# awslabs/aws-c-compression

Measured on AMD Instinct MI355X. Metric: GiB/s input consumed, encode+decode, 1 GiB random bytes; % HBM roofline, higher is better.
Workload: dtype u8

## Files before the change

### aws-c-compression_amd/csrc/hip/decode_common.hpp

```cpp
#ifndef HUFFMAN_AMD_DECODE_COMMON_HPP
#define HUFFMAN_AMD_DECODE_COMMON_HPP
#include "kernels_common.hpp"

namespace {


constexpr u32 kSubWords = HUFD_DEC_SUB_BYTES / 4;
constexpr u32 kSubRows = kSubWords + 2;
constexpr u32 kRowStride = HUFD_DEC_LANES + 1;
constexpr u32 kChunkWords = (kSubRows * kRowStride + 3u) & ~3u;
constexpr u32 kGroupLanes = 16;
constexpr u32 kGroups = HUFD_DEC_LANES / kGroupLanes;
constexpr u32 kQuarters = 4;
constexpr u32 kQuarterBits = HUFD_DEC_SUB_BITS / kQuarters;
constexpr u32 kCpRows = HUFD_DEC_CP_ROWS;
constexpr u32 kEmitThreads = HUFD_DEC_LANES * kQuarters;
constexpr u32 kExitStop = 15, kExitNoRef = 14;
constexpr u8 kRegularFew = 4;

__device__ __forceinline__ u16 fn_pack(bool stop, u32 exit_state, u32 count) {
    return (u16)((stop ? 0x8000u : 0u) | (exit_state << 11) | count);
}
__device__ __forceinline__ u32 wide_pack(bool stop, u32 exit_state, u32 count) {
    return (stop ? 0x80000000u : 0u) | (exit_state << 26) | count;
}
__device__ __forceinline__ u32 widen(u16 f) {
    return wide_pack((f & 0x8000u) != 0, (f >> 11) & 15u, f & 0x7FFu);
}
__device__ __forceinline__ bool wide_stop(u32 f) {
    return (f >> 31) != 0;
}
__device__ __forceinline__ u32 wide_state(u32 f) {
    return (f >> 26) & 31u;
}
__device__ __forceinline__ u32 wide_count(u32 f) {
    return f & 0x03FFFFFFu;
}

__device__ __forceinline__ u32 chunk_word(const u32 *timg, u32 lane, u32 r) {
    return timg[r * kRowStride + lane];
}

__device__ __forceinline__ u32 chunk_window(const u32 *timg, u32 lane, u32 pos) {
    const u32 r = pos >> 5;
    const u64 two = ((u64)chunk_word(timg, lane, r) << 32) | chunk_word(timg, lane, r + 1);
    return (u32)((two << (pos & 31)) >> 32);
}

template <u32 THREADS = HUFD_DEC_LANES>
__device__ __forceinline__ void chunk_load(u32 *timg, const u8 *src, u64 valid_bytes) {
    const u32 t = threadIdx.x;
// ... 512 lines not shown
```

### aws-c-compression_amd/csrc/hip/decode_emit_kernels.hip

```cpp
#include "decode_common.hpp"
#include "launch_common.hpp"

namespace {


__device__ __forceinline__ void dec_emit_chunk(
    const hufd_tables &tb,
    const hufd_dec_item *items,
    const u32 *chunk_item,
    const u8 *d_in,
    u8 *d_out,
    const u16 *fn_tab,
    const u16 *cp_tab,
    const u16 *lane_count_tab,
    const u8 *chunk_regular,
    const u32 *chunk_entry,
    const u64 *chunk_base,
    hufd_dec_result *results,
    u32 c) {

    const u32 ns = tb.n_states;
    u32 *timg = reinterpret_cast<u32 *>(dyn_lds);
    u8 *stage = reinterpret_cast<u8 *>(timg + kChunkWords);
    u16 *ftab = reinterpret_cast<u16 *>(stage);
    u32 *gtab = reinterpret_cast<u32 *>(stage + HUFD_DEC_STAGE_BYTES);
    u32 *g_entry = gtab + kGroups * HUFD_DEC_MAX_STATES;
    u32 *g_base = g_entry + kGroups;
    u32 *l_entry = g_base + kGroups;
    u32 *l_base = l_entry + HUFD_DEC_LANES;
    u32 *l_cnt = l_base + HUFD_DEC_LANES;
    u32 *blk_count = l_cnt + HUFD_DEC_LANES;
    u16 *cpt = reinterpret_cast<u16 *>(blk_count + 4);
    u16 *lut = cpt + kCpRows * HUFD_DEC_LANES;

    const u32 t = threadIdx.x;
    const u32 lane = t % HUFD_DEC_LANES, q = t / HUFD_DEC_LANES;
    const u32 entry = chunk_entry[c];
    if (!(entry & 0x100u)) {
        return;
    }
    const u32 item_index = chunk_item[c];
    const hufd_dec_item it = items[item_index];
    const u64 chunk_off = (u64)(c - it.first_chunk) * HUFD_DEC_CHUNK_BYTES;
    const u64 valid = it.in_len > chunk_off ? it.in_len - chunk_off : 0;
    const u64 cbase = chunk_base[c];

    HUFD_STAMP(1, 0);
    const u16 my_cp = cp_tab[(u64)c * kCpRows * HUFD_DEC_LANES + t];
    u16 my_fn[(HUFD_DEC_MAX_STATES * HUFD_DEC_LANES + kEmitThreads - 1) / kEmitThreads];
#pragma unroll
    for (u32 j = 0; j < sizeof(my_fn) / sizeof(my_fn[0]); ++j) {
        const u32 i = t + j * kEmitThreads;
        my_fn[j] = i < ns * HUFD_DEC_LANES ? fn_tab[(u64)c * ns * HUFD_DEC_LANES + i] : (u16)0;
    }
    chunk_load<kEmitThreads>(timg, d_in + it.in_off + chunk_off, valid);
    lut_load<kEmitThreads>(lut, tb);
    cpt[t] = my_cp;
#pragma unroll
    for (u32 j = 0; j < sizeof(my_fn) / sizeof(my_fn[0]); ++j) {
        const u32 i = t + j * kEmitThreads;
        if (i < ns * HUFD_DEC_LANES) {
            ftab[i] = my_fn[j];
        }
    }
    __syncthreads();
    HUFD_STAMP(1, 1);

    const u32 merged_row = (kQuarters - 1) * HUFD_DEC_LANES;
    bool lane_reached = false;
    u32 lane_state = 0, lane_count = 0, lane_stop = 0, lane_incl = 0;
    if (t < HUFD_DEC_LANES) {
        lane_state = t ? (u32)(cpt[merged_row + t - 1] >> 12) : (entry & 0xFFu);
        l_entry[t] = lane_state == kExitStop ? 1u : 0u;
    }
    if (t == 0) {
        blk_count[1] = 0;
    }
    __syncthreads();
    if (t < HUFD_DEC_LANES) {
        u32 first_unreached = HUFD_DEC_LANES;
        for (u32 w = HUFD_DEC_LANES / kWave; w-- > 0;) {
            const u64 b = __ballot(l_entry[w * kWave + (t & (kWave - 1))] != 0);
            first_unreached = b ? w * kWave + (u32)__builtin_ctzll(b) : first_unreached;
        }
        lane_reached = t < first_unreached;
        const u32 mine_row = cpt[merged_row + t];
        lane_stop = (mine_row >> 12) == kExitStop ? 1u : 0u;
        const bool fits = !lane_reached || (lane_state < kExitNoRef && ((mine_row >> lane_state) & 1u));
        if (!fits) {
            blk_count[1] = 1;
        }
        lane_state = (fits && lane_reached) ? lane_state : 0;
        lane_count = !lane_reached ? 0u
                     : (t != 0 && chunk_regular[c] != 0) ? (u32)lane_count_tab[(u64)c * HUFD_DEC_LANES + t]
                                                         : (u32)(ftab[lane_state * HUFD_DEC_LANES + t] & 0x7FFu);
        lane_incl = wave_inclusive_sum(lane_count, t & (kWave - 1));
        if ((t & (kWave - 1)) == kWave - 1) {
            g_base[t / kWave] = lane_incl;
        }
    }
    __syncthreads();
    const bool all_fit = blk_count[1] == 0;
    if (all_fit) {
        if (t < HUFD_DEC_LANES) {
            u32 before = 0, total = 0;
#pragma unroll
            for (u32 w = 0; w < HUFD_DEC_LANES / kWave; ++w) {
                const u32 sum = g_base[w];
                before += w < t / kWave ? sum : 0;
                total += sum;
            }
            l_base[t] = before + lane_incl - lane_count;
            l_cnt[t] = lane_count;
            l_entry[t] = entry_pack(lane_reached ? lane_state : 0u, lane_reached) | ((lane_reached && lane_stop) ? 0x200u : 0u);
            if (t == 0) {
                blk_count[0] = total;
            }
        }
    } else {
        if (t < kGroups * ns) {
            const u32 g = t / ns, start = t % ns;
            gtab[g * ns + start] = wide_pack(chain_fold(kGroupLanes, start, [&](u32 i, u32 stt) {
                return widen(ftab[stt * HUFD_DEC_LANES + g * kGroupLanes + i]);
            }));
        }
        __syncthreads();
        if (t == 0) {
// ... 107 lines not shown
    HUFD_STAMP(1, 4);

    if (staged && writable) {
        u8 *gbase = out_ptr - mis;
        const u32 lo = mis, hi = mis + writable;
        const u32 row_lo = (lo + 15) >> 4, row_hi = hi >> 4;
        if (row_lo <= row_hi) {
            for (u32 b = lo + t; b < row_lo * 16; b += kEmitThreads) {
                gbase[b] = stage[b];
            }
            for (u32 r = row_lo + t; r < row_hi; r += kEmitThreads) {
                *reinterpret_cast<uint4 *>(gbase + (u64)r * 16) = *reinterpret_cast<const uint4 *>(stage + r * 16);
            }
            for (u32 b = row_hi * 16 + t; b < hi; b += kEmitThreads) {
                gbase[b] = stage[b];
            }
        } else {
            for (u32 b = lo + t; b < hi; b += kEmitThreads) {
                gbase[b] = stage[b];
            }
        }
    }
    HUFD_STAMP(1, 5);
}

__global__ __launch_bounds__(kEmitThreads, 4) void dec_emit_kernel(
    hufd_tables tb,
    const hufd_dec_item *items,
    const u32 *chunk_item,
    u32 n_chunks,
    const u8 *d_in,
    u8 *d_out,
    const u16 *fn_tab,
    const u16 *cp_tab,
    const u16 *lane_count_tab,
    const u8 *chunk_regular,
    const u32 *chunk_entry,
    const u64 *chunk_base,
    hufd_dec_result *results,
    const u32 *list,
    const u32 *list_count,
    u32 *counters = nullptr ,
    u32 *summary = nullptr ,
    u32 self_cleared = 0 ) {
    if (blockIdx.x == 0 && threadIdx.x == 0) {
        if (summary) {
            for (u32 k = 0; k < HUFK_DEC_COUNTERS; ++k) {
                summary[k] = counters[k];
            }
        }
        if (self_cleared) {
            counters[HUFK_DEC_COUNT_SLOW] = 0;
            counters[HUFK_DEC_COUNT_LONG] = 0;
            counters[HUFK_DEC_COUNT_FEW] = 0;
        }
    }
    const u32 n = list ? *list_count : n_chunks;
    for (u32 i = blockIdx.x; i < n; i += gridDim.x) {
        dec_emit_chunk(tb, items, chunk_item, d_in, d_out, fn_tab, cp_tab, lane_count_tab, chunk_regular, chunk_entry, chunk_base, results, list ? list[i] : i);
        __syncthreads();
    }
}


constexpr u32 kEmitChains = 2;
constexpr u32 kEmitFastThreads = kEmitThreads / kEmitChains;

template <u32 LB>
struct emit_shared {
    u32 wlut[1u << LB];
    u32 lane_base[HUFD_DEC_LANES];
    u32 wave_tot[HUFD_DEC_LANES / 64];
    u32 pad[4];
    u8 dump[512];
    u32 tail_words[2][kTailWords];
    u8 stage[HUFD_DEC_STAGE_BYTES + 32];
};

template <u32 LB>
__host__ __device__ constexpr u32 emit_lds_bytes(u32 stage_bytes) {
    return (u32)sizeof(emit_shared<LB>) - HUFD_DEC_STAGE_BYTES + stage_bytes;
}


template <u32 LB, bool TAIL, u32 SURE = 0>
__device__ __forceinline__ void dec_emit_fast_chunk(
    const u32 c,
    const hufd_tables &tb,
    const hufd_chunk_rec *chunk_rec,
    const u8 *d_in,
    u8 *d_out,
    const u16 *cp_tab,
    const u16 *lane_count,
    const hufd_emit_rec *emit_rec,
    hufd_dec_result *results,
    u32 *slow_list,
    u32 *slow_count,
    u32 *dense_list,
    u32 *dense_count,
    u32 stage_limit ) {

    emit_shared<LB> &sh = *reinterpret_cast<emit_shared<LB> *>(dyn_lds);
    const u32 t = threadIdx.x;
    const u32 q = t % kQuarters;
    const u32 lanes[kEmitChains] = {2 * (t / kQuarters), 2 * (t / kQuarters) + 1};
    constexpr bool kNarrowBlock = TAIL && LB == 10;
    constexpr u32 kLutPerThread = kNarrowBlock ? (1u << LB) / HUFD_DEC_LANES : ((1u << LB) + kEmitFastThreads - 1) / kEmitFastThreads;
    const u32 lut_stride = kNarrowBlock ? blockDim.x : kEmitFastThreads;
    u32 lut_raw[kLutPerThread];
#pragma unroll
    for (u32 j = 0; j < kLutPerThread; ++j) {
        const u32 i = t + j * lut_stride;
        lut_raw[j] = i < (1u << LB) ? tb.dec_lut[i >> (LB - tb.lut_bits)] : 0u;
    }
    const hufd_emit_rec erec = emit_rec[c];
    const hufd_chunk_rec rec = chunk_rec[c];
    if (!(erec.flags & HUFD_EMIT_REACHED)) {
        return;
    }
    const u32 s0 = erec.flags & HUFD_EMIT_STATE_MASK;
    const u64 valid = rec.valid;
    if (!TAIL && valid < (u64)HUFD_DEC_CHUNK_BYTES + 8u) {
        return;
    }
    const u32 n_full = !TAIL ? HUFD_DEC_LANES : (valid >= 8u ? (u32)((valid - 8u) / HUFD_DEC_SUB_BYTES) : 0u);
    const u64 cbase = erec.base;
    const u16 *cpt = cp_tab + (u64)c * kCpRows * HUFD_DEC_LANES;
    const u32 merged_row = (kQuarters - 1) * HUFD_DEC_LANES;
    const u32 chunk_symbols = erec.symbols;
    const u32 regular = (erec.flags & HUFD_EMIT_REGULAR_MASK) >> HUFD_EMIT_REGULAR_SHIFT;
    if (TAIL && regular == 3) {
        return;
    }
    const bool fits = regular != 0 && (regular == 2 || !(erec.flags & HUFD_EMIT_STOPS)) && (erec.flags & HUFD_EMIT_MERGED) != 0 &&
                      cbase + chunk_symbols <= rec.out_cap;
    const bool fast = fits && chunk_symbols + 16 <= stage_limit &&
                      (lds_offset_of(sh.wlut) & ((4u << LB) - 1u)) == 0 && SURE <= row_walk(LB, tb.max_bits).sure;
    if (!fast) {
        if (t == 0) {
            if (fits && chunk_symbols + 32 <= 2 * HUFD_DEC_STAGE_BYTES) {
                dense_list[atomicAdd(dense_count, 1u)] = c;
            } else {
                slow_list[atomicAdd(slow_count, 1u)] = c;
            }
        }
        return;
    }

    HUFD_STAMP(1, 0);
    constexpr u32 kRows = kSubWords / kQuarters;
    const u8 *sub[kEmitChains];
    u32 w[kEmitChains][kRows + 1];
    u32 my_cp[kEmitChains], next_cp[kEmitChains], entry_state[kEmitChains], cnt[kEmitChains];
    bool whole[kEmitChains];
#pragma unroll
    for (u32 ch = 0; ch < kEmitChains; ++ch) {
        sub[ch] = d_in + rec.src_off + (u64)lanes[ch] * HUFD_DEC_SUB_BYTES;
        whole[ch] = !TAIL || lanes[ch] < n_full;
#pragma unroll
        for (u32 j = 0; j <= kRows; ++j) {
            w[ch][j] = 0;
        }
        if (whole[ch]) {
            const unaligned_uint4 *p = reinterpret_cast<const unaligned_uint4 *>(sub[ch] + q * kRows * 4);
#pragma unroll
            for (u32 j = 0; j < kRows / 4; ++j) {
                const unaligned_uint4 v = p[j];
                w[ch][4 * j + 0] = __builtin_bswap32(v.x);
                w[ch][4 * j + 1] = __builtin_bswap32(v.y);
                w[ch][4 * j + 2] = __builtin_bswap32(v.z);
                w[ch][4 * j + 3] = __builtin_bswap32(v.w);
            }
            w[ch][kRows] = __builtin_bswap32(reinterpret_cast<const unaligned_u32 *>(sub[ch] + (q + 1) * kRows * 4)->x);
        }
        my_cp[ch] = q ? cpt[(q - 1) * HUFD_DEC_LANES + lanes[ch]] : 0u;
        next_cp[ch] = q + 1 < kQuarters ? cpt[q * HUFD_DEC_LANES + lanes[ch]] : 0u;
        entry_state[ch] = lanes[ch] ? (u32)(cpt[merged_row + lanes[ch] - 1] >> 12) : s0;
        cnt[ch] = lane_count[(u64)c * HUFD_DEC_LANES + lanes[ch]];
    }
#pragma unroll
    for (u32 j = 0; j < kLutPerThread; ++j) {
        const u32 i = t + j * lut_stride;
        const u32 e = lut_raw[j];
        const u32 len = e & 0xFFu;
        if (i < (1u << LB)) {
            sh.wlut[i] = ((e >> 8) << 16) | ((0x10000u - (len ? len : kWalkDeadLen)) & 0xFFFFu);
        }
    }
    const u32 live_t = !TAIL ? kEmitFastThreads
                             : (4 * ((n_full + 1) / 2) + kWave - 1) / kWave * kWave < HUFD_DEC_LANES
                                   ? HUFD_DEC_LANES
                                   : (4 * ((n_full + 1) / 2) + kWave - 1) / kWave * kWave;
    if (TAIL && t >= live_t) {
        __builtin_amdgcn_s_waitcnt(0xC07F);
        return;
    }
    u32 incl = 0, own_cnt = 0;
    if (t < HUFD_DEC_LANES) {
        own_cnt = t < n_full + 2 ? lane_count[(u64)c * HUFD_DEC_LANES + t] : 0u;
        incl = wave_inclusive_sum(t ? own_cnt : 0u, t & (kWave - 1));
        if ((t & (kWave - 1)) == kWave - 1) {
            sh.wave_tot[t / kWave] = incl;
        }
    }
    __syncthreads();
    u32 rest = 0;
#pragma unroll
    for (u32 wv = 0; wv < HUFD_DEC_LANES / kWave; ++wv) {
        rest += sh.wave_tot[wv];
    }
    const u32 first_count = chunk_symbols - rest;
    if (t < HUFD_DEC_LANES) {
        u32 before = 0;
#pragma unroll
        for (u32 wv = 0; wv < HUFD_DEC_LANES / kWave; ++wv) {
            before += wv < t / kWave ? sh.wave_tot[wv] : 0u;
        }
        sh.lane_base[t] = t ? first_count + before + incl - own_cnt : 0u;
    }
    __syncthreads();
    HUFD_STAMP(1, 1);

    u8 *out_ptr = d_out + rec.out_off + cbase;
    const u32 mis = (u32)((uintptr_t)out_ptr & 15u);
    const row_walk rw(LB, tb.max_bits);
    u32 st[kEmitChains];
    u8 *const lds_bytes = reinterpret_cast<u8 *>(&sh);
    const u32 stage_at = (u32)(reinterpret_cast<u8 *>(sh.stage) - lds_bytes), dump_at = (u32)(sh.dump - lds_bytes);
    const u32 stage_base = lds_offset_of(lds_bytes);
    u32 dst[kEmitChains];
    bool idle[kEmitChains];
    bool extend = false;
// ... 19 lines not shown
    for (u32 r = 0; r < kRows; ++r) {
        u64 pair[kEmitChains];
#pragma unroll
        for (u32 ch = 0; ch < kEmitChains; ++ch) {
            pair[ch] = ((u64)w[ch][r] << 32) | w[ch][r + 1];
        }
#pragma unroll
        for (u32 i = 0; i < sure; ++i) {
            u32 e[kEmitChains];
#pragma unroll
            for (u32 ch = 0; ch < kEmitChains; ++ch) {
                e[ch] = lds_word_at(((u32)(pair[ch] >> (st[ch] & 63u)) & rw.mask) | table);
            }
#pragma unroll
            for (u32 ch = 0; ch < kEmitChains; ++ch) {
                lds_bytes[dst[ch]++] = (u8)(e[ch] >> 16);
                st[ch] += e[ch];
            }
        }
#pragma unroll
        for (u32 ch = 0; ch < kEmitChains; ++ch) {
            {
                u32 at = dst[ch] + stage_base;
                emit_uncertain_codes(st[ch], at, pair[ch], table, rw);
                dst[ch] = at - stage_base;
            }
            st[ch] += 32u;
            st[ch] = idle[ch] ? rw.state_at(0, 0) : st[ch];
            dst[ch] = idle[ch] ? dump_at : dst[ch];
        }
    }
    }
    if (extend) {
        const u32 extend_end = (cpt[1 * HUFD_DEC_LANES] & 0x8000u) ? 2 * kRows : ((cpt[2 * HUFD_DEC_LANES] & 0x8000u) ? 3 * kRows : 4 * kRows);
        u32 hi = w[0][kRows];
        for (u32 r = kRows; r < extend_end; ++r) {
            const u32 lo = __builtin_bswap32(reinterpret_cast<const unaligned_u32 *>(d_in + rec.src_off + (r + 1) * 4)->x);
            const u64 pair = ((u64)hi << 32) | lo;
            while ((st[0] & 0xFFFFu) > rw.thr) {
                const u32 e = *reinterpret_cast<const u32 *>(lut + ((u32)(pair >> (st[0] & 63u)) & rw.mask));
                lds_bytes[dst[0]++] = (u8)(e >> 16);
                st[0] += e;
            }
            st[0] += 32u;
            hi = lo;
        }
    }
    HUFD_STAMP(1, 3);
    __syncthreads();
    HUFD_STAMP(1, 4);

    {
        u8 *gbase = out_ptr - mis;
        const u32 lo = mis, hi = mis + (TAIL && n_full < HUFD_DEC_LANES ? sh.lane_base[n_full] : chunk_symbols);
        const u32 row_lo = (lo + 15) >> 4, row_hi = hi >> 4;
        if (row_lo <= row_hi) {
            if (lo + t < row_lo * 16) {
                gbase[lo + t] = sh.stage[lo + t];
            }
#pragma unroll 2
            for (u32 r = row_lo + t; r < row_hi; r += live_t) {
                *reinterpret_cast<uint4 *>(gbase + (u64)r * 16) = *reinterpret_cast<const uint4 *>(sh.stage + r * 16);
            }
            if (row_hi * 16 + t < hi) {
                gbase[row_hi * 16 + t] = sh.stage[row_hi * 16 + t];
            }
        } else if (lo + t < hi) {
            gbase[lo + t] = sh.stage[lo + t];
        }
    }
    HUFD_STAMP(1, 5);
}

template <u32 LB, bool TAIL, u32 SURE = 0>
__global__ __launch_bounds__(kEmitFastThreads, TAIL ? 6 : 8) void dec_emit_fast_kernel(
    hufd_tables tb,
    const hufd_chunk_rec *chunk_rec,
    const u32 *tail_chunks,
    const u8 *d_in,
    u8 *d_out,
    const u16 *cp_tab,
    const u16 *lane_count,
    const hufd_emit_rec *emit_rec,
    hufd_dec_result *results,
    u32 *slow_list,
    u32 *slow_count,
    u32 *dense_list,
    u32 *dense_count,
    u32 stage_limit ) {
    dec_emit_fast_chunk<LB, TAIL, SURE>(
        TAIL ? tail_chunks[blockIdx.x] : blockIdx.x, tb, chunk_rec, d_in, d_out, cp_tab, lane_count, emit_rec, results, slow_list,
        slow_count, dense_list, dense_count, stage_limit);
}

constexpr u32 kEmitBigStage = 2 * HUFD_DEC_STAGE_BYTES;

template <u32 LB, u32 SURE>
__global__ __launch_bounds__(kEmitFastThreads, 4) void dec_emit_big_kernel(
    hufd_tables tb,
    const hufd_chunk_rec *chunk_rec,
    const u8 *d_in,
    u8 *d_out,
    const u16 *cp_tab,
    const u16 *lane_count,
    const hufd_emit_rec *emit_rec,
    hufd_dec_result *results,
    u32 *slow_list,
    u32 *slow_count,
    const u32 *big_list,
    const u32 *big_count) {
    const u32 n = *big_count;
    for (u32 k = blockIdx.x; k < n; k += gridDim.x) {
        if (chunk_rec[big_list[k]].valid < HUFD_DEC_CHUNK_BYTES + 8u) {
            continue;
        }
        dec_emit_fast_chunk<LB, false, SURE>(
            big_list[k], tb, chunk_rec, d_in, d_out, cp_tab, lane_count, emit_rec, results, slow_list, slow_count, slow_list,
            slow_count, kEmitBigStage);
        __syncthreads();
    }
}


template <u32 LB>
struct emit_pack_shared {
    u32 wlut[1u << LB];
    u32 lane_excl[HUFD_DEC_LANES + 4];
    u32 wave_tot[HUFD_DEC_LANES / 64];
    u32 slot_chunk[kPackMaxSlots];
    u32 slot_full[kPackMaxSlots];
    u8 dump[512];
    __attribute__((aligned(16))) u8 stage[16];
};
__host__ __device__ constexpr u32 emit_pack_stage_bytes(u32 stage_limit) {
    return (stage_limit + 32u + 15u) & ~15u;
}

template <u32 LB, u32 SURE>
__global__ __launch_bounds__(kEmitFastThreads, 6) void dec_emit_pack_kernel(
    hufd_tables tb,
    const hufd_chunk_rec *chunk_rec,
    const u32 *tail_chunks,
    u32 n_tail,
    u32 width,
    u32 slots,
    const u8 *d_in,
    u8 *d_out,
    const u16 *cp_tab,
    const u16 *lane_count,
    const u8 *chunk_regular,
    const u32 *chunk_fn,
    const u32 *chunk_entry,
    const u64 *chunk_base,
    u32 *slow_list,
    u32 *slow_count,
    u32 stage_limit ) {

    emit_pack_shared<LB> &sh = *reinterpret_cast<emit_pack_shared<LB> *>(dyn_lds);
    const u32 ns = tb.n_states;
    const u32 t = threadIdx.x;
    const u32 half = (width + 1) / 2, slot_threads = kQuarters * half, slot_lanes = 2 * half;
    const u32 slot = t / slot_threads, tt = t % slot_threads;
    const u32 q = tt % kQuarters;
    const u32 lanes[kEmitChains] = {2 * (tt / kQuarters), 2 * (tt / kQuarters) + 1};
    constexpr u32 kLutPerThread = ((1u << LB) + kEmitFastThreads - 1) / kEmitFastThreads;
    u32 lut_raw[kLutPerThread];
#pragma unroll
    for (u32 j = 0; j < kLutPerThread; ++j) {
        const u32 i = t + j * kEmitFastThreads;
        lut_raw[j] = i < (1u << LB) ? tb.dec_lut[i >> (LB - tb.lut_bits)] : 0u;
    }
    const u32 li = blockIdx.x * slots + slot;
    const bool have = slot < slots && li < n_tail;
    const u32 c = have ? tail_chunks[li] : 0u;
    const u32 centry = have ? chunk_entry[c] : 0u;
    const u32 s0 = centry & 0xFFu;
    const hufd_chunk_rec rec = chunk_rec[c];
    const u64 valid = rec.valid;
    const u32 n_full = valid >= 8u ? (u32)((valid - 8u) / HUFD_DEC_SUB_BYTES) : 0u;
    const u64 cbase = have ? chunk_base[c] : 0;
    const u16 *cpt = cp_tab + (u64)c * kCpRows * HUFD_DEC_LANES;
    const u32 merged_row = (kQuarters - 1) * HUFD_DEC_LANES;
    const u32 f0 = have ? chunk_fn[(u64)c * ns + s0] : 0u;
    const u32 chunk_symbols = wide_count(f0);
    const u32 regular = have ? chunk_regular[c] : 0u;
    const bool wanted = have && (centry & 0x100u) != 0 && regular != 3;
    const bool fits = wanted && regular == 2 && ((cpt[merged_row] >> s0) & 1u) != 0 && cbase + chunk_symbols <= rec.out_cap;
    const bool fast = fits && chunk_symbols + 16 <= stage_limit && n_full + 2 <= slot_lanes &&
                      (lds_offset_of(sh.wlut) & ((4u << LB) - 1u)) == 0 && SURE <= row_walk(LB, tb.max_bits).sure;
    if (tt == 0 && slot < kPackMaxSlots) {
        sh.slot_chunk[slot] = fast ? c : HUFD_NONE32;
        sh.slot_full[slot] = n_full;
        if (wanted && !fast) {
            slow_list[atomicAdd(slow_count, 1u)] = c;
        }
    }

    constexpr u32 kRows = kSubWords / kQuarters;
    u32 w[kEmitChains][kRows + 1];
    u32 my_cp[kEmitChains], next_cp[kEmitChains], entry_state[kEmitChains], cnt[kEmitChains];
    bool whole[kEmitChains];
#pragma unroll
    for (u32 ch = 0; ch < kEmitChains; ++ch) {
        whole[ch] = fast && lanes[ch] < n_full;
#pragma unroll
        for (u32 j = 0; j <= kRows; ++j) {
            w[ch][j] = 0;
        }
        my_cp[ch] = next_cp[ch] = entry_state[ch] = cnt[ch] = 0;
        if (whole[ch]) {
            const u8 *sub = d_in + rec.src_off + (u64)lanes[ch] * HUFD_DEC_SUB_BYTES;
            const unaligned_uint4 *p = reinterpret_cast<const unaligned_uint4 *>(sub + q * kRows * 4);
#pragma unroll
            for (u32 j = 0; j < kRows / 4; ++j) {
                const unaligned_uint4 v = p[j];
                w[ch][4 * j + 0] = __builtin_bswap32(v.x);
                w[ch][4 * j + 1] = __builtin_bswap32(v.y);
                w[ch][4 * j + 2] = __builtin_bswap32(v.z);
                w[ch][4 * j + 3] = __builtin_bswap32(v.w);
            }
            w[ch][kRows] = __builtin_bswap32(reinterpret_cast<const unaligned_u32 *>(sub + (q + 1) * kRows * 4)->x);
            my_cp[ch] = q ? cpt[(q - 1) * HUFD_DEC_LANES + lanes[ch]] : 0u;
            next_cp[ch] = q + 1 < kQuarters ? cpt[q * HUFD_DEC_LANES + lanes[ch]] : 0u;
            entry_state[ch] = lanes[ch] ? (u32)(cpt[merged_row + lanes[ch] - 1] >> 12) : s0;
            cnt[ch] = lane_count[(u64)c * HUFD_DEC_LANES + lanes[ch]];
        }
    }
#pragma unroll
    for (u32 j = 0; j < kLutPerThread; ++j) {
        const u32 i = t + j * kEmitFastThreads;
        const u32 e = lut_raw[j];
        const u32 len = e & 0xFFu;
        if (i < (1u << LB)) {
            sh.wlut[i] = ((e >> 8) << 16) | ((0x10000u - (len ? len : kWalkDeadLen)) & 0xFFFFu);
        }
    }
    __syncthreads();

    u32 incl = 0, own = 0;
    if (t < HUFD_DEC_LANES) {
        const u32 sa = t / slot_lanes, la = t % slot_lanes;
        const u32 ca = sa < slots && sa < kPackMaxSlots ? sh.slot_chunk[sa] : HUFD_NONE32;
        own = ca != HUFD_NONE32 && la != 0 && la < sh.slot_full[sa] + 2 && la < HUFD_DEC_LANES ? lane_count[(u64)ca * HUFD_DEC_LANES + la] : 0u;
        incl = wave_inclusive_sum(own, t & (kWave - 1));
        if ((t & (kWave - 1)) == kWave - 1) {
            sh.wave_tot[t / kWave] = incl;
        }
    }
    __syncthreads();
    if (t < HUFD_DEC_LANES) {
        u32 before = 0;
#pragma unroll
        for (u32 wv = 0; wv < HUFD_DEC_LANES / kWave; ++wv) {
            before += wv < t / kWave ? sh.wave_tot[wv] : 0u;
        }
        sh.lane_excl[t] = before + incl - own;
        if (t == HUFD_DEC_LANES - 1) {
            sh.lane_excl[HUFD_DEC_LANES] = before + incl;
        }
    }
    __syncthreads();
    if (!fast) {
        return;
    }

    const u32 base_g = slot * slot_lanes;
    const u32 slot_first = sh.lane_excl[base_g], slot_end = sh.lane_excl[base_g + slot_lanes];
    const u32 first_count = chunk_symbols - (slot_end - slot_first);
    const auto base_of = [&](u32 l) { return l ? first_count + sh.lane_excl[base_g + l] - slot_first : 0u; };
    u8 *out_ptr = d_out + rec.out_off + cbase;
    const u32 mis = (u32)((uintptr_t)out_ptr & 15u);
    const row_walk rw(LB, tb.max_bits);
    u8 *const lds_bytes = reinterpret_cast<u8 *>(&sh);
    const u32 stage_at = (u32)(sh.stage - lds_bytes) + slot * emit_pack_stage_bytes(stage_limit), dump_at = (u32)(sh.dump - lds_bytes);
    u32 st[kEmitChains], dst[kEmitChains];
    bool idle[kEmitChains];
// ... 16 lines not shown
        for (u32 r = 0; r < kRows; ++r) {
            u64 pair[kEmitChains];
#pragma unroll
            for (u32 ch = 0; ch < kEmitChains; ++ch) {
                pair[ch] = ((u64)w[ch][r] << 32) | w[ch][r + 1];
            }
#pragma unroll
            for (u32 i = 0; i < SURE; ++i) {
                u32 e[kEmitChains];
#pragma unroll
                for (u32 ch = 0; ch < kEmitChains; ++ch) {
                    e[ch] = lds_word_at(((u32)(pair[ch] >> (st[ch] & 63u)) & rw.mask) | table);
                }
#pragma unroll
                for (u32 ch = 0; ch < kEmitChains; ++ch) {
                    lds_bytes[dst[ch]++] = (u8)(e[ch] >> 16);
                    st[ch] += e[ch];
                }
            }
#pragma unroll
            for (u32 ch = 0; ch < kEmitChains; ++ch) {
                while ((st[ch] & 0xFFFFu) > rw.thr) {
                    const u32 e = lds_word_at(((u32)(pair[ch] >> (st[ch] & 63u)) & rw.mask) | table);
                    lds_bytes[dst[ch]++] = (u8)(e >> 16);
                    st[ch] += e;
                }
                st[ch] += 32u;
                st[ch] = idle[ch] ? rw.state_at(0, 0) : st[ch];
                dst[ch] = idle[ch] ? dump_at : dst[ch];
            }
        }
    }
    if (extend) {
        const u32 extend_end = (cpt[1 * HUFD_DEC_LANES] & 0x8000u) ? 2 * kRows : ((cpt[2 * HUFD_DEC_LANES] & 0x8000u) ? 3 * kRows : 4 * kRows);
        u32 hi = w[0][kRows];
        for (u32 r = kRows; r < extend_end; ++r) {
            const u32 lo = __builtin_bswap32(reinterpret_cast<const unaligned_u32 *>(d_in + rec.src_off + (r + 1) * 4)->x);
            const u64 pair = ((u64)hi << 32) | lo;
            while ((st[0] & 0xFFFFu) > rw.thr) {
                const u32 e = lds_word_at(((u32)(pair >> (st[0] & 63u)) & rw.mask) | table);
                lds_bytes[dst[0]++] = (u8)(e >> 16);
                st[0] += e;
            }
            st[0] += 32u;
            hi = lo;
        }
    }
    __syncthreads();

    {
        u8 *gbase = out_ptr - mis;
        const u8 *stage = lds_bytes + stage_at;
        const u32 lo = mis, hi = mis + base_of(n_full);
        const u32 row_lo = (lo + 15) >> 4, row_hi = hi >> 4;
        if (row_lo <= row_hi) {
            if (lo + tt < row_lo * 16) {
                gbase[lo + tt] = stage[lo + tt];
            }
            for (u32 r = row_lo + tt; r < row_hi; r += slot_threads) {
                *reinterpret_cast<uint4 *>(gbase + (u64)r * 16) = *reinterpret_cast<const uint4 *>(stage + r * 16);
            }
            if (row_hi * 16 + tt < hi) {
                gbase[row_hi * 16 + tt] = stage[row_hi * 16 + tt];
            }
        } else if (lo + tt < hi) {
            gbase[lo + tt] = stage[lo + tt];
        }
    }
}

__global__ __launch_bounds__(kTailThreads) void dec_emit_tail_kernel(
    hufd_tables tb,
    const hufd_dec_item *items,
    const u32 *chunk_item,
    const u32 *tail_chunks,
    u32 n_tail,
    const u8 *d_in,
    u8 *d_out,
    const u16 *cp_tab,
    const u16 *lane_count,
    const u8 *chunk_regular,
    const u32 *chunk_fn,
    const u32 *chunk_entry,
    const u64 *chunk_base,
    hufd_dec_result *results,
    u32 stage_limit ) {

    tail_lds &sh = *reinterpret_cast<tail_lds *>(dyn_lds);
    u16 *lut = reinterpret_cast<u16 *>(dyn_lds + sizeof(tail_lds));
    for (u32 i = threadIdx.x; i < (1u << tb.lut_bits); i += kTailThreads) {
        lut[i] = tb.dec_lut[i];
    }
    __syncthreads();
    const u32 i = blockIdx.x * kTailThreads + threadIdx.x;
    if (i >= n_tail) {
        return;
    }
    const u32 c = tail_chunks[i];
    const u32 centry = chunk_entry[c];
    const u32 kind = chunk_regular[c];
    if (!(centry & 0x100u) || (kind != 2 && kind != 3)) {
        return;
    }
    const u32 ns = tb.n_states, s0 = centry & 0xFFu;
    const u32 item_index = chunk_item[c];
    const hufd_dec_item it = items[item_index];
    const u64 chunk_off = (u64)(c - it.first_chunk) * HUFD_DEC_CHUNK_BYTES;
    const u64 valid = it.in_len - chunk_off;
    const u64 cbase = chunk_base[c];
    if (kind == 3) {
        u32 *tiny = sh.words[threadIdx.x];
        load_be32_run(tiny, d_in + it.in_off + chunk_off, valid, kTailWords);
        const u64 room = it.out_cap > cbase ? it.out_cap - cbase : 0;
        u8 *out = d_out + it.out_off + cbase;
        const u32 rem = (u32)(valid * 8);
        tail_reader tr;
        tr.start(tiny, s0);
        u32 pos = s0, why = HUFD_STOP_NONE;
        u64 n = 0;
        for (;;) {
            u32 sym = 0;
            const u32 len = code_at(tr.peek(), lut, tb.lut_bits, pos, rem, &sym, &why);
            if (!len) {
                results[item_index].stop_kind = why;
                results[item_index].stop_bit = chunk_off * 8 + pos;
                break;
            }
            if (n == room) {
                results[item_index].cap_bit = chunk_off * 8 + pos;
                break;
            }
            out[n++] = (u8)sym;
            tr.skip(len);
            pos += len;
        }
        return;
    }
    const u16 *cpt = cp_tab + (u64)c * kCpRows * HUFD_DEC_LANES;
    const u32 merged_row = (kQuarters - 1) * HUFD_DEC_LANES;
    const u32 f0 = chunk_fn[(u64)c * ns + s0];
    const u32 chunk_symbols = wide_count(f0);
    if (((cpt[merged_row] >> s0) & 1u) == 0 || cbase + chunk_symbols > it.out_cap || chunk_symbols + 16 > stage_limit) {
        return;
    }
    const u32 n_full = (u32)((valid - 8u) / HUFD_DEC_SUB_BYTES);
    const u32 first = n_full, second = n_full + 1;
    const u32 n_first = lane_count[(u64)c * HUFD_DEC_LANES + first];
    const u32 n_second = second < HUFD_DEC_LANES ? lane_count[(u64)c * HUFD_DEC_LANES + second] : 0u;
    const u32 entry = cpt[merged_row + first - 1] >> 12;
    const u8 *tsrc = d_in + it.in_off + chunk_off + (u64)n_full * HUFD_DEC_SUB_BYTES;
    const u64 tail_bytes = valid - (u64)n_full * HUFD_DEC_SUB_BYTES;
    u32 *words = sh.words[threadIdx.x];
    load_be32_run(words, tsrc, tail_bytes, kTailWords);
    const u32 limit = (second < HUFD_DEC_LANES ? 2u : 1u) * HUFD_DEC_SUB_BITS;
    u8 *out = d_out + it.out_off + cbase + (chunk_symbols - n_first - n_second);
    u32 stop_pos = 0, stop_why = HUFD_STOP_NONE;
    (void)tail_follow(words, lut, tb.lut_bits, entry, (u32)(tail_bytes * 8), limit, out, &stop_pos, &stop_why);
    if (stop_why != HUFD_STOP_NONE) {
        results[item_index].stop_kind = stop_why;
        results[item_index].stop_bit = (chunk_off + (u64)n_full * HUFD_DEC_SUB_BYTES) * 8 + stop_pos;
    }
}


static uint32_t dec_emit_lds_bytes(const hufd_tables *tb) {
    return kChunkWords * 4 + HUFD_DEC_STAGE_BYTES + kGroups * HUFD_DEC_MAX_STATES * 4 + kGroups * 8 +
           HUFD_DEC_LANES * 12 + 16 + kCpRows * HUFD_DEC_LANES * 2 + (2u << tb->lut_bits) + 16;
}

}

using hufk_host::persistent_grid;
using hufk_host::stage_mark;
using hufk_host::current_compute_units;
using hufk_host::kBesideMinChunks;
using hufk_host::decode_launch_state;

hipError_t hufk_host::init_decode_emit(int lds_max) {
    hipError_t e = hipFuncSetAttribute(
        reinterpret_cast<const void *>(&dec_emit_kernel), hipFuncAttributeMaxDynamicSharedMemorySize, lds_max);
#define HUFK_ALLOW_BIG_LDS(LBV, SUREV)                                                                                  \
    if (e == hipSuccess) {                                                                                             \
        e = hipFuncSetAttribute(                                                                                       \
            reinterpret_cast<const void *>(&dec_emit_big_kernel<LBV, SUREV>), hipFuncAttributeMaxDynamicSharedMemorySize, \
            lds_max);                                                                                                  \
    }
    HUFK_ALLOW_BIG_LDS(10, 3)
    HUFK_ALLOW_BIG_LDS(10, 4)
    HUFK_ALLOW_BIG_LDS(12, 2)
#undef HUFK_ALLOW_BIG_LDS
    return e;
}

void hufk_host::decode_emit_stage(const struct hufk_decode_args *a, hipStream_t st, const decode_launch_state &s) {
    const uint32_t lb_of_launch = s.lb, sure = s.sure;
    u32 *const emit_count = a->counters + HUFK_DEC_COUNT_EMIT, *const dense_count = a->counters + HUFK_DEC_COUNT_DENSE;
#define HUFK_LAUNCH_EMIT_FAST(LBV, TAILV, SUREV, GRID, STREAMV)                                                          \
hipLaunchKernelGGL(                                                                                                \
    (dec_emit_fast_kernel<LBV, TAILV, SUREV>), dim3(GRID), dim3((TAILV) && (LBV) == 10 ? tail_block : kEmitFastThreads), \
    emit_lds_bytes<LBV>(TAILV ? tail_stage : HUFD_DEC_STAGE_BYTES), STREAMV, a->tables, a->chunk_rec,              \
    emit_single_chunks, (const u8 *)a->d_in, (u8 *)a->d_out, (const u16 *)a->cp_tab, (const u16 *)a->lane_count,   \
    (const hufd_emit_rec *)a->emit_rec, a->results, a->emit_list, emit_count,                                      \
    !TAILV && big ? a->dense_list : a->emit_list, !TAILV && big ? dense_count : emit_count,                  \
    TAILV ? tail_stage : HUFD_DEC_STAGE_BYTES)
    const uint32_t tail_live = a->tail_wide_lanes ? (kQuarters * ((a->tail_wide_lanes + 1) / 2) + kWave - 1) / kWave * kWave : kEmitFastThreads;
    const uint32_t tail_block = tail_live < HUFD_DEC_LANES ? HUFD_DEC_LANES : (tail_live < kEmitFastThreads ? tail_live : kEmitFastThreads);
    const bool some_inside = a->n_tail < a->n_chunks;
    const bool big = !a->quiet;
    const bool have_side = a->n_tail && a->side_stream && a->fork_event && a->join_event && a->n_chunks >= kBesideMinChunks;
    const bool beside = some_inside && have_side && (uint64_t)a->n_tail * 8 <= a->n_chunks;
    hipStream_t tst = beside ? (hipStream_t)a->side_stream : st;
    hipStream_t ends_st = have_side ? (hipStream_t)a->side_stream : st;
    (void)tst;
    (void)ends_st;
    if (have_side) {
        (void)hipEventRecord((hipEvent_t)a->fork_event, st);
        (void)hipStreamWaitEvent((hipStream_t)a->side_stream, (hipEvent_t)a->fork_event, 0);
    }
    const uint32_t emit_sure = sure;
    const uint32_t epack_width = a->tail_lanes + 2u < 16u ? 16u : a->tail_lanes + 2u;
    const uint32_t epack_threads = kQuarters * ((epack_width + 1) / 2);
    const uint32_t epack_stage = emit_pack_stage_bytes((a->tail_stage_bytes + 255u) & ~255u);
    const uint32_t epack_fixed = (uint32_t)(a->tables.lut_bits <= 10 ? sizeof(emit_pack_shared<10>) : sizeof(emit_pack_shared<12>));
    uint32_t epack_slots = kEmitFastThreads / epack_threads;
    epack_slots = epack_slots > kPackMaxSlots ? kPackMaxSlots : epack_slots;
    epack_slots = epack_slots * epack_stage + epack_fixed > 60u * 1024u ? (60u * 1024u - epack_fixed) / epack_stage : epack_slots;
    const bool epack = a->one_chunk_a_workgroup == 0 && a->n_tail_narrow >= kPackMinChunks && epack_width <= HUFD_DEC_LANES / 2 &&
                       a->tail_stage_bytes && epack_slots >= 2;
    const uint32_t tail_stage = epack ? (a->tail_stage_bytes + 255u) & ~255u
                                : a->tail_stage_bytes >= 4096 && a->tail_stage_bytes < HUFD_DEC_STAGE_BYTES
                                    ? (a->tail_stage_bytes + 255u) & ~255u
                                    : HUFD_DEC_STAGE_BYTES;
    const uint32_t e_packed = epack ? a->n_tail_narrow : 0u, e_single = a->n_tail - e_packed;
    const u32 *emit_single_chunks = a->tail_chunks + e_packed;
#define HUFK_LAUNCH_EMIT_PACK(LBV, SUREV)                                                                               \
hipLaunchKernelGGL(                                                                                                \
    (dec_emit_pack_kernel<LBV, SUREV>), dim3((e_packed + epack_slots - 1) / epack_slots), dim3(kEmitFastThreads),    \
    (uint32_t)sizeof(emit_pack_shared<LBV>) + epack_slots * epack_stage, tst, a->tables, a->chunk_rec, a->tail_chunks, \
    e_packed, epack_width, epack_slots, (const u8 *)a->d_in, (u8 *)a->d_out, (const u16 *)a->cp_tab,               \
    (const u16 *)a->lane_count, (const u8 *)a->chunk_regular, (const u32 *)a->chunk_fn, (const u32 *)a->chunk_entry, \
    (const u64 *)a->chunk_base, a->emit_list, emit_count, tail_stage)
    if (e_packed) {
        if (lb_of_launch == 10) {
            switch (emit_sure) {
                case 3: HUFK_LAUNCH_EMIT_PACK(10, 3); break;
                default: HUFK_LAUNCH_EMIT_PACK(10, 4); break;
            }
        } else {
            HUFK_LAUNCH_EMIT_PACK(12, 2);
        }
    }
#undef HUFK_LAUNCH_EMIT_PACK
    if (lb_of_launch == 10) {
        if (e_single) {
            switch (emit_sure) {
                case 3: HUFK_LAUNCH_EMIT_FAST(10, true, 3, e_single, tst); break;
                default: HUFK_LAUNCH_EMIT_FAST(10, true, 4, e_single, tst); break;
            }
        }
        if (some_inside) {
            switch (emit_sure) {
                case 3: HUFK_LAUNCH_EMIT_FAST(10, false, 3, a->n_chunks, st); break;
                default: HUFK_LAUNCH_EMIT_FAST(10, false, 4, a->n_chunks, st); break;
            }
        }
    } else {
        if (e_single) {
            HUFK_LAUNCH_EMIT_FAST(12, true, 2, e_single, tst);
        }
        if (some_inside) {
            HUFK_LAUNCH_EMIT_FAST(12, false, 2, a->n_chunks, st);
        }
    }
#undef HUFK_LAUNCH_EMIT_FAST
    if (a->n_tail) {
        const uint32_t lds = (uint32_t)sizeof(tail_lds) + (2u << a->tables.lut_bits);
        hipLaunchKernelGGL(
            dec_emit_tail_kernel, dim3((a->n_tail + kTailThreads - 1) / kTailThreads), dim3(kTailThreads), lds, ends_st,
            a->tables, a->items, a->chunk_item, a->tail_chunks, a->n_tail, (const u8 *)a->d_in, (u8 *)a->d_out,
            (const u16 *)a->cp_tab, (const u16 *)a->lane_count, (const u8 *)a->chunk_regular,
            (const u32 *)a->chunk_fn, (const u32 *)a->chunk_entry, (const u64 *)a->chunk_base, a->results, tail_stage);
    }
    if (have_side) {
        (void)hipEventRecord((hipEvent_t)a->join_event, (hipStream_t)a->side_stream);
        (void)hipStreamWaitEvent(st, (hipEvent_t)a->join_event, 0);
    }
#define HUFK_LAUNCH_EMIT_BIG(LBV, SUREV)                                                                                \
do {                                                                                                               \
    const uint32_t lds = emit_lds_bytes<LBV>(kEmitBigStage);                                                       \
    hipLaunchKernelGGL(                                                                                            \
        (dec_emit_big_kernel<LBV, SUREV>),                                                                         \
        dim3(persistent_grid(dec_emit_big_kernel<LBV, SUREV>, kEmitFastThreads, lds, a->n_chunks)),                 \
        dim3(kEmitFastThreads), lds, st, a->tables, a->chunk_rec, (const u8 *)a->d_in, (u8 *)a->d_out,             \
        (const u16 *)a->cp_tab, (const u16 *)a->lane_count, (const hufd_emit_rec *)a->emit_rec, a->results,        \
        a->emit_list, emit_count,                                                                               \
        (const u32 *)a->dense_list, (const u32 *)dense_count);                                                  \
} while (0)
    if (!big) {
    } else if (lb_of_launch == 10) {
        switch (emit_sure) {
            case 3: HUFK_LAUNCH_EMIT_BIG(10, 3); break;
            default: HUFK_LAUNCH_EMIT_BIG(10, 4); break;
        }
    } else {
        HUFK_LAUNCH_EMIT_BIG(12, 2);
    }
#undef HUFK_LAUNCH_EMIT_BIG
    hipLaunchKernelGGL(
        dec_emit_kernel,
        dim3(persistent_grid(dec_emit_kernel, kEmitThreads, dec_emit_lds_bytes(&a->tables), a->n_chunks)),
        dim3(kEmitThreads), dec_emit_lds_bytes(&a->tables), st, a->tables, a->items, a->chunk_item, a->n_chunks,
        (const u8 *)a->d_in, (u8 *)a->d_out, a->fn_tab, a->cp_tab, (const u16 *)a->lane_count,
        (const u8 *)a->chunk_regular, a->chunk_entry, a->chunk_base, a->results, (const u32 *)a->emit_list,
        (const u32 *)emit_count, a->counters, a->summary, a->counters_self_cleared);
}
```

### aws-c-compression_amd/csrc/hip/decode_launch.hip

```cpp
#include "decode_common.hpp"
#include "launch_common.hpp"

namespace {


__device__ void dec_finish_item(
    const hufd_dec_item &it,
    u64 total,
    bool stopped,
    hufd_dec_item_state *state,
    hufd_dec_result *result) {
    state->total_symbols = total;
    result->total_symbols = total;
    result->cap_bit = kNoBit;
    result->reserved = 0;
    if (!stopped) {
        result->stop_kind = HUFD_STOP_END;
        result->stop_bit = it.in_len * 8;
    } else {
        result->stop_kind = HUFD_STOP_NONE;
        result->stop_bit = kNoBit;
    }
}

__device__ __forceinline__ hufd_emit_rec emit_rec_of(
    u32 c, u32 state, bool stopped, u64 total, u32 f, const u8 *chunk_regular, const u16 *cp_tab) {
    hufd_emit_rec r;
    r.flags = state & HUFD_EMIT_STATE_MASK;
    r.symbols = 0;
    r.base = total;
    if (!stopped) {
        const u32 regular = chunk_regular[c];
        const u32 merged = cp_tab[((u64)c * kCpRows + (kQuarters - 1)) * HUFD_DEC_LANES];
        r.flags |= HUFD_EMIT_REACHED | (regular << HUFD_EMIT_REGULAR_SHIFT) | (((merged >> state) & 1u) ? HUFD_EMIT_MERGED : 0u) |
                   (wide_stop(f) ? HUFD_EMIT_STOPS : 0u);
        r.symbols = wide_count(f);
    }
    return r;
}

__global__ __launch_bounds__(256) void dec_scan_small_kernel(
    const hufd_dec_item *items,
    u32 n_items,
    u32 ns,
    const u32 *chunk_fn,
    const u8 *chunk_regular,
    const u16 *cp_tab,
    u32 *chunk_entry,
    u64 *chunk_base,
    hufd_emit_rec *emit_rec,
    hufd_dec_item_state *states,
    hufd_dec_result *results) {

    const u32 i = blockIdx.x * blockDim.x + threadIdx.x;
    if (i >= n_items) {
        return;
    }
    const hufd_dec_item it = items[i];
    if (it.tiny) {
        return;
    }
    if (it.n_chunks > HUFD_SCAN_SMALL_MAX) {
        return;
    }
    u32 state = it.first_bit;
    u64 total = 0;
    bool stopped = false;
    for (u32 k = 0; k < it.n_chunks; ++k) {
        const u32 c = it.first_chunk + k;
        chunk_entry[c] = entry_pack(state, !stopped);
        chunk_base[c] = total;
        const u32 f = stopped ? 0u : chunk_fn[(u64)c * ns + state];
        emit_rec[c] = emit_rec_of(c, state, stopped, total, f, chunk_regular, cp_tab);
        if (!stopped) {
            total += wide_count(f);
            stopped = wide_stop(f);
            state = wide_state(f);
        }
    }
    dec_finish_item(it, total, stopped, &states[i], &results[i]);
}

constexpr u32 kRunChunks = HUFD_SCAN_RUN_CHUNKS, kSubRun = HUFD_SCAN_SUB_CHUNKS, kSubRuns = kRunChunks / kSubRun;

__device__ __forceinline__ u32 scan_run_load(const hufd_dec_item &it, u32 k, u32 ns, const u32 *chunk_fn, u32 *fn, u32 *sub) {
    const u32 lo = k * kRunChunks;
    const u32 n = it.n_chunks - lo < kRunChunks ? it.n_chunks - lo : kRunChunks;
    const u32 *src = chunk_fn + (u64)(it.first_chunk + lo) * ns;
    for (u32 i = threadIdx.x; i < n * ns; i += blockDim.x) {
        fn[i] = src[i];
    }
    __syncthreads();
    if (threadIdx.x < kSubRuns * ns) {
        const u32 j = threadIdx.x / ns, start = threadIdx.x % ns;
        const u32 first = j * kSubRun;
        const u32 cnt = first < n ? (n - first < kSubRun ? n - first : kSubRun) : 0;
        sub[j * ns + start] =
            wide_pack(chain_fold(cnt, start, [&](u32 i, u32 stt) { return fn[(first + i) * ns + stt]; }));
    }
    __syncthreads();
    return n;
}

__device__ __host__ constexpr u32 scan_run_lds_bytes_device(u32 ns) {
    return kRunChunks * ns * 4 + kSubRuns * ns * 4 + kSubRuns * 4 + kSubRuns * 8 + 16;
}
// ... 40 lines not shown
        }
        __syncthreads();
        const u32 groups = (n + kTopGroup - 1) / kTopGroup;
        for (u32 idx = threadIdx.x; idx < groups * ns; idx += blockDim.x) {
            const u32 g = idx / ns, first = g * kTopGroup;
            const u32 cnt = n - first < kTopGroup ? n - first : kTopGroup;
            const fold_result r = chain_fold(cnt, idx % ns, [&](u32 q, u32 stt) { return fn[(first + q) * ns + stt]; });
            group_to[idx] = (r.stop ? 0x80000000u : 0u) | r.state;
            group_count[idx] = (u32)r.count;
        }
        __syncthreads();
        for (u32 g = 0; g < groups && !p.stopped; ++g) {
            const u32 to = group_to[g * ns + p.state];
            p.total += group_count[g * ns + p.state];
            p.stopped = (to >> 31) != 0;
            p.state = to & 0x7FFFFFFFu;
        }
    }
    __syncthreads();
    return p;
}

static uint32_t scan_apply_lds_bytes(uint32_t ns) {
    return scan_run_lds_bytes(ns) + kTopTile * ns * 4 + 2 * kTopGroups * ns * 4;
}

__global__ __launch_bounds__(256) void dec_scan_apply_kernel(
    const hufd_dec_item *items,
    const u32 *runs,
    u32 ns,
    const u32 *chunk_fn,
    const u32 *run_fn,
    const u8 *chunk_regular,
    const u16 *cp_tab,
    u32 *chunk_entry,
    u64 *chunk_base,
    hufd_emit_rec *emit_rec,
    hufd_dec_item_state *states,
    hufd_dec_result *results) {
    u32 *fn = reinterpret_cast<u32 *>(dyn_lds);
    u32 *sub = fn + kRunChunks * ns;
    u32 *sub_entry = sub + kSubRuns * ns;
    u64 *sub_base = reinterpret_cast<u64 *>(sub_entry + kSubRuns);
    u32 *path_fn = reinterpret_cast<u32 *>(dyn_lds + scan_run_lds_bytes_device(ns));
    u32 *path_group = path_fn + kTopTile * ns;
    const u32 run = blockIdx.x;
    const u32 item = runs[2 * run], k = runs[2 * run + 1];
    const hufd_dec_item it = items[item];
    const scan_point at = scan_path_to_run(it, run_fn + (u64)(run - k) * ns, k, ns, path_fn, path_group);
    const u32 n = scan_run_load(it, k, ns, chunk_fn, fn, sub);
    if (threadIdx.x == 0) {
        u32 state = at.state;
        bool stopped = at.stopped;
        u64 total = at.total;
        for (u32 j = 0; j < kSubRuns; ++j) {
            sub_entry[j] = entry_pack(state, !stopped);
            sub_base[j] = total;
            if (!stopped) {
                const u32 f = sub[j * ns + state];
                total += wide_count(f);
                stopped = wide_stop(f);
                state = wide_state(f);
            }
        }
        if ((k + 1) * kRunChunks >= it.n_chunks) {
            dec_finish_item(it, total, stopped, &states[item], &results[item]);
        }
    }
    __syncthreads();
    if (threadIdx.x < kSubRuns) {
        const u32 j = threadIdx.x;
        u32 state = sub_entry[j] & 0xFFu;
        bool stopped = !(sub_entry[j] & 0x100u);
        u64 total = sub_base[j];
        const u32 first = j * kSubRun;
        const u32 cnt = first < n ? (n - first < kSubRun ? n - first : kSubRun) : 0;
        for (u32 q = 0; q < cnt; ++q) {
            const u32 c = it.first_chunk + k * kRunChunks + first + q;
            chunk_entry[c] = entry_pack(state, !stopped);
            chunk_base[c] = total;
            if (!stopped) {
                const u32 f = fn[(first + q) * ns + state];
                total += wide_count(f);
                stopped = wide_stop(f);
                state = wide_state(f);
            }
        }
    }
    __syncthreads();
    for (u32 q = threadIdx.x; q < n; q += blockDim.x) {
        const u32 c = it.first_chunk + k * kRunChunks + q;
        const u32 centry = chunk_entry[c];
        const u32 state = centry & 0xFFu;
        const bool stopped = !(centry & 0x100u);
        emit_rec[c] = emit_rec_of(c, state, stopped, chunk_base[c], stopped ? 0u : fn[q * ns + state], chunk_regular, cp_tab);
    }
}


__global__ __launch_bounds__(256) void dec_plan_chunks_kernel(
    const hufd_dec_item *items, u32 n_items, u32 n_chunks, u32 *chunk_item, hufd_chunk_rec *chunk_rec) {
    const u32 c = blockIdx.x * blockDim.x + threadIdx.x;
    if (c >= n_chunks) {
        return;
    }
    u32 lo = 0, hi = n_items;
    while (hi - lo > 1) {
        const u32 mid = lo + (hi - lo) / 2;
        if (items[mid].first_chunk <= c) {
            lo = mid;
        } else {
            hi = mid;
        }
    }
    const hufd_dec_item it = items[lo];
    const u64 off = (u64)(c - it.first_chunk) * HUFD_DEC_CHUNK_BYTES, left = it.in_len - off;
    hufd_chunk_rec rec;
    rec.src_off = it.in_off + off;
    rec.out_off = it.out_off;
    rec.out_cap = it.out_cap;
    rec.valid = left < 0xFFFFFFFFull ? (u32)left : 0xFFFFFFFFu;
    rec.item = lo;
    rec.entry_bit = c == it.first_chunk ? it.first_bit : HUFD_NONE32;
    rec.reserved = 0;
    chunk_item[c] = lo;
    chunk_rec[c] = rec;
}

// ... 190 lines not shown
    const bool fixed = a->n_fixed_blocks && a->tables.fixed_bits;
    if (fixed) {
        (void)hipMemsetAsync(a->states, 0xFF, (size_t)a->n_items * sizeof(hufd_dec_item_state), st);
    }
    const uint32_t lb_of_launch = a->tables.lut_bits <= 10 ? 10u : 12u;
    const uint32_t sure_of_coder = row_walk(lb_of_launch, a->tables.max_bits).sure;
    const uint32_t sure = lb_of_launch == 10 ? (sure_of_coder > 4 ? 4u : sure_of_coder) : (sure_of_coder > 2 ? 2u : sure_of_coder);
    if (a->n_chunks && (a->tables.max_bits > HUFD_DEC_MAX_LUT_BITS || (lb_of_launch == 10 ? sure < 3 : sure != 2))) {
        return (int)hipErrorInvalidValue;
    }
    const bool one_go = a->n_tiny || a->n_deep || fixed;
    struct hufk_decode_args counting;
    const struct hufk_decode_args *items_pass = a;
    if (pk && one_go) {
        const int e = hufk_unpack_blank(a->items, a->n_items, pk->items, st);
        if (e) {
            return e;
        }
        counting = *a;
        counting.items = pk->items;
        items_pass = &counting;
    }
    decode_launch_state state = {lb_of_launch, sure, false};
    if (a->n_chunks) {
        if (!a->counters_self_cleared) {
            (void)hipMemsetAsync(a->counters, 0, HUFK_DEC_COUNTERS * sizeof(uint32_t), st);
        }
        hufk_host::decode_sync_stage(a, st, state);
    }
    stage_mark(a->stage_events, 1, st);
    if (a->n_tiny != a->n_items && a->n_large != a->n_items) {
        hipLaunchKernelGGL(
            dec_scan_small_kernel, dim3((a->n_items + 255) / 256), dim3(256), 0, st, a->items, a->n_items, ns, a->chunk_fn,
            (const u8 *)a->chunk_regular, (const u16 *)a->cp_tab, a->chunk_entry, a->chunk_base, a->emit_rec, a->states, a->results);
    }
    hufk_host::decode_items_stage(items_pass, st);
    if (a->n_large) {
        const uint32_t lds = scan_run_lds_bytes(ns);
        hipLaunchKernelGGL(
            dec_scan_runs_kernel, dim3(a->n_runs), dim3(256), lds, st, a->items, a->runs, ns, a->chunk_fn, a->run_fn);
        hipLaunchKernelGGL(
            dec_scan_apply_kernel, dim3(a->n_runs), dim3(256), scan_apply_lds_bytes(ns), st, a->items, a->runs, ns, a->chunk_fn,
            (const u32 *)a->run_fn, (const u8 *)a->chunk_regular, (const u16 *)a->cp_tab, a->chunk_entry, a->chunk_base,
            a->emit_rec, a->states, a->results);
    }
    hufk_host::decode_sync_true_stage(a, st, state);
    stage_mark(a->stage_events, 2, st);
    struct hufk_decode_args placed;
    if (pk) {
        const int e = hufk_unpack_offsets(
            a->items, a->results, a->n_items, pk->tile_items, pk->align, pk->capacity, pk->tile_sums, pk->offsets, pk->items,
            pk->summary, a->chunk_rec, a->n_chunks, pk->chunk_rec, pk->stored_rec, st);
        if (e) {
            return e;
        }
        placed = *a;
        placed.items = pk->items;
        placed.chunk_rec = pk->chunk_rec;
        placed.tail_stage_bytes = pk->tail_stage_bytes;
        a = &placed;
        if (one_go) {
            if (fixed) {
                (void)hipMemsetAsync(a->states, 0xFF, (size_t)a->n_items * sizeof(hufd_dec_item_state), st);
            }
            hufk_host::decode_items_stage(a, st);
        }
    }
    if (a->n_chunks) {
        hufk_host::decode_emit_stage(a, st, state);
    }
    if (pk && pk->stored_rec) {
        const int e = hufk_stored_copy_decode(
            pk->stored_rec, pk->stored_tile_first, pk->stored_tiles, a->n_items, pk->items, a->results, a->d_in, a->d_out, st);
        if (e) {
            return e;
        }
// ... 38 lines not shown
```

### aws-c-compression_amd/csrc/hip/decode_sync_kernels.hip

```cpp
#include "decode_common.hpp"
#include "launch_common.hpp"

namespace {


template <u32 NS>
__device__ __forceinline__ void dec_sync_chunk(
    const hufd_tables &tb,
    const hufd_dec_item *items,
    const u32 *chunk_item,
    const u8 *d_in,
    u16 *fn_tab,
    u16 *cp_tab,
    u32 *chunk_fn,
    u8 *chunk_regular,
    u32 c) {

    const u32 ns = tb.n_states;
    u32 *timg = reinterpret_cast<u32 *>(dyn_lds);
    u16 *ftab = reinterpret_cast<u16 *>(timg);
    u32 *gtab = timg + kChunkWords;
    u16 *lut = reinterpret_cast<u16 *>(gtab + kGroups * ns);

    const u32 lane = threadIdx.x;
    const hufd_dec_item it = items[chunk_item[c]];
    const u64 chunk_off = (u64)(c - it.first_chunk) * HUFD_DEC_CHUNK_BYTES;
    const u64 valid = it.in_len > chunk_off ? it.in_len - chunk_off : 0;
    if (lane == 0) {
        chunk_regular[c] = 0;
    }

    HUFD_STAMP(0, 0);
    chunk_load(timg, d_in + it.in_off + chunk_off, valid);
    lut_load(lut, tb);
    const u32 shift = 32 - tb.lut_bits;

    __syncthreads();
    HUFD_STAMP(0, 1);

    const u32 rem = clamp_remaining(valid, lane);
    constexpr u32 kDead = 0xFFFFFFFFu;
    constexpr u32 kNobody = 0xFFFFFFFEu;

    u32 pos[NS], cnt[NS];
    u32 p = kDead;
    {
// ... 63 lines not shown
        r_live = r_live && !ref_stop && ref_pos < end;
        if (qq + 1 < kQuarters) {
            cp_ok[qq] = r_live && ref_pos - bound < 16u;
            cp_pos[qq] = ref_pos;
            cp_steps[qq] = ref_steps;
        }
    }
    if (have_ref && ref_pos < HUFD_DEC_SUB_BITS) {
        ref_stop = true;
    }
    const u32 ref_exit = ref_stop ? 0 : ref_pos - HUFD_DEC_SUB_BITS;
    u16 fn[NS];
#pragma unroll
    for (u32 s = 0; s < NS; ++s) {
        if (pos[s] == kDead) {
            fn[s] = fn_pack(true, 0, cnt[s] - 1u);
        } else if (have_ref) {
            fn[s] = fn_pack(ref_stop, ref_exit, (cnt[s] + ref_steps) & 0x7FFu);
        } else {
            fn[s] = fn_pack(false, pos[s] - HUFD_DEC_SUB_BITS, cnt[s]);
        }
    }
    HUFD_STAMP(0, 3);
    __syncthreads();
    HUFD_STAMP(0, 4);
#pragma unroll
    for (u32 s = 0; s < NS; ++s) {
        if (s < ns) {
            ftab[s * HUFD_DEC_LANES + lane] = fn[s];
            fn_tab[((u64)c * ns + s) * HUFD_DEC_LANES + lane] = fn[s];
        }
    }
    {
        u16 *cp = cp_tab + (u64)c * kCpRows * HUFD_DEC_LANES + lane;
#pragma unroll
        for (u32 qq = 0; qq + 1 < kQuarters; ++qq) {
            const u32 tail = ref_steps - cp_steps[qq];
            cp[qq * HUFD_DEC_LANES] =
                (u16)(cp_ok[qq] ? 0x8000u | ((cp_pos[qq] - (qq + 1) * kQuarterBits) << 11) | tail : 0u);
        }
        u32 merged = 0;
#pragma unroll
        for (u32 s = 0; s < NS; ++s) {
            merged |= (have_ref && pos[s] != kDead) ? 1u << s : 0u;
        }
        const u32 common = have_ref ? (ref_stop ? kExitStop : ref_exit) : kExitNoRef;
        cp[(kQuarters - 1) * HUFD_DEC_LANES] = (u16)(merged | (common << 12));
    }
    __syncthreads();

    if (lane < kGroups * ns) {
        const u32 g = lane / ns, start = lane % ns;
        gtab[g * ns + start] = wide_pack(chain_fold(kGroupLanes, start, [&](u32 i, u32 stt) {
            return widen(ftab[stt * HUFD_DEC_LANES + g * kGroupLanes + i]);
        }));
    }
    __syncthreads();
    if (lane < ns) {
        chunk_fn[(u64)c * ns + lane] =
            wide_pack(chain_fold(kGroups, lane, [&](u32 g, u32 stt) { return gtab[g * ns + stt]; }));
    }
    HUFD_STAMP(0, 5);
}

template <u32 NS>
__global__ __launch_bounds__(HUFD_DEC_LANES) void dec_sync_kernel(
    hufd_tables tb,
    const hufd_dec_item *items,
    const u32 *chunk_item,
    u32 n_chunks,
    const u8 *d_in,
    u16 *fn_tab,
    u16 *cp_tab,
    u32 *chunk_fn,
    u8 *chunk_regular,
    const u32 *list,
    const u32 *list_count,
    u32 *clear ) {
    if (clear && blockIdx.x == 0 && threadIdx.x == 0) {
        clear[HUFK_DEC_COUNT_EMIT] = 0;
        clear[HUFK_DEC_COUNT_DENSE] = 0;
    }
    const u32 n = list ? *list_count : n_chunks;
    for (u32 i = blockIdx.x; i < n; i += gridDim.x) {
        const u32 c = list ? list[i] : i;
        if (list && chunk_regular[c] == kRegularFew) {
            continue;
        }
        dec_sync_chunk<NS>(tb, items, chunk_item, d_in, fn_tab, cp_tab, chunk_fn, chunk_regular, c);
        __syncthreads();
    }
}

template <u32 LB>
struct lean_shared {
    u32 wlut[1u << LB];
    u32 exit_state[HUFD_DEC_LANES];
    u32 sub0[kFastMaxMeet + 4];
    u32 wave_sum[HUFD_DEC_LANES / 64];
    u32 bad;
    u32 pad[3];
    u16 hops[1u << LB];
};



constexpr u32 kOneRecs = 9;
__device__ __host__ constexpr u32 one_rec_row(u32 j) {
    return j == 0 ? 6u : j == 1 ? 8u : j == 2 ? 10u : j == 3 ? 12u : j == 4 ? 16u : j == 5 ? 20u : j == 6 ? 24u : j == 7 ? 28u : 32u;
}
constexpr u32 kOneMaxMerge = kSubWords;
constexpr u32 kOneMaxMerge0 = kSubWords;
constexpr u32 kOneRecs0 = kOneRecs;
constexpr u32 kOneGarbageRow = 4, kOneGarbageDead = 48;

__device__ __host__ constexpr u32 one_rec_index(u32 row) {
    u32 at = kOneRecs;
    for (u32 j = 0; j < kOneRecs; ++j) {
        at = one_rec_row(j) == row ? j : at;
    }
    return at;
}
// ... 29 lines not shown
    }
    template <u32 SURE>
    __device__ __forceinline__ u32 row(u32 state, u32 xh, u32 xl, u32 table) const {
#pragma unroll
        for (u32 i = 0; i < SURE; ++i) {
            state += look(state, xh, xl, table);
        }
        return byte_rows_uncertain(state, xh, xl, table, mask, thr);
    }
};

template <u32 LB>
struct one_shared {
    u32 wlut[1u << LB];
    u32 exit_state[HUFD_DEC_LANES];
    u32 sub0[kSubWords + 4];
    u32 last0;
    u32 tiny[kTailWords];
    u32 wave_sum[HUFD_DEC_LANES / 64];
    u32 bad;
    u32 decided0;
    u32 moved;
    u32 bad_mine;

};

template <u32 LB, u32 SURE, bool TAIL = false>
__global__ __launch_bounds__(HUFD_DEC_LANES, 8) void dec_sync_one_kernel(
    hufd_tables tb,
    const hufd_chunk_rec *chunk_rec,
    const u32 *tail_chunks,
    const u8 *d_in,
    u16 *fn_tab,
    u16 *cp_tab,
    u32 *chunk_fn,
    u16 *lane_count,
    u8 *chunk_regular,
    u32 *tail_entry,
    u32 *slow_list,
    u32 *slow_count,
    u32 *long_list,
    u32 *long_count) {
    constexpr bool FOLLOW = false;
    const u32 c = TAIL ? wave_uniform(tail_chunks[blockIdx.x]) : blockIdx.x;
#include "decode_sync_one_body.inc"
}

template <u32 LB, u32 SURE>
__global__ __launch_bounds__(HUFD_DEC_LANES, 8) void dec_sync_one_mixed_kernel(
    hufd_tables tb,
    const hufd_chunk_rec *chunk_rec,
    const u32 *tail_chunks,
    u32 n_tail,
    const u8 *d_in,
    u16 *fn_tab,
    u16 *cp_tab,
    u32 *chunk_fn,
    u16 *lane_count,
    u8 *chunk_regular,
    u32 *tail_entry,
    u32 *slow_list,
    u32 *slow_count,
    u32 *long_list,
    u32 *long_count) {
    if (blockIdx.x < n_tail) {
        constexpr bool TAIL = true, FOLLOW = true;
        const u32 c = wave_uniform(tail_chunks[blockIdx.x]);
#include "decode_sync_one_body.inc"
    } else {
        constexpr bool TAIL = false, FOLLOW = false;
        const u32 c = blockIdx.x - n_tail;
#include "decode_sync_one_body.inc"
    }
}




template <u32 LB>
struct pack_shared {
    u32 wlut[1u << LB];
    u32 exit_state[HUFD_DEC_LANES];
    u32 sub0[kPackMaxSlots][kFastMaxMeet + 4];
    u32 sum[kPackMaxSlots];
    u32 bad[kPackMaxSlots];
    u32 alive[kPackMaxSlots];
    u32 meet0[kPackMaxSlots];
    u32 tail0[kPackMaxSlots];
    u16 hops[1u << LB];
};

template <u32 LB, u32 SURE>
__global__ __launch_bounds__(HUFD_DEC_LANES, 6) void dec_sync_pack_kernel(
    hufd_tables tb,
    const hufd_chunk_rec *chunk_rec,
    const u32 *tail_chunks,
    u32 n_tail,
    u32 width,
    const u8 *d_in,
    u16 *fn_tab,
    u16 *cp_tab,
    u32 *chunk_fn,
    u16 *lane_count,
    u8 *chunk_regular,
    u32 *tail_entry,
    u32 *long_list,
    u32 *long_count) {

    pack_shared<LB> &sh = *reinterpret_cast<pack_shared<LB> *>(dyn_lds);
    const u32 ns = tb.n_states;
    const u32 t = threadIdx.x;
    const u32 slots = HUFD_DEC_LANES / width;
    const u32 slot = t / width, lane = t % width;
    const row_walk rw(LB, tb.max_bits);
    const u32 table = lds_offset_of(sh.wlut);
    {
        constexpr u32 kLutPerLane = (1u << LB) / HUFD_DEC_LANES;
        u32 lut_raw[kLutPerLane];
#pragma unroll
        for (u32 j = 0; j < kLutPerLane; ++j) {
            lut_raw[j] = tb.dec_lut[(t + j * HUFD_DEC_LANES) >> (LB - tb.lut_bits)];
        }
#pragma unroll
        for (u32 j = 0; j < kLutPerLane; ++j) {
            const u32 len = lut_raw[j] & 0xFFu;
            sh.wlut[t + j * HUFD_DEC_LANES] = 0x10000u - (len ? len : kWalkDeadLen);
            sh.hops[t + j * HUFD_DEC_LANES] = (u16)(len ? 1u << len : 0u);
        }
    }
    const u32 li = blockIdx.x * slots + slot;
    const bool have = slot < slots && li < n_tail;
    const u32 c = have ? tail_chunks[li] : 0u;
    const hufd_chunk_rec rec = chunk_rec[c];
    const u64 valid = rec.valid;
    const u8 *src = d_in + rec.src_off;
    const u32 n_full = valid >= 8u ? (u32)((valid - 8u) / HUFD_DEC_SUB_BYTES) : 0u;
    const bool eligible = tb.lut_bits <= LB && tb.max_bits <= HUFD_DEC_MAX_LUT_BITS && rw.sure >= SURE && (table & ((4u << LB) - 1u)) == 0 &&
                          n_full <= width;
    bool mine = have;
    if (mine && n_full == 0 && tb.lut_bits <= HUFD_DEC_MAX_LUT_BITS) {
        if (lane == 0) {
            chunk_regular[c] = 3;
        }
        mine = false;
    }
    if (mine && !eligible) {
        if (lane == 0) {
            chunk_regular[c] = 0;
            long_list[atomicAdd(long_count, 1u)] = c;
        }
        mine = false;
    }
    const bool active = mine && lane < n_full;
    u16 *cp = cp_tab + (u64)c * kCpRows * HUFD_DEC_LANES;
    u32 w[kFastRows];
    {
        const u32 from = active ? lane : 0u;
        const u8 *at = mine ? src + (u64)from * HUFD_DEC_SUB_BYTES : d_in;
        const unaligned_uint4 *line = reinterpret_cast<const unaligned_uint4 *>(at);
#pragma unroll
        for (u32 q = 0; q < kSubWords / 4; ++q) {
            const unaligned_uint4 v = mine ? line[q] : unaligned_uint4{0, 0, 0, 0};
            w[4 * q + 0] = v.x;
            w[4 * q + 1] = v.y;
            w[4 * q + 2] = v.z;
            w[4 * q + 3] = v.w;
        }
        w[kSubWords] = mine ? reinterpret_cast<const unaligned_u32 *>(at + HUFD_DEC_SUB_BYTES)->x : 0u;
    }
#pragma unroll
    for (u32 r = 0; r < kFastRows; ++r) {
        w[r] = __builtin_bswap32(w[r]);
    }
    if (slot < kPackMaxSlots && lane == 0) {
        sh.bad[slot] = 0;
        sh.sum[slot] = 0;
        sh.alive[slot] = 0;
#pragma unroll
        for (u32 r = 0; r <= kFastMaxMeet; ++r) {
            sh.sub0[slot][r] = w[r];
        }
    }
    __syncthreads();

    u64 heads = active ? (1ull << ns) - 1ull : 0ull;
    u32 meet_row = 0;
    bool one = false, settled = false;
// ... 67 lines not shown
            const u32 lo = sh.sub0[slot][r + 1];
            st = lean_row<SURE, true>(st, hi, lo, table, rw);
            const bool now = rw.died(st) && !dd;
            cand_dead = now ? (st >> 16) - 1u : cand_dead;
            dd = dd || now;
            st = rw.next_row(st, dd);
            hi = lo;
        }
        cand_reached = !dd && rw.offset_of(st) == target;
        cand_count = (st >> 16) + sh.tail0[slot];
        if (cand_reached) {
            atomicOr(&sh.alive[slot], 1u << lane);
        }
    }
    if (active && lane) {
        atomicAdd(&sh.sum[slot], count);
    }
    if (mine && !ok) {
        sh.bad[slot] = 1;
    }
    __syncthreads();
    if (!mine) {
        return;
    }
    if (sh.bad[slot]) {
        if (lane == 0) {
            chunk_regular[c] = 0;
            long_list[atomicAdd(long_count, 1u)] = c;
        }
        return;
    }

    if (active) {
        u16 *mcp = cp + lane;
#pragma unroll
        for (u32 qq = 0; qq + 1 < kQuarters; ++qq) {
            const bool usable = (qq + 1) * (kSubWords / kQuarters) >= meet_row;
            u32 tail = ref_count - (cp_state[qq] >> 16), bits = rw.offset_of(cp_state[qq]);
            bool have_cp = usable;
            if (qq == 0 && late && lane != 0) {
                tail = count - (head_cp >> 16);
                bits = rw.offset_of(head_cp);
                have_cp = true;
            }
            mcp[qq * HUFD_DEC_LANES] = (u16)(have_cp ? 0x8000u | (bits << 11) | tail : 0u);
        }
        lane_count[(u64)c * HUFD_DEC_LANES + lane] = (u16)(lane ? count : ref_count);
        mcp[(kQuarters - 1) * HUFD_DEC_LANES] = (u16)((lane ? 1u << entry : sh.alive[slot]) | (ref_exit << 12));
    }
    if (lane < 2 && n_full + lane < HUFD_DEC_LANES) {
        const u32 l = n_full + lane;
#pragma unroll
        for (u32 qq = 0; qq + 1 < kQuarters; ++qq) {
            cp[qq * HUFD_DEC_LANES + l] = 0;
        }
        lane_count[(u64)c * HUFD_DEC_LANES + l] = 0;
        cp[(kQuarters - 1) * HUFD_DEC_LANES + l] = (u16)(kExitStop << 12);
    }
    if (lane + 1 == n_full) {
        tail_entry[c] = ref_exit;
    }
    if (lane == 0) {
        chunk_regular[c] = 2;
    }
    if (lane < ns) {
        const u32 rest = sh.sum[slot];
        const u32 first_exit = sh.exit_state[slot * width];
        fn_tab[((u64)c * ns + lane) * HUFD_DEC_LANES] =
            cand_reached ? fn_pack(false, first_exit, cand_count & 0x7FFu) : fn_pack(true, 0, cand_dead);
        chunk_fn[(u64)c * ns + lane] = cand_reached ? wide_pack(false, 0u, cand_count + rest) : wide_pack(true, 0, cand_dead);
    }
}


constexpr u32 kGuessRows = 8;
constexpr u32 kGuessRounds = 6;
constexpr u32 kGuessDeadMark = 1u << 25;
constexpr u32 kGuessDeadEntry = kGuessDeadMark + 0x10000u - 1u;

template <u32 LB, u32 SURE>
__device__ __forceinline__ void dec_sync_guess_chunk(
    const u32 c,
    const hufd_tables &tb,
    const hufd_chunk_rec *chunk_rec,
    const u8 *d_in,
    u16 *fn_tab,
    u16 *cp_tab,
    u32 *chunk_fn,
    u16 *lane_count,
    u8 *chunk_regular,
    u32 *slow_list,
    u32 *slow_count) {

    lean_shared<LB> &sh = *reinterpret_cast<lean_shared<LB> *>(dyn_lds);
    u32 *again = sh.pad;
    const u32 ns = tb.n_states;
    const u32 lane = threadIdx.x;
    const hufd_chunk_rec rec = chunk_rec[c];
    const u8 *src = d_in + rec.src_off;
    const row_walk rw(LB, tb.max_bits);
    const u32 table = lds_offset_of(sh.wlut);
    const bool eligible = tb.lut_bits <= LB && tb.max_bits <= HUFD_DEC_MAX_LUT_BITS && tb.min_bits >= 3 && rw.sure >= SURE &&
                          (table & ((4u << LB) - 1u)) == 0;
    if (!eligible) {
        if (lane == 0) {
            slow_list[atomicAdd(slow_count, 1u)] = c;
        }
        return;
    }

    for (u32 i = lane; i < (1u << LB); i += HUFD_DEC_LANES) {
        const u32 len = tb.dec_lut[i >> (LB - tb.lut_bits)] & 0xFFu;
        sh.wlut[i] = len ? 0x10000u - len : kGuessDeadEntry;
        sh.hops[i] = (u16)(len ? 1u << len : 0u);
    }
    if (lane == 0) {
        sh.bad = 0;
        again[0] = 0;
    }
    __syncthreads();
    u32 meet_row = 0, meet_bit = 0;
    if (lane < kWave) {
// ... 141 lines not shown
                if (e & kGuessDeadMark) {
                    dd = true;
                    cand_dead = st >> 16;
                } else {
                    st += e;
                }
            }
            st = rw.next_row(st, dd);
            hi = lo;
        }
        cand_reached = !dd && lane < ns && rw.offset_of(st) == target;
        cand_alive = __ballot(cand_reached);
        cand_count = (st >> 16) + tail0;
    }

    const u32 wsum = wave_sum(lane ? count : 0u);
    if ((lane & (kWave - 1)) == 0) {
        sh.wave_sum[lane / kWave] = wsum;
    }
    if (!ok) {
        sh.bad = 1;
    }
    __syncthreads();
    if (sh.bad) {
        if (lane == 0) {
            slow_list[atomicAdd(slow_count, 1u)] = c;
        }
        return;
    }

    u32 lane_o = lane;
    opaque(lane_o);
    u16 *fn_out = fn_tab + (u64)c * ns * HUFD_DEC_LANES;
    u16 *cp = cp_tab + (u64)c * kCpRows * HUFD_DEC_LANES + lane_o;
#pragma unroll
    for (u32 qq = 0; qq + 1 < kQuarters; ++qq) {
        const bool have = lane != 0 || (qq + 1) * (kSubWords / kQuarters) >= meet_row;
        const u32 tail = count - (cp_state[qq] >> 16), bits = rw.offset_of(cp_state[qq]);
        cp[qq * HUFD_DEC_LANES] = (u16)(have ? 0x8000u | (bits << 11) | tail : 0u);
    }
    lane_count[(u64)c * HUFD_DEC_LANES + lane_o] = (u16)count;
    cp[(kQuarters - 1) * HUFD_DEC_LANES] = (u16)((lane ? 1u << entry : (u32)cand_alive) | (exit_bit << 12));
    if (lane == 0) {
        chunk_regular[c] = 1;
    }
    if (lane < ns) {
        u32 rest = 0;
#pragma unroll
        for (u32 wv = 0; wv < HUFD_DEC_LANES / kWave; ++wv) {
            rest += sh.wave_sum[wv];
        }
        const u32 first_exit = sh.exit_state[0];
        const u32 last_exit = sh.exit_state[HUFD_DEC_LANES - 1];
        fn_out[(u64)lane_o * HUFD_DEC_LANES] =
            cand_reached ? fn_pack(false, first_exit, cand_count & 0x7FFu) : fn_pack(true, 0, cand_dead);
        chunk_fn[(u64)c * ns + lane_o] =
            cand_reached ? wide_pack(false, last_exit, cand_count + rest) : wide_pack(true, 0, cand_dead);
    }
}

template <u32 LB, u32 SURE>
__global__ __launch_bounds__(HUFD_DEC_LANES, 4) void dec_sync_guess_kernel(
    hufd_tables tb,
    const hufd_chunk_rec *chunk_rec,
    const u8 *d_in,
    u16 *fn_tab,
    u16 *cp_tab,
    u32 *chunk_fn,
    u16 *lane_count,
    u8 *chunk_regular,
    const u32 *given_up,
    const u32 *given_up_count,
    u32 *slow_list,
    u32 *slow_count) {
    const u32 n = *given_up_count;
    for (u32 k = blockIdx.x; k < n; k += gridDim.x) {
        const u32 c = given_up[k];
        if (chunk_rec[c].valid < (u64)HUFD_DEC_CHUNK_BYTES + 8u) {
            if (threadIdx.x == 0) {
                slow_list[atomicAdd(slow_count, 1u)] = c;
            }
            continue;
        }
        dec_sync_guess_chunk<LB, SURE>(c, tb, chunk_rec, d_in, fn_tab, cp_tab, chunk_fn, lane_count, chunk_regular, slow_list, slow_count);
        __syncthreads();
    }
}


constexpr u32 kFewMaxWalks = 8;
constexpr u32 kFewHeadRows = 2;

template <u32 LB>
struct few_shared {
    u32 wlut[1u << LB];
    u16 ftab[HUFD_DEC_MAX_STATES * HUFD_DEC_LANES];
    u32 gtab[kGroups * HUFD_DEC_MAX_STATES];
    u32 entry_of[HUFD_DEC_LANES];
    u32 bad;
    u32 pad[3];
};

template <u32 LB>
__device__ __forceinline__ u32 few_row(u32 st, u32 hi, u32 lo, u32 table, const row_walk &rw, bool &dd, u32 &dead_count) {
    st = lean_row<0, true, true>(st, hi, lo, table, rw);
    const bool now = rw.died(st) && !dd;
    dead_count = now ? (st >> 16) - 1u : dead_count;
    dd = dd || now;
    return rw.next_row(st, dd);
}

template <u32 LB>
__device__ __forceinline__ void few_load_words(u32 (&w)[kFastRows], const u8 *sub) {
    const unaligned_uint4 *line = reinterpret_cast<const unaligned_uint4 *>(sub);
#pragma unroll
    for (u32 q = 0; q < kSubWords / 4; ++q) {
        const unaligned_uint4 v = line[q];
        w[4 * q + 0] = __builtin_bswap32(v.x);
        w[4 * q + 1] = __builtin_bswap32(v.y);
        w[4 * q + 2] = __builtin_bswap32(v.z);
        w[4 * q + 3] = __builtin_bswap32(v.w);
    }
    w[kSubWords] = __builtin_bswap32(reinterpret_cast<const unaligned_u32 *>(sub + HUFD_DEC_SUB_BYTES)->x);
}

template <u32 LB>
__device__ __forceinline__ void few_table(few_shared<LB> &sh, const hufd_tables &tb, u32 lane) {
    for (u32 i = lane; i < (1u << LB); i += HUFD_DEC_LANES) {
        const u32 len = tb.dec_lut[i >> (LB - tb.lut_bits)] & 0xFFu;
        sh.wlut[i] = 0x10000u - (len ? len : kWalkDeadLen);
    }
}

template <u32 LB>
__global__ __launch_bounds__(HUFD_DEC_LANES, 4) void dec_sync_few_kernel(
    hufd_tables tb,
    const hufd_chunk_rec *chunk_rec,
    const u8 *d_in,
    u16 *fn_tab,
    u16 *cp_tab,
    u32 *chunk_fn,
    u8 *chunk_regular,
    const u32 *list,
    const u32 *list_count,
    u32 *done_list,
    u32 *done_count) {

    few_shared<LB> &sh = *reinterpret_cast<few_shared<LB> *>(dyn_lds);
    const u32 ns = tb.n_states;
    const u32 lane = threadIdx.x;
    const u32 table = lds_offset_of(sh.wlut);
    const row_walk rw(LB, tb.max_bits);
    const u32 n = *list_count;
    if (n == 0 || tb.lut_bits > LB || tb.max_bits > HUFD_DEC_MAX_LUT_BITS || ns > HUFD_DEC_MAX_STATES || (table & ((4u << LB) - 1u)) != 0) {
        return;
    }
    few_table<LB>(sh, tb, lane);
    if (lane == 0) {
        sh.bad = 0;
    }
    __syncthreads();
    for (u32 k = blockIdx.x; k < n; k += gridDim.x) {
        const u32 c = list[k];
        const hufd_chunk_rec rec = chunk_rec[c];
        if (rec.valid < (u64)HUFD_DEC_CHUNK_BYTES + 8u) {
            continue;
        }
        u32 w[kFastRows];
        few_load_words<LB>(w, d_in + rec.src_off + (u64)lane * HUFD_DEC_SUB_BYTES);

        u32 landed = 0, pending = 0;
#pragma unroll
        for (u32 s = 0; s < HUFD_DEC_MAX_STATES; ++s) {
// ... 20 lines not shown
            bool dd = false;
#pragma unroll
            for (u32 r = kFewHeadRows; r < kSubWords; ++r) {
                st = few_row<LB>(st, w[r], w[r + 1], table, rw, dd, dead_count);
            }
            const u32 ex = rw.offset_of(st);
            ok = ok && (dd || ex < ns);
            const u32 more = dd ? dead_count : st >> 16;
            for (u32 s = 0; s < ns; ++s) {
                const u32 f = sh.ftab[s * HUFD_DEC_LANES + lane];
                if (((pending >> s) & 1u) && ((f >> 11) & 15u) == o) {
                    sh.ftab[s * HUFD_DEC_LANES + lane] = fn_pack(dd, dd ? 0u : ex & 15u, ((f & 0x7FFu) + more) & 0x7FFu);
                    pending &= ~(1u << s);
                }
            }
        }
        if (!ok) {
            sh.bad = 1;
        }
        __syncthreads();
        const bool bad = sh.bad != 0;
        __syncthreads();
        if (bad) {
            if (lane == 0) {
                sh.bad = 0;
            }
            __syncthreads();
            continue;
        }
        for (u32 s = 0; s < ns; ++s) {
            fn_tab[((u64)c * ns + s) * HUFD_DEC_LANES + lane] = sh.ftab[s * HUFD_DEC_LANES + lane];
        }
        {
            u16 *cp = cp_tab + (u64)c * kCpRows * HUFD_DEC_LANES + lane;
#pragma unroll
            for (u32 qq = 0; qq + 1 < kQuarters; ++qq) {
                cp[qq * HUFD_DEC_LANES] = 0;
            }
            cp[(kQuarters - 1) * HUFD_DEC_LANES] = (u16)(kExitNoRef << 12);
        }
        __syncthreads();
        if (lane < kGroups * ns) {
            const u32 g = lane / ns, start = lane % ns;
            sh.gtab[g * ns + start] = wide_pack(chain_fold(kGroupLanes, start, [&](u32 i, u32 stt) {
                return widen(sh.ftab[stt * HUFD_DEC_LANES + g * kGroupLanes + i]);
            }));
        }
        __syncthreads();
        if (lane < ns) {
            chunk_fn[(u64)c * ns + lane] =
                wide_pack(chain_fold(kGroups, lane, [&](u32 g, u32 stt) { return sh.gtab[g * ns + stt]; }));
        }
        if (lane == 0) {
            chunk_regular[c] = kRegularFew;
            done_list[atomicAdd(done_count, 1u)] = c;
        }
        __syncthreads();
    }
}

template <u32 LB>
__global__ __launch_bounds__(HUFD_DEC_LANES, 8) void dec_sync_true_kernel(
    hufd_tables tb,
    const hufd_chunk_rec *chunk_rec,
    const u8 *d_in,
    const u16 *fn_tab,
    u16 *cp_tab,
    u16 *lane_count,
    u8 *chunk_regular,
    const u32 *chunk_entry,
    hufd_emit_rec *emit_rec,
    const u32 *list,
    const u32 *list_count) {

    few_shared<LB> &sh = *reinterpret_cast<few_shared<LB> *>(dyn_lds);
    const u32 ns = tb.n_states;
    const u32 lane = threadIdx.x;
    const u32 table = lds_offset_of(sh.wlut);
    const row_walk rw(LB, tb.max_bits);
    const u32 n = *list_count;
    if (n == 0) {
        return;
    }
    few_table<LB>(sh, tb, lane);
    if (lane == 0) {
        sh.bad = 0;
    }
    __syncthreads();
    for (u32 k = blockIdx.x; k < n; k += gridDim.x) {
        const u32 c = list[k];
        const u32 centry = chunk_entry[c];
        if (!(centry & 0x100u)) {
            if (lane == 0) {
                chunk_regular[c] = 0;
                emit_rec[c].flags &= ~(HUFD_EMIT_REGULAR_MASK | HUFD_EMIT_MERGED);
            }
            continue;
        }
        const hufd_chunk_rec rec = chunk_rec[c];
        u32 w[kFastRows];
        few_load_words<LB>(w, d_in + rec.src_off + (u64)lane * HUFD_DEC_SUB_BYTES);
// ... 5 lines not shown
            u32 at = centry & 0xFFu;
            bool stops = at >= ns;
            for (u32 l = 0; l < HUFD_DEC_LANES && !stops; ++l) {
                sh.entry_of[l] = at;
                const u32 f = sh.ftab[at * HUFD_DEC_LANES + l];
                stops = (f & 0x8000u) != 0;
                at = (f >> 11) & 15u;
            }
            sh.bad = stops ? 1u : 0u;
        }
        __syncthreads();
        bool ok = sh.bad == 0;
        const u32 entry = ok ? sh.entry_of[lane] : 0u;
        const u32 next_entry = ok && lane + 1 < HUFD_DEC_LANES ? sh.entry_of[lane + 1] : HUFD_NONE32;
        __syncthreads();
        u32 st = rw.state_at(entry, 0), dead_count = 0;
        u32 cp_state[kQuarters - 1] = {0, 0, 0};
        bool dd = false;
#pragma unroll
        for (u32 r = 0; r < kSubWords; ++r) {
            if (r && r % (kSubWords / kQuarters) == 0) {
                cp_state[r / (kSubWords / kQuarters) - 1] = st;
            }
            st = few_row<LB>(st, w[r], w[r + 1], table, rw, dd, dead_count);
        }
        const u32 count = st >> 16, ex = rw.offset_of(st);
        if (ok && (dd || ex >= ns || (next_entry != HUFD_NONE32 && ex != next_entry))) {
            sh.bad = 1;
        }
        __syncthreads();
        const bool good = sh.bad == 0;
        __syncthreads();
        if (good) {
            u16 *cp = cp_tab + (u64)c * kCpRows * HUFD_DEC_LANES + lane;
#pragma unroll
            for (u32 qq = 0; qq + 1 < kQuarters; ++qq) {
                const u32 tail = count - (cp_state[qq] >> 16), bits = rw.offset_of(cp_state[qq]);
                cp[qq * HUFD_DEC_LANES] = (u16)(bits < 16u ? 0x8000u | (bits << 11) | tail : 0u);
            }
            lane_count[(u64)c * HUFD_DEC_LANES + lane] = (u16)count;
            cp[(kQuarters - 1) * HUFD_DEC_LANES] = (u16)((1u << entry) | (ex << 12));
        }
        if (lane == 0) {
            chunk_regular[c] = good ? 1 : 0;
            emit_rec[c].flags = (emit_rec[c].flags & ~(HUFD_EMIT_REGULAR_MASK | HUFD_EMIT_MERGED)) |
                                (good ? (1u << HUFD_EMIT_REGULAR_SHIFT) | HUFD_EMIT_MERGED : 0u);
            sh.bad = 0;
        }
        __syncthreads();
    }
}

__global__ __launch_bounds__(kTailThreads) void dec_sync_tail_kernel(
    hufd_tables tb,
    const hufd_dec_item *items,
    const u32 *chunk_item,
    const u32 *tail_chunks,
    u32 n_tail,
    const u8 *d_in,
    const u8 *chunk_regular,
    const u32 *tail_entry,
    u16 *fn_tab,
    u16 *cp_tab,
    u32 *chunk_fn,
    u16 *lane_count) {

    tail_lds &sh = *reinterpret_cast<tail_lds *>(dyn_lds);
    u16 *lut = reinterpret_cast<u16 *>(dyn_lds + sizeof(tail_lds));
    for (u32 i = threadIdx.x; i < (1u << tb.lut_bits); i += kTailThreads) {
        lut[i] = tb.dec_lut[i];
    }
    __syncthreads();
    const u32 i = blockIdx.x * kTailThreads + threadIdx.x;
    if (i >= n_tail) {
        return;
    }
    const u32 c = tail_chunks[i];
    const u32 kind = chunk_regular[c];
    if (kind != 2 && kind != 3) {
        return;
    }
    const u32 ns = tb.n_states;
    const hufd_dec_item it = items[chunk_item[c]];
    const u64 chunk_off = (u64)(c - it.first_chunk) * HUFD_DEC_CHUNK_BYTES;
    const u64 valid = it.in_len - chunk_off;
    if (kind == 3) {
        u32 *tiny = sh.words[threadIdx.x];
        load_be32_run(tiny, d_in + it.in_off + chunk_off, valid, kTailWords);
        const bool only = c == it.first_chunk;
        for (u32 st = only ? it.first_bit : 0u; st < (only ? it.first_bit + 1u : ns); ++st) {
            u32 stop_pos = 0, stop_why = 0;
            const tail_walk tw = tail_follow(tiny, lut, tb.lut_bits, st, (u32)(valid * 8), 2 * HUFD_DEC_SUB_BITS, nullptr, &stop_pos, &stop_why);
            chunk_fn[(u64)c * ns + st] = wide_pack(true, 0, tw.count[0] + tw.count[1]);
        }
        return;
    }
    const u32 n_full = (u32)((valid - 8u) / HUFD_DEC_SUB_BYTES);
    const u8 *tsrc = d_in + it.in_off + chunk_off + (u64)n_full * HUFD_DEC_SUB_BYTES;
    const u64 tail_bytes = valid - (u64)n_full * HUFD_DEC_SUB_BYTES;
    u32 *words = sh.words[threadIdx.x];
    load_be32_run(words, tsrc, tail_bytes, kTailWords);
    const u32 entry = tail_entry[c];
    const u32 limit = (n_full + 1 < HUFD_DEC_LANES ? 2u : 1u) * HUFD_DEC_SUB_BITS;
    u32 stop_pos = 0, stop_why = 0;
    const tail_walk tw = tail_follow(words, lut, tb.lut_bits, entry, (u32)(tail_bytes * 8), limit, nullptr, &stop_pos, &stop_why);

    u16 *fn_out = fn_tab + (u64)c * ns * HUFD_DEC_LANES;
    u16 *cp = cp_tab + (u64)c * kCpRows * HUFD_DEC_LANES;
    for (u32 k = 0; k < 2; ++k) {
        const u32 lane = n_full + k;
        const bool reached = k == 0 || tw.stop != 0;
        if (lane >= HUFD_DEC_LANES || !reached) {
            break;
        }
        const u32 my_entry = k == 0 ? entry : tw.exit;
        const bool stops_here = tw.stop == k;
        lane_count[(u64)c * HUFD_DEC_LANES + lane] = (u16)tw.count[k];
        fn_out[(u64)my_entry * HUFD_DEC_LANES + lane] =
            stops_here ? fn_pack(true, 0, tw.count[k] & 0x7FFu) : fn_pack(false, tw.exit, tw.count[k] & 0x7FFu);
        cp[(kQuarters - 1) * HUFD_DEC_LANES + lane] = (u16)((1u << my_entry) | ((stops_here ? kExitStop : tw.exit) << 12));
    }
    const bool stops = tw.stop != 2u;
    for (u32 st = 0; st < ns; ++st) {
        const u32 f = chunk_fn[(u64)c * ns + st];
        if (!wide_stop(f)) {
            chunk_fn[(u64)c * ns + st] = wide_pack(stops, stops ? 0u : tw.exit, wide_count(f) + tw.count[0] + tw.count[1]);
        }
    }
}


static uint32_t dec_sync_lds_bytes(const hufd_tables *tb) {
    return kChunkWords * 4 + kGroups * tb->n_states * 4 + (2u << tb->lut_bits);
}

}

using hufk_host::persistent_grid;
using hufk_host::stage_mark;
using hufk_host::current_compute_units;
using hufk_host::kBesideMinChunks;
using hufk_host::decode_launch_state;

hipError_t hufk_host::init_decode_sync(int lds_max) {
    hipError_t e = hipSuccess;
    const void *kernels[] = {
        reinterpret_cast<const void *>(&dec_sync_kernel<8>), reinterpret_cast<const void *>(&dec_sync_kernel<10>),
        reinterpret_cast<const void *>(&dec_sync_kernel<12>)};
    for (const void *k : kernels) {
        if (e == hipSuccess) {
            e = hipFuncSetAttribute(k, hipFuncAttributeMaxDynamicSharedMemorySize, lds_max);
        }
    }
    return e;
}

void hufk_host::decode_sync_stage(const struct hufk_decode_args *a, hipStream_t st, decode_launch_state &s) {
    const uint32_t ns = a->tables.n_states, lb_of_launch = s.lb, sure = s.sure;
    bool few = false;
    const auto sync = ns <= 8 ? dec_sync_kernel<8> : (ns <= 10 ? dec_sync_kernel<10> : dec_sync_kernel<12>);
    u32 *const slow_count = a->counters + HUFK_DEC_COUNT_SLOW, *const few_count = a->counters + HUFK_DEC_COUNT_FEW;
    const bool some_inside = a->n_tail < a->n_chunks;
    const bool guessing = some_inside && !a->quiet;
    u32 *lean_long_list = guessing ? a->emit_list : a->slow_list;
    u32 *lean_long_count = guessing ? a->counters + HUFK_DEC_COUNT_LONG : slow_count;
    const bool folded = hufk_host::tails_are_folded(a);
    const bool beside = !folded && some_inside && a->n_tail && a->side_stream && a->fork_event && a->join_event &&
                        (uint64_t)a->n_tail * 8 <= a->n_chunks && a->n_chunks >= kBesideMinChunks;
    hipStream_t tst = beside ? (hipStream_t)a->side_stream : st;
    if (beside) {
        (void)hipEventRecord((hipEvent_t)a->fork_event, st);
        (void)hipStreamWaitEvent(tst, (hipEvent_t)a->fork_event, 0);
    }
    const uint32_t pack_width = a->tail_lanes + 2u < 16u ? 16u : a->tail_lanes + 2u;
    const bool pack = a->one_chunk_a_workgroup == 0 && a->n_tail_narrow >= kPackMinChunks && pack_width <= HUFD_DEC_LANES / 2;
    const uint32_t pack_slots = HUFD_DEC_LANES / pack_width;
    const uint32_t n_packed = pack ? a->n_tail_narrow : 0u, n_single = a->n_tail - n_packed;
    const u32 *single_chunks = a->tail_chunks + n_packed;
#define HUFK_LAUNCH_SYNC_LEAN(LBV, SUREV)                                                                               \
if (folded) {                                                                                                      \
    hipLaunchKernelGGL(                                                                                            \
        (dec_sync_one_mixed_kernel<LBV, SUREV>), dim3(a->n_chunks + a->n_tail), dim3(HUFD_DEC_LANES),              \
        (uint32_t)sizeof(one_shared<LBV>), st, a->tables, a->chunk_rec, a->tail_chunks, a->n_tail,                  \
        (const u8 *)a->d_in, a->fn_tab, a->cp_tab, a->chunk_fn, a->lane_count, a->chunk_regular, a->tail_entry,     \
        a->slow_list, slow_count, lean_long_list, lean_long_count);                                                \
} else if (n_packed) {                                                                                                    \
    hipLaunchKernelGGL(                                                                                            \
        (dec_sync_pack_kernel<LBV, SUREV>), dim3((n_packed + pack_slots - 1) / pack_slots), dim3(HUFD_DEC_LANES),   \
        (uint32_t)sizeof(pack_shared<LBV>), tst, a->tables, a->chunk_rec, a->tail_chunks, n_packed, pack_width,     \
        (const u8 *)a->d_in, a->fn_tab, a->cp_tab, a->chunk_fn, a->lane_count, a->chunk_regular, a->tail_entry,     \
        lean_long_list, lean_long_count);                                                                          \
}                                                                                                                  \
if (!folded && n_single) {                                                                                         \
    hipLaunchKernelGGL(                                                                                            \
        (dec_sync_one_kernel<LBV, SUREV, true>), dim3(n_single), dim3(HUFD_DEC_LANES),                              \
        (uint32_t)sizeof(one_shared<LBV>), tst, a->tables, a->chunk_rec, single_chunks,                             \
        (const u8 *)a->d_in, a->fn_tab, a->cp_tab, a->chunk_fn, a->lane_count, a->chunk_regular, a->tail_entry,     \
        a->slow_list, slow_count, lean_long_list, lean_long_count);                                                \
}                                                                                                                  \
if (!folded && some_inside) {                                                                                      \
    hipLaunchKernelGGL(                                                                                            \
        (dec_sync_one_kernel<LBV, SUREV, false>), dim3(a->n_chunks), dim3(HUFD_DEC_LANES),                          \
        (uint32_t)sizeof(one_shared<LBV>), st, a->tables, a->chunk_rec, a->tail_chunks,                             \
        (const u8 *)a->d_in, a->fn_tab, a->cp_tab, a->chunk_fn, a->lane_count, a->chunk_regular, a->tail_entry,     \
        a->slow_list, slow_count, lean_long_list, lean_long_count);                                                \
}
    if (lb_of_launch == 10) {
        switch (sure) {
            case 3: HUFK_LAUNCH_SYNC_LEAN(10, 3); break;
            default: HUFK_LAUNCH_SYNC_LEAN(10, 4); break;
        }
    } else {
        HUFK_LAUNCH_SYNC_LEAN(12, 2);
    }
#undef HUFK_LAUNCH_SYNC_LEAN
    if (a->n_tail && !folded) {
        const uint32_t lds = (uint32_t)sizeof(tail_lds) + (2u << a->tables.lut_bits);
        hipLaunchKernelGGL(
            dec_sync_tail_kernel, dim3((a->n_tail + kTailThreads - 1) / kTailThreads), dim3(kTailThreads), lds, tst,
            a->tables, a->items, a->chunk_item, a->tail_chunks, a->n_tail, (const u8 *)a->d_in,
            (const u8 *)a->chunk_regular, (const u32 *)a->tail_entry, a->fn_tab, a->cp_tab, a->chunk_fn, a->lane_count);
    }
    if (beside) {
        (void)hipEventRecord((hipEvent_t)a->join_event, tst);
        (void)hipStreamWaitEvent(st, (hipEvent_t)a->join_event, 0);
    }
    const u32 *long_list = a->slow_list, *long_count = slow_count;
    if (guessing) {
#define HUFK_LAUNCH_SYNC_GUESS(LBV, SUREV)                                                                              \
hipLaunchKernelGGL(                                                                                                \
    (dec_sync_guess_kernel<LBV, SUREV>),                                                                           \
    dim3(persistent_grid(dec_sync_guess_kernel<LBV, SUREV>, HUFD_DEC_LANES, (uint32_t)sizeof(lean_shared<LBV>),     \
                         a->n_chunks)),                                                                            \
    dim3(HUFD_DEC_LANES), (uint32_t)sizeof(lean_shared<LBV>), st, a->tables, a->chunk_rec, (const u8 *)a->d_in,     \
    a->fn_tab, a->cp_tab, a->chunk_fn, a->lane_count, a->chunk_regular, (const u32 *)a->slow_list,                 \
    (const u32 *)slow_count, a->emit_list, a->counters + HUFK_DEC_COUNT_LONG)
        if (lb_of_launch == 10) {
            switch (sure) {
                case 3: HUFK_LAUNCH_SYNC_GUESS(10, 3); break;
                default: HUFK_LAUNCH_SYNC_GUESS(10, 4); break;
            }
        } else {
            HUFK_LAUNCH_SYNC_GUESS(12, 2);
        }
#undef HUFK_LAUNCH_SYNC_GUESS
        long_list = a->emit_list;
        long_count = a->counters + HUFK_DEC_COUNT_LONG;
        if (a->few_walks) {
            few = true;
            if (a->tables.lut_bits <= 10) {
                hipLaunchKernelGGL(
                    (dec_sync_few_kernel<10>),
                    dim3(persistent_grid(dec_sync_few_kernel<10>, HUFD_DEC_LANES, (uint32_t)sizeof(few_shared<10>), a->n_chunks)),
                    dim3(HUFD_DEC_LANES), (uint32_t)sizeof(few_shared<10>), st, a->tables, a->chunk_rec, (const u8 *)a->d_in,
                    a->fn_tab, a->cp_tab, a->chunk_fn, a->chunk_regular, long_list, long_count, a->slow_list, few_count);
            } else {
                hipLaunchKernelGGL(
                    (dec_sync_few_kernel<12>),
                    dim3(persistent_grid(dec_sync_few_kernel<12>, HUFD_DEC_LANES, (uint32_t)sizeof(few_shared<12>), a->n_chunks)),
                    dim3(HUFD_DEC_LANES), (uint32_t)sizeof(few_shared<12>), st, a->tables, a->chunk_rec, (const u8 *)a->d_in,
                    a->fn_tab, a->cp_tab, a->chunk_fn, a->chunk_regular, long_list, long_count, a->slow_list, few_count);
            }
        }
    }
    hipLaunchKernelGGL(
        sync, dim3(persistent_grid(sync, HUFD_DEC_LANES, dec_sync_lds_bytes(&a->tables), a->n_chunks)),
        dim3(HUFD_DEC_LANES), dec_sync_lds_bytes(&a->tables), st, a->tables, a->items, a->chunk_item, a->n_chunks,
        (const u8 *)a->d_in, a->fn_tab, a->cp_tab, a->chunk_fn, a->chunk_regular, long_list, long_count,
        a->counters_self_cleared ? a->counters : (u32 *)nullptr);
    s.few = few;
}

void hufk_host::decode_sync_true_stage(const struct hufk_decode_args *a, hipStream_t st, const decode_launch_state &s) {
    if (!s.few) {
        return;
    }
    if (a->tables.lut_bits <= 10) {
        hipLaunchKernelGGL(
            (dec_sync_true_kernel<10>),
            dim3(persistent_grid(dec_sync_true_kernel<10>, HUFD_DEC_LANES, (uint32_t)sizeof(few_shared<10>), a->n_chunks)),
            dim3(HUFD_DEC_LANES), (uint32_t)sizeof(few_shared<10>), st, a->tables, a->chunk_rec, (const u8 *)a->d_in,
            (const u16 *)a->fn_tab, a->cp_tab, a->lane_count, a->chunk_regular, (const u32 *)a->chunk_entry,
            a->emit_rec, (const u32 *)a->slow_list, (const u32 *)(a->counters + HUFK_DEC_COUNT_FEW));
    } else {
        hipLaunchKernelGGL(
            (dec_sync_true_kernel<12>),
            dim3(persistent_grid(dec_sync_true_kernel<12>, HUFD_DEC_LANES, (uint32_t)sizeof(few_shared<12>), a->n_chunks)),
            dim3(HUFD_DEC_LANES), (uint32_t)sizeof(few_shared<12>), st, a->tables, a->chunk_rec, (const u8 *)a->d_in,
            (const u16 *)a->fn_tab, a->cp_tab, a->lane_count, a->chunk_regular, (const u32 *)a->chunk_entry,
            a->emit_rec, (const u32 *)a->slow_list, (const u32 *)(a->counters + HUFK_DEC_COUNT_FEW));
    }
}
```

### aws-c-compression_amd/csrc/hip/decode_sync_one_body.inc

```

    static_assert(TAIL || !FOLLOW, "only a chunk its stream ends in has an end to follow");
    HUFD_STAMP(0, 0);
    one_shared<LB> &sh = *reinterpret_cast<one_shared<LB> *>(dyn_lds);
    const u32 ns = tb.n_states;
    const u32 lane = threadIdx.x;
    const hufd_chunk_rec rec = chunk_rec[c];
    const u64 valid = rec.valid;
    const u8 *src = d_in + rec.src_off;
    if (!TAIL && valid < (u64)HUFD_DEC_CHUNK_BYTES + 8u) {
        return;
    }
    const u32 n_full = !TAIL ? HUFD_DEC_LANES : (valid >= 8u ? (u32)((valid - 8u) / HUFD_DEC_SUB_BYTES) : 0u);
    const bool active = !TAIL || lane < n_full;
    if (TAIL && n_full == 0 && tb.lut_bits <= HUFD_DEC_MAX_LUT_BITS) {
        if (lane == 0) {
            chunk_regular[c] = 3;
        }
        if (FOLLOW) {
            u16 *lut = reinterpret_cast<u16 *>(sh.wlut);
            for (u32 i = lane; i < (1u << tb.lut_bits); i += HUFD_DEC_LANES) {
                lut[i] = tb.dec_lut[i];
            }
            __syncthreads();
            if (lane == 0) {
                u32 *tiny = sh.tiny;
                load_be32_run(tiny, src, valid, kTailWords);
                const bool only = rec.entry_bit != HUFD_NONE32;
                for (u32 st = only ? rec.entry_bit : 0u; st < (only ? rec.entry_bit + 1u : ns); ++st) {
                    u32 stop_pos = 0, stop_why = 0;
                    const tail_walk tw = tail_follow(tiny, lut, tb.lut_bits, st, (u32)(valid * 8), 2 * HUFD_DEC_SUB_BITS, nullptr, &stop_pos, &stop_why);
                    chunk_fn[(u64)c * ns + st] = wide_pack(true, 0, tw.count[0] + tw.count[1]);
                }
            }
        }
        return;
    }
    const one_walk ow(LB);
    u32 table = lds_offset_of(sh.wlut);
    opaque(table);
    const bool eligible = n_full >= 1 && tb.lut_bits <= LB && tb.max_bits <= HUFD_DEC_MAX_LUT_BITS &&
                          row_walk(LB, tb.max_bits).sure >= SURE && (table & ((4u << LB) - 1u)) == 0;
    if (!eligible) {
        if (lane == 0) {
            chunk_regular[c] = 0;
            long_list[atomicAdd(long_count, 1u)] = c;
        }
        return;
    }
    u16 *cp = cp_tab + (u64)c * kCpRows * HUFD_DEC_LANES + lane;
    constexpr u32 kLutPerLane = (1u << LB) / HUFD_DEC_LANES, kLutBatch = 4;
    const auto table_share = [&](u32 j0) {
        u32 lut_raw[kLutBatch];
#pragma unroll
        for (u32 j = 0; j < kLutBatch; ++j) {
            lut_raw[j] = tb.dec_lut[(lane + (j0 + j) * HUFD_DEC_LANES) >> (LB - tb.lut_bits)];
        }
#pragma unroll
        for (u32 j = 0; j < kLutBatch; ++j) {
            sh.wlut[lane + (j0 + j) * HUFD_DEC_LANES] = one_walk::entry_of(lut_raw[j] & 0xFFu);
        }
    };
    if (TAIL && lane >= kWave && (lane & ~(kWave - 1)) >= n_full) {
#pragma unroll
        for (u32 j0 = 0; j0 < kLutPerLane; j0 += kLutBatch) {
            table_share(j0);
        }
        if (!FOLLOW || (lane != n_full && lane != n_full + 1)) {
#pragma unroll
            for (u32 qq = 0; qq + 1 < kQuarters; ++qq) {
                cp[qq * HUFD_DEC_LANES] = 0;
            }
            lane_count[(u64)c * HUFD_DEC_LANES + lane] = 0;
            cp[(kQuarters - 1) * HUFD_DEC_LANES] = (u16)(kExitStop << 12);
        }
        return;
    }
    u32 w[kFastRows];
    {
        const u32 mine = active ? lane : 0u;
        const unaligned_uint4 *line = reinterpret_cast<const unaligned_uint4 *>(src + (u64)mine * HUFD_DEC_SUB_BYTES);
#pragma unroll
        for (u32 q = 0; q < kSubWords / 4; ++q) {
            const unaligned_uint4 v = line[q];
            w[4 * q + 0] = v.x;
            w[4 * q + 1] = v.y;
            w[4 * q + 2] = v.z;
            w[4 * q + 3] = v.w;
        }
        w[kSubWords] = reinterpret_cast<const unaligned_u32 *>(src + (u64)(mine + 1) * HUFD_DEC_SUB_BYTES)->x;
    }
#pragma unroll
    for (u32 j0 = 0; j0 < kLutPerLane; j0 += kLutBatch) {
        table_share(j0);
    }
    if (lane == 0) {
        sh.bad = 0;
        sh.decided0 = 0;
        sh.moved = 0;
        sh.bad_mine = 0;
#pragma unroll
        for (u32 wv = 0; wv < HUFD_DEC_LANES / kWave; ++wv) {
            sh.wave_sum[wv] = 0;
        }
    }
    {
        u32 behind = __builtin_bswap32(w[kFastRows - 1]);
// ... 113 lines not shown
            }
        }
        if (active && lane && !hopeless && !met && entry < ns) {
            met = true;
            h_at = st;
            r_at = last;
            meet_row = kSubWords;
            ref_exit = ow.offset_of(st);
            sh.exit_state[lane] = ref_exit;
            sh.moved = 1;
        }
        if (active && lane) {
            ok_mine = !hopeless && met && entry < ns && ref_exit < ns && one_walk::dead_of(h_at) == 0 &&
                      one_walk::dead_of(last) == one_walk::dead_of(r_at);
            count = one_walk::count_of(h_at) + one_walk::count_of(last) - one_walk::count_of(r_at);
        }
    }

    HUFD_STAMP(0, 7);
    {
        const u32 wsum0 = wave_sum(lane ? count : 0u);
        if ((lane & (kWave - 1)) == 0) {
            sh.wave_sum[lane / kWave] = wsum0;
        }
        if (!ok) {
            sh.bad = 1;
        }
        if (!ok_mine) {
            sh.bad_mine = 1;
        }
    }
    __syncthreads();
    const bool stay = sh.moved != 0;
    auto lane_records = [&]() {
        if (active) {
#pragma unroll
            for (u32 qq = 0; qq + 1 < kQuarters; ++qq) {
                const u32 boundary = (qq + 1) * (kSubWords / kQuarters);
                bool have = boundary >= meet_row;
                const u32 at_boundary = kept_get(kOneRecs + qq);
                u32 tail = one_walk::count_of(last) - one_walk::count_of(at_boundary), bits = ow.offset_of(at_boundary);
                if (!have && lane != 0) {
                    tail = count - one_walk::count_of(head_cp[qq]);
                    bits = ow.offset_of(head_cp[qq]);
                    have = true;
                }
                cp[qq * HUFD_DEC_LANES] = (u16)(have ? 0x8000u | (bits << 11) | tail : 0u);
            }
        } else if (!FOLLOW || (lane != n_full && lane != n_full + 1)) {
#pragma unroll
            for (u32 qq = 0; qq + 1 < kQuarters; ++qq) {
                cp[qq * HUFD_DEC_LANES] = 0;
            }
            lane_count[(u64)c * HUFD_DEC_LANES + lane] = 0;
            cp[(kQuarters - 1) * HUFD_DEC_LANES] = (u16)(kExitStop << 12);
        }
        if (TAIL && lane + 1 == n_full) {
            tail_entry[c] = ref_exit;
        }
    };
    if (!stay && lane >= kWave) {
        if (!sh.bad && !sh.bad_mine) {
            lane_records();
            if (active) {
                lane_count[(u64)c * HUFD_DEC_LANES + lane] = (u16)count;
                cp[(kQuarters - 1) * HUFD_DEC_LANES] = (u16)((1u << entry) | (ref_exit << 12));
            }
        }
        return;
    }
    u32 cand_count = 0, cand_dead = 0, meet_row0 = 0, ref_count0 = 0;
    bool cand_reached = false;
    u64 cand_alive = 0;
    if (lane < kWave) {
        constexpr u32 kTwin = kWave - 1;
        const bool twin = lane == kTwin;
        const u32 last0 = sh.last0;
        u32 st = ow.state_at(lane < ns ? lane : 0u);
        const u32 only = rec.entry_bit;
        bool dd = only == HUFD_NONE32 ? lane >= ns : lane != only, met = false;
        u32 c_at = 0, r_at = 0;
        u32 at0 = st, latest = 0;
        u32 hi = sh.sub0[0];
        for (u32 r = 0; !hopeless; ++r) {
            const u32 there = __shfl(st, kTwin);
            const bool now = !twin && !dd && !met && ((st ^ there) & one_walk::kPos) == 0 && one_walk::dead_of(last0) == one_walk::dead_of(there);
            if (now) {
                met = true;
                c_at = st;
                r_at = there;
            }
            if (__any(now)) {
                at0 = there;
                latest = r;
            }
            if (__all(dd || met || twin) || r == kSubWords) {
                break;
            }
            const u32 lo = sh.sub0[r + 1];
            if (twin) {
// ... 100 lines not shown
                    }
                    fine = ref_exit < ns && one_walk::dead_of(h_at) == 0 && one_walk::dead_of(last) == one_walk::dead_of(r_at);
                    count = one_walk::count_of(h_at) + one_walk::count_of(last) - one_walk::count_of(r_at);
                }
                ok_mine = fine;
            }
            __syncthreads();
            if (!sh.moved) {
                break;
            }
        }
        if (round == kRounds || !ok_mine) {
            sh.bad = 1;
        }
        const u32 wsum_now = wave_sum(lane ? count : 0u);
        if ((lane & (kWave - 1)) == 0) {
            sh.wave_sum[lane / kWave] = wsum_now;
        }
        __syncthreads();
    }
    if (sh.bad) {
        if (lane == 0) {
            chunk_regular[c] = 0;
            if (TAIL || !sh.decided0) {
                long_list[atomicAdd(long_count, 1u)] = c;
            } else {
                slow_list[atomicAdd(slow_count, 1u)] = c;
            }
        }
        return;
    }

    u16 *fn_out = fn_tab + (u64)c * ns * HUFD_DEC_LANES;
    lane_records();
    if (active) {
        const u32 total = lane ? count : ref_count0;
        lane_count[(u64)c * HUFD_DEC_LANES + lane] = (u16)total;
        cp[(kQuarters - 1) * HUFD_DEC_LANES] = (u16)((lane ? 1u << entry : (u32)cand_alive) | (ref_exit << 12));
    }
    if (lane == 0) {
        chunk_regular[c] = TAIL ? 2 : 1;
    }
    u32 follow_exit = 0, follow_count = 0, follow_stop = 2;
    if (FOLLOW && lane < kWave) {
        u16 *lut = reinterpret_cast<u16 *>(sh.wlut);
        u32 *words = sh.wlut + (1u << LB) / 2;
        const u32 entry_t = sh.exit_state[n_full - 1];
        wave_step();
        for (u32 i = lane; i < (1u << tb.lut_bits); i += kWave) {
            lut[i] = tb.dec_lut[i];
        }
        tail_walk tw = {{0, 0}, 0, 2};
        if (lane == 0) {
            const u8 *tsrc = src + (u64)n_full * HUFD_DEC_SUB_BYTES;
            const u64 tail_bytes = valid - (u64)n_full * HUFD_DEC_SUB_BYTES;
            load_be32_run(words, tsrc, tail_bytes, kTailWords);
        }
        wave_step();
        if (lane == 0) {
            const u64 tail_bytes = valid - (u64)n_full * HUFD_DEC_SUB_BYTES;
            const u32 limit = (n_full + 1 < HUFD_DEC_LANES ? 2u : 1u) * HUFD_DEC_SUB_BITS;
            u32 stop_pos = 0, stop_why = 0;
            tw = tail_follow(words, lut, tb.lut_bits, entry_t, (u32)(tail_bytes * 8), limit, nullptr, &stop_pos, &stop_why);
            for (u32 k = 0; k < 2; ++k) {
                const u32 ln = n_full + k;
                if (ln >= HUFD_DEC_LANES) {
                    break;
                }
                u16 *cpl = cp_tab + (u64)c * kCpRows * HUFD_DEC_LANES + ln;
                const bool reached = k == 0 || tw.stop != 0;
#pragma unroll
                for (u32 qq = 0; qq + 1 < kQuarters; ++qq) {
                    cpl[qq * HUFD_DEC_LANES] = 0;
                }
                if (reached) {
                    const u32 my_entry = k == 0 ? entry_t : tw.exit;
                    const bool stops_here = tw.stop == k;
                    lane_count[(u64)c * HUFD_DEC_LANES + ln] = (u16)tw.count[k];
                    fn_out[(u64)my_entry * HUFD_DEC_LANES + ln] =
                        stops_here ? fn_pack(true, 0, tw.count[k] & 0x7FFu) : fn_pack(false, tw.exit, tw.count[k] & 0x7FFu);
                    cpl[(kQuarters - 1) * HUFD_DEC_LANES] = (u16)((1u << my_entry) | ((stops_here ? kExitStop : tw.exit) << 12));
                } else {
                    lane_count[(u64)c * HUFD_DEC_LANES + ln] = 0;
                    cpl[(kQuarters - 1) * HUFD_DEC_LANES] = (u16)(kExitStop << 12);
                }
            }
        }
        follow_exit = __shfl(tw.exit, 0);
        follow_count = __shfl(tw.count[0] + tw.count[1], 0);
        follow_stop = __shfl(tw.stop, 0);
    }
    if (lane < ns) {
        u32 rest = 0;
#pragma unroll
        for (u32 wv = 0; wv < HUFD_DEC_LANES / kWave; ++wv) {
            rest += sh.wave_sum[wv];
        }
        const u32 first_exit = sh.exit_state[0];
        const u32 last_exit = sh.exit_state[HUFD_DEC_LANES - 1];
        fn_out[(u64)lane * HUFD_DEC_LANES] =
            cand_reached ? fn_pack(false, first_exit, cand_count & 0x7FFu) : fn_pack(true, 0, cand_dead);
        const bool stops = follow_stop != 2u;
        chunk_fn[(u64)c * ns + lane] =
            cand_reached ? (FOLLOW ? wide_pack(stops, stops ? 0u : follow_exit, cand_count + rest + follow_count)
                                   : wide_pack(false, TAIL ? 0u : last_exit, cand_count + rest))
                         : wide_pack(true, 0, cand_dead);
    }
    HUFD_STAMP(0, 6);
```

### aws-c-compression_amd/csrc/hip/device_types.h

```cpp
#ifndef HUFFMAN_AMD_DEVICE_TYPES_H
#define HUFFMAN_AMD_DEVICE_TYPES_H
#include <stdint.h>

#define HUFD_ENC_SEG_BYTES 16384u
#define HUFD_ENC_THREADS 256u
#define HUFD_ENC_BLOCK_BYTES 4096u
#define HUFD_ENC_BLOCK_MAX_BYTES 16384u
#define HUFD_ENC_TINY_BYTES 512u

#define HUFD_DEC_SUB_BYTES 128u
#define HUFD_DEC_SUB_BITS (HUFD_DEC_SUB_BYTES * 8u)
#define HUFD_DEC_LANES 256u
#define HUFD_DEC_CHUNK_BYTES (HUFD_DEC_SUB_BYTES * HUFD_DEC_LANES)
#define HUFD_TINY_MANY_BYTES 2048u
#define HUFD_ENC_SOLO_BYTES 4096u
#define HUFD_ENC_SOLO_MANY_BYTES HUFD_ENC_SEG_BYTES
#define HUFD_ENC_SOLO_MANY_ITEMS 256u
#define HUFD_ENC_TINY_WAVE_BYTES 1024u
#define HUFD_ENC_TINY_PER_BYTE 18u
#define HUFD_ENC_TINY_PER_BYTE_ONE_PASS 100u
#define HUFD_DEC_TINY_PER_BYTE 40u
#define HUFD_TINY_FEW_BYTES 128u
#define HUFD_DEC_MAX_STATES 16u
#define HUFD_DEC_CP_ROWS 4u
// ... 137 lines not shown
    uint64_t total_symbols;
};

struct hufd_dec_result {
    uint64_t total_symbols;
    uint64_t stop_bit;
    uint64_t cap_bit;
    uint32_t stop_kind;
    uint32_t reserved;
};

struct hufd_chunk_rec {
    uint64_t src_off;
    uint64_t out_off;
    uint64_t out_cap;
    uint32_t valid;
    uint32_t item;
    uint32_t entry_bit;
    uint32_t reserved;
};

#define HUFD_EMIT_STATE_MASK 0xFFu
#define HUFD_EMIT_REACHED 0x100u
#define HUFD_EMIT_REGULAR_SHIFT 9u
#define HUFD_EMIT_REGULAR_MASK (7u << HUFD_EMIT_REGULAR_SHIFT)
#define HUFD_EMIT_MERGED 0x1000u
#define HUFD_EMIT_STOPS 0x2000u
struct hufd_emit_rec {
    uint32_t flags;
    uint32_t symbols;
    uint64_t base;
};

#define HUFD_ITEMS_DEVICE_ARRAY 0u
#define HUFD_ITEMS_STRIDED 1u
#define HUFD_ITEMS_FROM_ENCODE 2u
#define HUFD_ITEMS_PACKED_INPUT 3u
#define HUFD_ITEMS_BLOCK_RANGES 4u
#define HUFD_ITEMS_SYMBOL_RANGES 5u
#define HUFD_ITEMS_ITEM_BLOCK_RANGES 6u
#define HUFD_ITEMS_ITEM_SYMBOL_RANGES 7u
#define HUFD_ITEMS_PACKED_STORED_INPUT 8u
struct hufd_block_range {
    uint64_t first_block;
    uint64_t block_count;
    uint64_t out_offset;
};
struct hufd_symbol_range {
    uint64_t first_symbol;
    uint64_t symbol_count;
    uint64_t out_offset;
};
struct hufd_item_block_range {
    uint64_t item;
    uint64_t first_block;
    uint64_t block_count;
    uint64_t out_offset;
};
struct hufd_item_symbol_range {
    uint64_t item;
    uint64_t first_symbol;
    uint64_t symbol_count;
    uint64_t out_offset;
};
#define HUFD_NO_BIT 0xFFFFFFFFFFFFFFFFull
struct hufd_item_source {
// ... 54 lines not shown
```

### aws-c-compression_amd/csrc/hip/huffman_kernels.h

```cpp
#ifndef HUFFMAN_AMD_KERNELS_H
#define HUFFMAN_AMD_KERNELS_H
#include <stdint.h>

#include "device_types.h"

#ifdef __cplusplus
extern "C" {
#endif

struct hufk_encode_args {
    struct hufd_tables tables;
    const struct hufd_enc_item *items;
    uint32_t n_items;
    const struct hufd_enc_seg *segs;
    uint32_t n_segs;
    const uint32_t *large_items;
    uint32_t n_large;
    const uint32_t *tiny_items;
    uint32_t n_tiny;
    const uint32_t *solo_items;
    uint32_t n_solo;
    uint32_t length_only;
    const void *d_in;
    void *d_out;
// ... 26 lines not shown
#define HUFK_DEC_COUNT_FEW 2u
#define HUFK_DEC_COUNT_EMIT 3u
#define HUFK_DEC_COUNT_DENSE 4u
#define HUFK_DEC_COUNTERS 8u

struct hufk_decode_args {
    struct hufd_tables tables;
    const struct hufd_dec_item *items;
    uint32_t n_items;
    const uint32_t *chunk_item;
    uint32_t n_chunks;
    const uint32_t *tail_chunks;
    uint32_t n_tail;
    const uint32_t *tiny_items;
    uint32_t n_tiny;
    const uint32_t *deep_items;
    uint32_t n_deep;
    const struct hufk_wide_item *wide;
    uint32_t n_wide;
    uint64_t wide_from;
    void *wide_block;
    uint32_t wide_fails;
    uint32_t few_walks;
    const uint32_t *fixed_blocks;
    uint32_t n_fixed_blocks;
    const uint32_t *large_items;
    uint32_t n_large;
    const uint32_t *runs;
    uint32_t n_runs;
    uint32_t *run_fn;
    const void *d_in;
    void *d_out;
    uint16_t *fn_tab;
    uint16_t *cp_tab;
    uint32_t *chunk_fn;
    uint32_t *slow_list;
    uint32_t *emit_list;
    uint32_t *dense_list;
    uint32_t *counters;
    uint32_t counters_self_cleared;
    uint32_t *summary;
    uint32_t quiet;
    uint16_t *lane_count;
    uint8_t *chunk_regular;
    uint32_t *tail_entry;
    uint32_t *chunk_entry;
    uint64_t *chunk_base;
    struct hufd_emit_rec *emit_rec;
    const struct hufd_chunk_rec *chunk_rec;
    void *side_stream;
    void *fork_event;
    void *join_event;
    struct hufd_dec_item_state *states;
    struct hufd_dec_result *results;
    uint32_t tail_stage_bytes;
    uint32_t tail_lanes;
    uint32_t tail_wide_lanes;
    uint32_t n_tail_narrow;
    uint32_t one_chunk_a_workgroup;
    uint32_t tails_apart;
    void **stage_events;
    const uint64_t *stored_rec;
    const uint64_t *stored_tile_first;
    uint64_t stored_tiles;
};

int hufk_init(void);

uint32_t hufk_enc_image_words(uint32_t max_bits);
int hufk_encode_one_pass_applies(const struct hufd_tables *tables);
uint64_t hufk_encode_zero_bytes(uint32_t n_segs, uint32_t n_items);
int hufk_encode_launch(const struct hufk_encode_args *args, void *stream);
int hufk_decode_launch(const struct hufk_decode_args *args, void *stream);
struct hufk_decode_pack {
    uint32_t tile_items;
    uint32_t tail_stage_bytes;
// ... 167 lines not shown
```

### aws-c-compression_amd/csrc/host/engine.c

```c
#include "engine.h"
#include "arena.h"

#include <aws/compression/huffman_amd_batch_index.h>
#include <aws/compression/huffman_amd_packed_index.h>
#include <aws/compression/huffman_amd_build.h>
#include <aws/compression/huffman_amd_fit.h>
#include <aws/compression/huffman_amd_index.h>
#include <aws/compression/huffman_amd_packed.h>
#include <aws/compression/huffman_amd_plan_counts.h>
#include <aws/compression/huffman_amd_planes.h>
#include <aws/compression/huffman_amd_planes_delta.h>
#include <aws/compression/huffman_amd_ranges.h>
#include <aws/compression/huffman_amd_stored.h>
#include <aws/compression/huffman_amd_stored_index.h>

#include <assert.h>
#include <stdlib.h>
#include <string.h>

static uint32_t s_testing_encode_road = 0, s_testing_decode_road = 0;
static uint64_t s_testing_per_byte[2] = {0, 0};

void aws_huffman_amd_testing_set_encode_road(uint32_t flags) {
    __atomic_store_n(&s_testing_encode_road, flags, __ATOMIC_RELAXED);
// ... 1480 lines not shown
}

int aws_huffman_amd_encode_plan_results(
    struct aws_huffman_amd_encode_plan *p,
    struct aws_huffman_amd_encode_result *results,
    void *stream) {

    struct hufd_enc_result *raw = malloc((p->n_items ? p->n_items : 1) * sizeof(*raw));
    if (!raw) {
        return aws_raise_error(AWS_ERROR_OOM);
    }
    if (aws_huffman_amd_encode_plan_raw_results(p, raw, stream)) {
        free(raw);
        return AWS_OP_ERR;
    }
    for (uint32_t i = 0; i < p->n_items; ++i) {
        aws_huffman_amd_encode_result_from_raw(&raw[i], &results[i]);
    }
    free(raw);
    return AWS_OP_SUCCESS;
}


#define DEC_SUMMARY_BYTES 256u
#define DEC_PLAN_ARRAYS(X, ci, cc, cl, cr, ns)                                                                            \
    X(d_items, (ci) * sizeof(struct hufd_dec_item))                                                                    \
    X(d_chunk_item, (cc) * sizeof(uint32_t))                                                                           \
    X(d_tail, (ci) * 2 * sizeof(uint32_t))                                                                             \
    X(d_tiny, (ci) * sizeof(uint32_t))                                                                                 \
    X(d_large, (cl) * 2 * sizeof(uint32_t))                                                                            \
    X(d_runs, (cr) * 2 * sizeof(uint32_t))                                                                             \
    X(d_run_fn, (cr) * (ns) * sizeof(uint32_t))                                                                        \
    X(d_fn_tab, (cc) * (ns) * HUFD_DEC_LANES * sizeof(uint16_t))                                                       \
    X(d_cp_tab, (cc) * HUFD_DEC_CP_ROWS * HUFD_DEC_LANES * sizeof(uint16_t))                                           \
    X(d_chunk_fn, (cc) * (ns) * sizeof(uint32_t))                                                                      \
    X(d_slow_list, ((cc) + 1) * sizeof(uint32_t))                                         \
    X(d_emit_list, ((cc) + 1) * sizeof(uint32_t))                                                                      \
    X(d_dense_list, ((cc) + 1) * sizeof(uint32_t))                                                                     \
    X(d_counters, HUFK_DEC_COUNTERS * sizeof(uint32_t))                                                                \
    X(d_lane_count, (cc) * HUFD_DEC_LANES * sizeof(uint16_t))                                                          \
    X(d_chunk_regular, (cc))                                                                                           \
    X(d_tail_entry, (cc) * sizeof(uint32_t))                                                                           \
    X(d_chunk_entry, (cc) * sizeof(uint32_t))                                                                          \
    X(d_chunk_base, (cc) * sizeof(uint64_t))                                                                           \
    X(d_emit_rec, (cc) * sizeof(struct hufd_emit_rec))                                                                 \
    X(d_chunk_rec, (cc) * sizeof(struct hufd_chunk_rec))                                                               \
    X(d_states, (ci) * sizeof(struct hufd_dec_item_state))                                                             \
                                                                                 \
    X(d_summary, DEC_SUMMARY_BYTES)                                                                                    \
    X(d_results, (ci) * sizeof(struct hufd_dec_result))

static void dec_plan_release_device(struct aws_huffman_amd_decode_plan *p) {
    hufs_free(p->d_arena);
    p->d_arena = NULL;
#define DEC_FORGET(name, bytes) p->name = NULL;
    DEC_PLAN_ARRAYS(DEC_FORGET, 0, 0, 0, 0, 0)
#undef DEC_FORGET
    p->cap_items = p->cap_chunks = p->cap_large = p->cap_runs = 0;
}

static bool dec_item_is_tiny(const struct aws_huffman_amd_decode_item *it, uint64_t limit) {
    return it->in_len > 0 && it->in_len <= limit;
}

static uint64_t dec_tiny_limit(const struct aws_huffman_amd_decode_item *items, size_t n_items, struct item_stats *st) {
    static const uint64_t classes[2] = {HUFD_DEC_COOP_BYTES, HUFD_DEC_TINY_BYTES};
    uint64_t count[2] = {0, 0}, longest[2] = {0, 0};
    st->shortest = UINT64_MAX;
    st->longest = 0;
    st->worst_bits = 0;
    for (size_t i = 0; i < n_items; ++i) {
        const uint64_t len = items[i].in_len;
        st->shortest = len < st->shortest ? len : st->shortest;
        st->longest = len > st->longest ? len : st->longest;
        st->worst_bits = items[i].first_bit > st->worst_bits ? items[i].first_bit : st->worst_bits;
        for (int c = 0; c < 2; ++c) {
            if (len <= classes[c]) {
                ++count[c];
                longest[c] = len > longest[c] ? len : longest[c];
            }
        }
    }
    for (int c = 0; c < 2; ++c) {
// ... 836 lines not shown
    void **stage_events) {

    struct hufk_decode_args a;
    memset(&a, 0, sizeof(a));
    a.tables = p->engine->tables;
    a.items = p->d_items;
    a.n_items = p->n_items;
    a.chunk_item = p->d_chunk_item;
    a.n_chunks = p->n_chunks;
    a.tail_chunks = p->d_tail;
    a.n_tail = p->n_tail;
    a.tail_stage_bytes = p->tail_stage_bytes;
    a.tail_lanes = p->tail_lanes;
    a.tail_wide_lanes = p->tail_wide_lanes;
    a.n_tail_narrow = p->n_tail_narrow;
    a.deep_items = p->d_tiny + (p->n_items - p->n_deep);
    a.n_deep = p->n_deep;
    a.wide = p->h_wide;
    a.n_wide = p->n_wide;
    a.wide_from = p->wide_from;
    a.wide_block = p->d_wide_block;
    a.fixed_blocks = p->d_fixed;
    a.n_fixed_blocks = p->n_fixed;
    a.tiny_items = p->d_tiny;
    a.n_tiny = p->n_tiny;
    a.large_items = p->d_large;
    a.n_large = p->n_large;
    a.runs = p->d_runs;
    a.n_runs = p->n_runs;
    a.run_fn = p->d_run_fn;
    a.d_in = device_input;
    a.d_out = device_output;
    a.fn_tab = p->d_fn_tab;
    a.cp_tab = p->d_cp_tab;
    a.chunk_fn = p->d_chunk_fn;
    a.slow_list = p->d_slow_list + 1;
    a.emit_list = p->d_emit_list + 1;
    a.dense_list = p->d_dense_list + 1;
    a.counters = p->d_counters;
    a.counters_self_cleared = 1;
    a.summary = p->d_summary;
    a.quiet = p->quiet && !(testing_decode_road() & AWS_HUFFMAN_AMD_TEST_DECODE_ALL_KERNELS);
    a.lane_count = p->d_lane_count;
    a.chunk_regular = p->d_chunk_regular;
    a.tail_entry = p->d_tail_entry;
    a.chunk_entry = p->d_chunk_entry;
    a.chunk_base = p->d_chunk_base;
    a.emit_rec = p->d_emit_rec;
    a.chunk_rec = p->d_chunk_rec;
    a.side_stream = p->engine->side_stream;
    a.fork_event = p->engine->fork_event;
    a.join_event = p->engine->join_event;
    a.states = p->d_states;
    a.results = p->d_results;
    {
        const uint32_t road = testing_decode_road();
        a.one_chunk_a_workgroup = (road & AWS_HUFFMAN_AMD_TEST_DECODE_ONE_CHUNK_A_WORKGROUP) != 0;
        a.tails_apart = (road & AWS_HUFFMAN_AMD_TEST_DECODE_TAILS_APART) != 0;
        a.wide_fails = road & AWS_HUFFMAN_AMD_TEST_DECODE_WIDE_FN_FAILS ? 2u : (road & AWS_HUFFMAN_AMD_TEST_DECODE_WIDE_FAILS ? 1u : 0u);
        a.few_walks = road & AWS_HUFFMAN_AMD_TEST_DECODE_LONG_WAY ? 0u : 1u;
    }
    a.stage_events = stage_events;
    if (p->stored_ranges) {
        a.stored_rec = p->d_stored_rec;
        a.stored_tile_first = p->d_stored_tile_first;
        a.stored_tiles = p->stored_tiles;
    }
    *args = a;
}

int aws_huffman_amd_decode_plan_launch_staged(
    struct aws_huffman_amd_decode_plan *p,
    const void *device_input,
    void *device_output,
    void *stream,
    void **stage_events) {
// ... 1617 lines not shown
```

### aws-c-compression_amd/csrc/host/engine.h

```cpp
#ifndef HUFFMAN_AMD_ENGINE_H
#define HUFFMAN_AMD_ENGINE_H
#include <aws/compression/huffman_amd.h>

#include <pthread.h>

#include "../hip/device_types.h"
#include "../hip/hip_shim.h"
#include "../hip/huffman_kernels.h"

struct aws_huffman_amd_engine {
    int device;
    void *stream;
    void *side_stream;
    void *fork_event, *join_event;

    struct aws_huffman_symbol_coder *coder;
    void *key_encode;
    void *key_decode;
    void *key_userdata;
    uint64_t fingerprint;

    uint64_t enc_table[256];
    uint16_t *dec_lut_host;
    uint32_t *deep_lut_host;
// ... 70 lines not shown
    struct hufd_enc_item *d_packed_items;
    uint64_t *d_pack_tile_sums;
    uint64_t *d_pack_summary;
    size_t cap_packed_items, cap_pack_tiles;
    bool packed;
    bool packed_sized;
    bool stored;
    void *d_block_index_arena;
    uint64_t *d_block_index_tile_first;
    uint64_t *d_block_index_tile_sums;
    uint64_t *d_block_index_summary;
    size_t cap_block_index_items, cap_block_index_tiles;
    bool block_indexed;
};

struct aws_huffman_amd_decode_plan {
    struct aws_huffman_amd_engine *engine;
    uint32_t n_items, n_chunks, n_large, n_runs, n_tail, n_tiny, n_deep;
    uint32_t tail_stage_bytes;
    uint32_t tail_lanes;
    uint32_t tail_wide_lanes;
    uint32_t n_tail_narrow;
    size_t cap_items, cap_chunks, cap_large, cap_runs;
    struct aws_huffman_amd_decode_item *h_items;
    void *d_arena;
    struct hufd_dec_item *d_items;
    uint32_t *d_chunk_item;
    uint32_t *d_tiny;
    uint32_t *d_tail;
    uint32_t *d_large;
    uint32_t *d_runs;
    uint32_t *d_run_fn;
    uint16_t *d_fn_tab;
    uint16_t *d_cp_tab;
    uint32_t *d_chunk_fn;
    uint32_t *d_slow_list;
    uint32_t *d_emit_list;
    uint32_t *d_dense_list;
    uint32_t *d_counters;
    uint32_t launches_with_chunks;
    uint16_t *d_lane_count;
    uint8_t *d_chunk_regular;
    uint32_t *d_tail_entry;
    uint32_t *d_chunk_entry;
    uint64_t *d_chunk_base;
    struct hufd_emit_rec *d_emit_rec;
    struct hufd_chunk_rec *d_chunk_rec;
    struct aws_huffman_amd_plan_stats stats;
    void *d_plan_scratch;
    size_t cap_plan_scratch;
    void *done_event;
    bool done_on_engine_stream;
    bool unkeepable;
    uint64_t *d_range_bits;
    size_t cap_range_bits;
    bool chained;
    struct hufd_dec_item_state *d_states;
    uint32_t *d_summary;
    struct hufd_dec_result *d_results;
    bool quiet;
    struct hufk_wide_item *h_wide;
    uint32_t n_wide;
    uint64_t wide_from;
    void *d_wide_block;
    size_t cap_wide_block;
    uint32_t *d_fixed;
    uint32_t n_fixed;
    size_t cap_fixed;
    void *d_packed_arena;
    struct hufd_dec_item *d_packed_items;
    struct hufd_chunk_rec *d_packed_chunk_rec;
    uint64_t *d_pack_tile_sums;
    uint64_t *d_pack_summary;
    size_t cap_packed_items, cap_packed_chunks, cap_pack_tiles;
// ... 45 lines not shown
```

Measured before the change: 671.4.

## Pack per-lane checkpoints, merged word and count into one 16-byte record

Replaces the separate row-major cp_tab (four u16 rows per chunk) and lane_count arrays with an array of 16-byte per-lane records holding three checkpoints, the merged exit word and the symbol count. Producers write each lane's data with one vector store, and emit kernels read it with one vector load instead of several scattered u16 loads. The intent is fewer memory transactions on the decode scan-to-emit handoff. In exchange the footprint grows from 10 to 16 bytes per lane, and some paths still do extra scalar record reads for the neighbouring lane's merged word.

```diff
diff --git a/aws-c-compression_amd/csrc/hip/decode_common.hpp b/aws-c-compression_amd/csrc/hip/decode_common.hpp
--- a/aws-c-compression_amd/csrc/hip/decode_common.hpp
+++ b/aws-c-compression_amd/csrc/hip/decode_common.hpp
@@ -17,6 +17,42 @@
 constexpr u32 kEmitThreads = HUFD_DEC_LANES * kQuarters;
 constexpr u32 kExitStop = 15, kExitNoRef = 14;
 constexpr u8 kRegularFew = 4;
+
+static_assert(sizeof(hufd_lane_rec) == 16 && alignof(hufd_lane_rec) == 16, "a record is one 16-byte load or store");
+static_assert(kQuarters - 1 == 3 && kCpRows == kQuarters, "three checkpoints and the merged word a record");
+
+__device__ __forceinline__ uint4 lane_rec_load(const hufd_lane_rec *lane_rec, u32 c, u32 lane) {
+    return *reinterpret_cast<const uint4 *>(lane_rec + (u64)c * HUFD_DEC_LANES + lane);
+}
+__device__ __forceinline__ void lane_rec_store(hufd_lane_rec *lane_rec, u32 c, u32 lane, const uint4 &v) {
+    *reinterpret_cast<uint4 *>(lane_rec + (u64)c * HUFD_DEC_LANES + lane) = v;
+}
+__device__ __forceinline__ uint4 lane_rec_pack(u32 cp0, u32 cp1, u32 cp2, u32 merged, u32 count) {
+    uint4 v;
+    v.x = (cp0 & 0xFFFFu) | (cp1 << 16);
+    v.y = (cp2 & 0xFFFFu) | (merged << 16);
+    v.z = count & 0xFFFFu;
+    v.w = 0;
+    return v;
+}
+__device__ __forceinline__ uint4 lane_rec_unreached() {
+    return lane_rec_pack(0, 0, 0, kExitStop << 12, 0);
+}
+__device__ __forceinline__ u32 lane_rec_cp(const uint4 &v, u32 qq) {
+    return qq == 0 ? v.x & 0xFFFFu : (qq == 1 ? v.x >> 16 : v.y & 0xFFFFu);
+}
+__device__ __forceinline__ u32 lane_rec_merged(const uint4 &v) {
+    return v.y >> 16;
+}
+__device__ __forceinline__ u32 lane_rec_count(const uint4 &v) {
+    return v.z & 0xFFFFu;
+}
+__device__ __forceinline__ u32 lane_rec_merged(const hufd_lane_rec *lane_rec, u32 c, u32 lane) {
+    return lane_rec[(u64)c * HUFD_DEC_LANES + lane].merged;
+}
+__device__ __forceinline__ u32 lane_rec_count(const hufd_lane_rec *lane_rec, u32 c, u32 lane) {
+    return lane_rec[(u64)c * HUFD_DEC_LANES + lane].count;
+}
 
 __device__ __forceinline__ u16 fn_pack(bool stop, u32 exit_state, u32 count) {
     return (u16)((stop ? 0x8000u : 0u) | (exit_state << 11) | count);
diff --git a/aws-c-compression_amd/csrc/hip/decode_emit_kernels.hip b/aws-c-compression_amd/csrc/hip/decode_emit_kernels.hip
--- a/aws-c-compression_amd/csrc/hip/decode_emit_kernels.hip
+++ b/aws-c-compression_amd/csrc/hip/decode_emit_kernels.hip
@@ -11,8 +11,7 @@
     const u8 *d_in,
     u8 *d_out,
     const u16 *fn_tab,
-    const u16 *cp_tab,
-    const u16 *lane_count_tab,
+    const hufd_lane_rec *lane_rec,
     const u8 *chunk_regular,
     const u32 *chunk_entry,
     const u64 *chunk_base,
@@ -46,7 +45,10 @@
     const u64 cbase = chunk_base[c];
 
     HUFD_STAMP(1, 0);
-    const u16 my_cp = cp_tab[(u64)c * kCpRows * HUFD_DEC_LANES + t];
+    uint4 my_rec = lane_rec_unreached();
+    if (t < HUFD_DEC_LANES) {
+        my_rec = lane_rec_load(lane_rec, c, t);
+    }
     u16 my_fn[(HUFD_DEC_MAX_STATES * HUFD_DEC_LANES + kEmitThreads - 1) / kEmitThreads];
 #pragma unroll
     for (u32 j = 0; j < sizeof(my_fn) / sizeof(my_fn[0]); ++j) {
@@ -55,7 +57,13 @@
     }
     chunk_load<kEmitThreads>(timg, d_in + it.in_off + chunk_off, valid);
     lut_load<kEmitThreads>(lut, tb);
-    cpt[t] = my_cp;
+    if (t < HUFD_DEC_LANES) {
+#pragma unroll
+        for (u32 qq = 0; qq + 1 < kQuarters; ++qq) {
+            cpt[qq * HUFD_DEC_LANES + t] = (u16)lane_rec_cp(my_rec, qq);
+        }
+        cpt[(kQuarters - 1) * HUFD_DEC_LANES + t] = (u16)lane_rec_merged(my_rec);
+    }
 #pragma unroll
     for (u32 j = 0; j < sizeof(my_fn) / sizeof(my_fn[0]); ++j) {
         const u32 i = t + j * kEmitThreads;
@@ -92,7 +100,7 @@
         }
         lane_state = (fits && lane_reached) ? lane_state : 0;
         lane_count = !lane_reached ? 0u
-                     : (t != 0 && chunk_regular[c] != 0) ? (u32)lane_count_tab[(u64)c * HUFD_DEC_LANES + t]
+                     : (t != 0 && chunk_regular[c] != 0) ? lane_rec_count(my_rec)
                                                          : (u32)(ftab[lane_state * HUFD_DEC_LANES + t] & 0x7FFu);
         lane_incl = wave_inclusive_sum(lane_count, t & (kWave - 1));
         if ((t & (kWave - 1)) == kWave - 1) {
@@ -266,8 +274,7 @@
     const u8 *d_in,
     u8 *d_out,
     const u16 *fn_tab,
-    const u16 *cp_tab,
-    const u16 *lane_count_tab,
+    const hufd_lane_rec *lane_rec,
     const u8 *chunk_regular,
     const u32 *chunk_entry,
     const u64 *chunk_base,
@@ -291,7 +298,7 @@
     }
     const u32 n = list ? *list_count : n_chunks;
     for (u32 i = blockIdx.x; i < n; i += gridDim.x) {
-        dec_emit_chunk(tb, items, chunk_item, d_in, d_out, fn_tab, cp_tab, lane_count_tab, chunk_regular, chunk_entry, chunk_base, results, list ? list[i] : i);
+        dec_emit_chunk(tb, items, chunk_item, d_in, d_out, fn_tab, lane_rec, chunk_regular, chunk_entry, chunk_base, results, list ? list[i] : i);
         __syncthreads();
     }
 }
@@ -324,8 +331,7 @@
     const hufd_chunk_rec *chunk_rec,
     const u8 *d_in,
     u8 *d_out,
-    const u16 *cp_tab,
-    const u16 *lane_count,
+    const hufd_lane_rec *lane_rec,
     const hufd_emit_rec *emit_rec,
     hufd_dec_result *results,
     u32 *slow_list,
@@ -359,8 +365,6 @@
     }
     const u32 n_full = !TAIL ? HUFD_DEC_LANES : (valid >= 8u ? (u32)((valid - 8u) / HUFD_DEC_SUB_BYTES) : 0u);
     const u64 cbase = erec.base;
-    const u16 *cpt = cp_tab + (u64)c * kCpRows * HUFD_DEC_LANES;
-    const u32 merged_row = (kQuarters - 1) * HUFD_DEC_LANES;
     const u32 chunk_symbols = erec.symbols;
     const u32 regular = (erec.flags & HUFD_EMIT_REGULAR_MASK) >> HUFD_EMIT_REGULAR_SHIFT;
     if (TAIL && regular == 3) {
@@ -387,6 +391,8 @@
     u32 w[kEmitChains][kRows + 1];
     u32 my_cp[kEmitChains], next_cp[kEmitChains], entry_state[kEmitChains], cnt[kEmitChains];
     bool whole[kEmitChains];
+    const uint4 recs[kEmitChains] = {lane_rec_load(lane_rec, c, lanes[0]), lane_rec_load(lane_rec, c, lanes[1])};
+    const u32 entry_front = lanes[0] ? (u32)__builtin_ctz((lane_rec_merged(recs[0]) & 0xFFFu) | 0x1000u) : s0;
 #pragma unroll
     for (u32 ch = 0; ch < kEmitChains; ++ch) {
         sub[ch] = d_in + rec.src_off + (u64)lanes[ch] * HUFD_DEC_SUB_BYTES;
@@ -407,10 +413,11 @@
             }
             w[ch][kRows] = __builtin_bswap32(reinterpret_cast<const unaligned_u32 *>(sub[ch] + (q + 1) * kRows * 4)->x);
         }
-        my_cp[ch] = q ? cpt[(q - 1) * HUFD_DEC_LANES + lanes[ch]] : 0u;
-        next_cp[ch] = q + 1 < kQuarters ? cpt[q * HUFD_DEC_LANES + lanes[ch]] : 0u;
-        entry_state[ch] = lanes[ch] ? (u32)(cpt[merged_row + lanes[ch] - 1] >> 12) : s0;
-        cnt[ch] = lane_count[(u64)c * HUFD_DEC_LANES + lanes[ch]];
+        const u64 cps = ((u64)recs[ch].y << 32) | recs[ch].x;
+        my_cp[ch] = q ? (u32)(cps >> (16u * (q - 1u))) & 0xFFFFu : 0u;
+        next_cp[ch] = q + 1 < kQuarters ? (u32)(cps >> (16u * q)) & 0xFFFFu : 0u;
+        entry_state[ch] = ch ? lane_rec_merged(recs[0]) >> 12 : entry_front;
+        cnt[ch] = lane_rec_count(recs[ch]);
     }
 #pragma unroll
     for (u32 j = 0; j < kLutPerThread; ++j) {
@@ -431,7 +438,7 @@
     }
     u32 incl = 0, own_cnt = 0;
     if (t < HUFD_DEC_LANES) {
-        own_cnt = t < n_full + 2 ? lane_count[(u64)c * HUFD_DEC_LANES + t] : 0u;
+        own_cnt = t < n_full + 2 ? lane_rec_count(lane_rec, c, t) : 0u;
         incl = wave_inclusive_sum(t ? own_cnt : 0u, t & (kWave - 1));
         if ((t & (kWave - 1)) == kWave - 1) {
             sh.wave_tot[t / kWave] = incl;
@@ -517,7 +524,8 @@
     }
     }
     if (extend) {
-        const u32 extend_end = (cpt[1 * HUFD_DEC_LANES] & 0x8000u) ? 2 * kRows : ((cpt[2 * HUFD_DEC_LANES] & 0x8000u) ? 3 * kRows : 4 * kRows);
+        const uint4 rec0 = lane_rec_load(lane_rec, c, 0);
+        const u32 extend_end = (lane_rec_cp(rec0, 1) & 0x8000u) ? 2 * kRows : ((lane_rec_cp(rec0, 2) & 0x8000u) ? 3 * kRows : 4 * kRows);
         u32 hi = w[0][kRows];
         for (u32 r = kRows; r < extend_end; ++r) {
             const u32 lo = __builtin_bswap32(reinterpret_cast<const unaligned_u32 *>(d_in + rec.src_off + (r + 1) * 4)->x);
@@ -564,8 +572,7 @@
     const u32 *tail_chunks,
     const u8 *d_in,
     u8 *d_out,
-    const u16 *cp_tab,
-    const u16 *lane_count,
+    const hufd_lane_rec *lane_rec,
     const hufd_emit_rec *emit_rec,
     hufd_dec_result *results,
     u32 *slow_list,
@@ -574,7 +581,7 @@
     u32 *dense_count,
     u32 stage_limit ) {
     dec_emit_fast_chunk<LB, TAIL, SURE>(
-        TAIL ? tail_chunks[blockIdx.x] : blockIdx.x, tb, chunk_rec, d_in, d_out, cp_tab, lane_count, emit_rec, results, slow_list,
+        TAIL ? tail_chunks[blockIdx.x] : blockIdx.x, tb, chunk_rec, d_in, d_out, lane_rec, emit_rec, results, slow_list,
         slow_count, dense_list, dense_count, stage_limit);
 }
 
@@ -586,8 +593,7 @@
     const hufd_chunk_rec *chunk_rec,
     const u8 *d_in,
     u8 *d_out,
-    const u16 *cp_tab,
-    const u16 *lane_count,
+    const hufd_lane_rec *lane_rec,
     const hufd_emit_rec *emit_rec,
     hufd_dec_result *results,
     u32 *slow_list,
@@ -600,7 +606,7 @@
             continue;
         }
         dec_emit_fast_chunk<LB, false, SURE>(
-            big_list[k], tb, chunk_rec, d_in, d_out, cp_tab, lane_count, emit_rec, results, slow_list, slow_count, slow_list,
+            big_list[k], tb, chunk_rec, d_in, d_out, lane_rec, emit_rec, results, slow_list, slow_count, slow_list,
             slow_count, kEmitBigStage);
         __syncthreads();
     }
@@ -631,8 +637,7 @@
     u32 slots,
     const u8 *d_in,
     u8 *d_out,
-    const u16 *cp_tab,
-    const u16 *lane_count,
+    const hufd_lane_rec *lane_rec,
     const u8 *chunk_regular,
     const u32 *chunk_fn,
     const u32 *chunk_entry,
@@ -664,13 +669,11 @@
     const u64 valid = rec.valid;
     const u32 n_full = valid >= 8u ? (u32)((valid - 8u) / HUFD_DEC_SUB_BYTES) : 0u;
     const u64 cbase = have ? chunk_base[c] : 0;
-    const u16 *cpt = cp_tab + (u64)c * kCpRows * HUFD_DEC_LANES;
-    const u32 merged_row = (kQuarters - 1) * HUFD_DEC_LANES;
     const u32 f0 = have ? chunk_fn[(u64)c * ns + s0] : 0u;
     const u32 chunk_symbols = wide_count(f0);
     const u32 regular = have ? chunk_regular[c] : 0u;
     const bool wanted = have && (centry & 0x100u) != 0 && regular != 3;
-    const bool fits = wanted && regular == 2 && ((cpt[merged_row] >> s0) & 1u) != 0 && cbase + chunk_symbols <= rec.out_cap;
+    const bool fits = wanted && regular == 2 && ((lane_rec_merged(lane_rec, c, 0) >> s0) & 1u) != 0 && cbase + chunk_symbols <= rec.out_cap;
     const bool fast = fits && chunk_symbols + 16 <= stage_limit && n_full + 2 <= slot_lanes &&
                       (lds_offset_of(sh.wlut) & ((4u << LB) - 1u)) == 0 && SURE <= row_walk(LB, tb.max_bits).sure;
     if (tt == 0 && slot < kPackMaxSlots) {
@@ -685,6 +688,7 @@
     u32 w[kEmitChains][kRows + 1];
     u32 my_cp[kEmitChains], next_cp[kEmitChains], entry_state[kEmitChains], cnt[kEmitChains];
     bool whole[kEmitChains];
+    uint4 recs[kEmitChains] = {lane_rec_unreached(), lane_rec_unreached()};
 #pragma unroll
     for (u32 ch = 0; ch < kEmitChains; ++ch) {
         whole[ch] = fast && lanes[ch] < n_full;
@@ -705,10 +709,12 @@
                 w[ch][4 * j + 3] = __builtin_bswap32(v.w);
             }
             w[ch][kRows] = __builtin_bswap32(reinterpret_cast<const unaligned_u32 *>(sub + (q + 1) * kRows * 4)->x);
-            my_cp[ch] = q ? cpt[(q - 1) * HUFD_DEC_LANES + lanes[ch]] : 0u;
-            next_cp[ch] = q + 1 < kQuarters ? cpt[q * HUFD_DEC_LANES + lanes[ch]] : 0u;
-            entry_state[ch] = lanes[ch] ? (u32)(cpt[merged_row + lanes[ch] - 1] >> 12) : s0;
-            cnt[ch] = lane_count[(u64)c * HUFD_DEC_LANES + lanes[ch]];
+            recs[ch] = lane_rec_load(lane_rec, c, lanes[ch]);
+            const u64 cps = ((u64)recs[ch].y << 32) | recs[ch].x;
+            my_cp[ch] = q ? (u32)(cps >> (16u * (q - 1u))) & 0xFFFFu : 0u;
+            next_cp[ch] = q + 1 < kQuarters ? (u32)(cps >> (16u * q)) & 0xFFFFu : 0u;
+            entry_state[ch] = ch ? lane_rec_merged(recs[0]) >> 12 : (lanes[0] ? lane_rec_merged(lane_rec, c, lanes[0] - 1) >> 12 : s0);
+            cnt[ch] = lane_rec_count(recs[ch]);
         }
     }
 #pragma unroll
@@ -726,7 +732,7 @@
     if (t < HUFD_DEC_LANES) {
         const u32 sa = t / slot_lanes, la = t % slot_lanes;
         const u32 ca = sa < slots && sa < kPackMaxSlots ? sh.slot_chunk[sa] : HUFD_NONE32;
-        own = ca != HUFD_NONE32 && la != 0 && la < sh.slot_full[sa] + 2 && la < HUFD_DEC_LANES ? lane_count[(u64)ca * HUFD_DEC_LANES + la] : 0u;
+        own = ca != HUFD_NONE32 && la != 0 && la < sh.slot_full[sa] + 2 && la < HUFD_DEC_LANES ? lane_rec_count(lane_rec, ca, la) : 0u;
         incl = wave_inclusive_sum(own, t & (kWave - 1));
         if ((t & (kWave - 1)) == kWave - 1) {
             sh.wave_tot[t / kWave] = incl;
@@ -809,7 +815,8 @@
         }
     }
     if (extend) {
-        const u32 extend_end = (cpt[1 * HUFD_DEC_LANES] & 0x8000u) ? 2 * kRows : ((cpt[2 * HUFD_DEC_LANES] & 0x8000u) ? 3 * kRows : 4 * kRows);
+        const uint4 rec0 = lane_rec_load(lane_rec, c, 0);
+        const u32 extend_end = (lane_rec_cp(rec0, 1) & 0x8000u) ? 2 * kRows : ((lane_rec_cp(rec0, 2) & 0x8000u) ? 3 * kRows : 4 * kRows);
         u32 hi = w[0][kRows];
         for (u32 r = kRows; r < extend_end; ++r) {
             const u32 lo = __builtin_bswap32(reinterpret_cast<const unaligned_u32 *>(d_in + rec.src_off + (r + 1) * 4)->x);
@@ -854,8 +861,7 @@
     u32 n_tail,
     const u8 *d_in,
     u8 *d_out,
-    const u16 *cp_tab,
-    const u16 *lane_count,
+    const hufd_lane_rec *lane_rec,
     const u8 *chunk_regular,
     const u32 *chunk_fn,
     const u32 *chunk_entry,
@@ -913,18 +919,16 @@
         }
         return;
     }
-    const u16 *cpt = cp_tab + (u64)c * kCpRows * HUFD_DEC_LANES;
-    const u32 merged_row = (kQuarters - 1) * HUFD_DEC_LANES;
     const u32 f0 = chunk_fn[(u64)c * ns + s0];
     const u32 chunk_symbols = wide_count(f0);
-    if (((cpt[merged_row] >> s0) & 1u) == 0 || cbase + chunk_symbols > it.out_cap || chunk_symbols + 16 > stage_limit) {
+    if (((lane_rec_merged(lane_rec, c, 0) >> s0) & 1u) == 0 || cbase + chunk_symbols > it.out_cap || chunk_symbols + 16 > stage_limit) {
         return;
     }
     const u32 n_full = (u32)((valid - 8u) / HUFD_DEC_SUB_BYTES);
     const u32 first = n_full, second = n_full + 1;
-    const u32 n_first = lane_count[(u64)c * HUFD_DEC_LANES + first];
-    const u32 n_second = second < HUFD_DEC_LANES ? lane_count[(u64)c * HUFD_DEC_LANES + second] : 0u;
-    const u32 entry = cpt[merged_row + first - 1] >> 12;
+    const u32 n_first = lane_rec_count(lane_rec, c, first);
+    const u32 n_second = second < HUFD_DEC_LANES ? lane_rec_count(lane_rec, c, second) : 0u;
+    const u32 entry = lane_rec_merged(lane_rec, c, first - 1) >> 12;
     const u8 *tsrc = d_in + it.in_off + chunk_off + (u64)n_full * HUFD_DEC_SUB_BYTES;
     const u64 tail_bytes = valid - (u64)n_full * HUFD_DEC_SUB_BYTES;
     u32 *words = sh.words[threadIdx.x];
@@ -976,7 +980,7 @@
 hipLaunchKernelGGL(                                                                                                \
     (dec_emit_fast_kernel<LBV, TAILV, SUREV>), dim3(GRID), dim3((TAILV) && (LBV) == 10 ? tail_block : kEmitFastThreads), \
     emit_lds_bytes<LBV>(TAILV ? tail_stage : HUFD_DEC_STAGE_BYTES), STREAMV, a->tables, a->chunk_rec,              \
-    emit_single_chunks, (const u8 *)a->d_in, (u8 *)a->d_out, (const u16 *)a->cp_tab, (const u16 *)a->lane_count,   \
+    emit_single_chunks, (const u8 *)a->d_in, (u8 *)a->d_out, (const hufd_lane_rec *)a->lane_rec,                   \
     (const hufd_emit_rec *)a->emit_rec, a->results, a->emit_list, emit_count,                                      \
     !TAILV && big ? a->dense_list : a->emit_list, !TAILV && big ? dense_count : emit_count,                  \
     TAILV ? tail_stage : HUFD_DEC_STAGE_BYTES)
@@ -1014,8 +1018,8 @@
 hipLaunchKernelGGL(                                                                                                \
     (dec_emit_pack_kernel<LBV, SUREV>), dim3((e_packed + epack_slots - 1) / epack_slots), dim3(kEmitFastThreads),    \
     (uint32_t)sizeof(emit_pack_shared<LBV>) + epack_slots * epack_stage, tst, a->tables, a->chunk_rec, a->tail_chunks, \
-    e_packed, epack_width, epack_slots, (const u8 *)a->d_in, (u8 *)a->d_out, (const u16 *)a->cp_tab,               \
-    (const u16 *)a->lane_count, (const u8 *)a->chunk_regular, (const u32 *)a->chunk_fn, (const u32 *)a->chunk_entry, \
+    e_packed, epack_width, epack_slots, (const u8 *)a->d_in, (u8 *)a->d_out, (const hufd_lane_rec *)a->lane_rec,   \
+    (const u8 *)a->chunk_regular, (const u32 *)a->chunk_fn, (const u32 *)a->chunk_entry,                           \
     (const u64 *)a->chunk_base, a->emit_list, emit_count, tail_stage)
     if (e_packed) {
         if (lb_of_launch == 10) {
@@ -1055,7 +1059,7 @@
         hipLaunchKernelGGL(
             dec_emit_tail_kernel, dim3((a->n_tail + kTailThreads - 1) / kTailThreads), dim3(kTailThreads), lds, ends_st,
             a->tables, a->items, a->chunk_item, a->tail_chunks, a->n_tail, (const u8 *)a->d_in, (u8 *)a->d_out,
-            (const u16 *)a->cp_tab, (const u16 *)a->lane_count, (const u8 *)a->chunk_regular,
+            (const hufd_lane_rec *)a->lane_rec, (const u8 *)a->chunk_regular,
             (const u32 *)a->chunk_fn, (const u32 *)a->chunk_entry, (const u64 *)a->chunk_base, a->results, tail_stage);
     }
     if (have_side) {
@@ -1069,7 +1073,7 @@
         (dec_emit_big_kernel<LBV, SUREV>),                                                                         \
         dim3(persistent_grid(dec_emit_big_kernel<LBV, SUREV>, kEmitFastThreads, lds, a->n_chunks)),                 \
         dim3(kEmitFastThreads), lds, st, a->tables, a->chunk_rec, (const u8 *)a->d_in, (u8 *)a->d_out,             \
-        (const u16 *)a->cp_tab, (const u16 *)a->lane_count, (const hufd_emit_rec *)a->emit_rec, a->results,        \
+        (const hufd_lane_rec *)a->lane_rec, (const hufd_emit_rec *)a->emit_rec, a->results,                        \
         a->emit_list, emit_count,                                                                               \
         (const u32 *)a->dense_list, (const u32 *)dense_count);                                                  \
 } while (0)
@@ -1087,7 +1091,7 @@
         dec_emit_kernel,
         dim3(persistent_grid(dec_emit_kernel, kEmitThreads, dec_emit_lds_bytes(&a->tables), a->n_chunks)),
         dim3(kEmitThreads), dec_emit_lds_bytes(&a->tables), st, a->tables, a->items, a->chunk_item, a->n_chunks,
-        (const u8 *)a->d_in, (u8 *)a->d_out, a->fn_tab, a->cp_tab, (const u16 *)a->lane_count,
+        (const u8 *)a->d_in, (u8 *)a->d_out, a->fn_tab, (const hufd_lane_rec *)a->lane_rec,
         (const u8 *)a->chunk_regular, a->chunk_entry, a->chunk_base, a->results, (const u32 *)a->emit_list,
         (const u32 *)emit_count, a->counters, a->summary, a->counters_self_cleared);
 }
diff --git a/aws-c-compression_amd/csrc/hip/decode_launch.hip b/aws-c-compression_amd/csrc/hip/decode_launch.hip
--- a/aws-c-compression_amd/csrc/hip/decode_launch.hip
+++ b/aws-c-compression_amd/csrc/hip/decode_launch.hip
@@ -24,14 +24,14 @@
 }
 
 __device__ __forceinline__ hufd_emit_rec emit_rec_of(
-    u32 c, u32 state, bool stopped, u64 total, u32 f, const u8 *chunk_regular, const u16 *cp_tab) {
+    u32 c, u32 state, bool stopped, u64 total, u32 f, const u8 *chunk_regular, const hufd_lane_rec *lane_rec) {
     hufd_emit_rec r;
     r.flags = state & HUFD_EMIT_STATE_MASK;
     r.symbols = 0;
     r.base = total;
     if (!stopped) {
         const u32 regular = chunk_regular[c];
-        const u32 merged = cp_tab[((u64)c * kCpRows + (kQuarters - 1)) * HUFD_DEC_LANES];
+        const u32 merged = lane_rec_merged(lane_rec, c, 0);
         r.flags |= HUFD_EMIT_REACHED | (regular << HUFD_EMIT_REGULAR_SHIFT) | (((merged >> state) & 1u) ? HUFD_EMIT_MERGED : 0u) |
                    (wide_stop(f) ? HUFD_EMIT_STOPS : 0u);
         r.symbols = wide_count(f);
@@ -45,7 +45,7 @@
     u32 ns,
     const u32 *chunk_fn,
     const u8 *chunk_regular,
-    const u16 *cp_tab,
+    const hufd_lane_rec *lane_rec,
     u32 *chunk_entry,
     u64 *chunk_base,
     hufd_emit_rec *emit_rec,
@@ -71,7 +71,7 @@
         chunk_entry[c] = entry_pack(state, !stopped);
         chunk_base[c] = total;
         const u32 f = stopped ? 0u : chunk_fn[(u64)c * ns + state];
-        emit_rec[c] = emit_rec_of(c, state, stopped, total, f, chunk_regular, cp_tab);
+        emit_rec[c] = emit_rec_of(c, state, stopped, total, f, chunk_regular, lane_rec);
         if (!stopped) {
             total += wide_count(f);
             stopped = wide_stop(f);
@@ -178,7 +178,7 @@
     const u32 *chunk_fn,
     const u32 *run_fn,
     const u8 *chunk_regular,
-    const u16 *cp_tab,
+    const hufd_lane_rec *lane_rec,
     u32 *chunk_entry,
     u64 *chunk_base,
     hufd_emit_rec *emit_rec,
@@ -239,7 +239,7 @@
         const u32 centry = chunk_entry[c];
         const u32 state = centry & 0xFFu;
         const bool stopped = !(centry & 0x100u);
-        emit_rec[c] = emit_rec_of(c, state, stopped, chunk_base[c], stopped ? 0u : fn[q * ns + state], chunk_regular, cp_tab);
+        emit_rec[c] = emit_rec_of(c, state, stopped, chunk_base[c], stopped ? 0u : fn[q * ns + state], chunk_regular, lane_rec);
     }
 }
 
@@ -496,7 +496,7 @@
     if (a->n_tiny != a->n_items && a->n_large != a->n_items) {
         hipLaunchKernelGGL(
             dec_scan_small_kernel, dim3((a->n_items + 255) / 256), dim3(256), 0, st, a->items, a->n_items, ns, a->chunk_fn,
-            (const u8 *)a->chunk_regular, (const u16 *)a->cp_tab, a->chunk_entry, a->chunk_base, a->emit_rec, a->states, a->results);
+            (const u8 *)a->chunk_regular, (const hufd_lane_rec *)a->lane_rec, a->chunk_entry, a->chunk_base, a->emit_rec, a->states, a->results);
     }
     hufk_host::decode_items_stage(items_pass, st);
     if (a->n_large) {
@@ -505,7 +505,7 @@
             dec_scan_runs_kernel, dim3(a->n_runs), dim3(256), lds, st, a->items, a->runs, ns, a->chunk_fn, a->run_fn);
         hipLaunchKernelGGL(
             dec_scan_apply_kernel, dim3(a->n_runs), dim3(256), scan_apply_lds_bytes(ns), st, a->items, a->runs, ns, a->chunk_fn,
-            (const u32 *)a->run_fn, (const u8 *)a->chunk_regular, (const u16 *)a->cp_tab, a->chunk_entry, a->chunk_base,
+            (const u32 *)a->run_fn, (const u8 *)a->chunk_regular, (const hufd_lane_rec *)a->lane_rec, a->chunk_entry, a->chunk_base,
             a->emit_rec, a->states, a->results);
     }
     hufk_host::decode_sync_true_stage(a, st, state);
diff --git a/aws-c-compression_amd/csrc/hip/decode_sync_kernels.hip b/aws-c-compression_amd/csrc/hip/decode_sync_kernels.hip
--- a/aws-c-compression_amd/csrc/hip/decode_sync_kernels.hip
+++ b/aws-c-compression_amd/csrc/hip/decode_sync_kernels.hip
@@ -11,7 +11,7 @@
     const u32 *chunk_item,
     const u8 *d_in,
     u16 *fn_tab,
-    u16 *cp_tab,
+    hufd_lane_rec *lane_rec,
     u32 *chunk_fn,
     u8 *chunk_regular,
     u32 c) {
@@ -141,12 +141,11 @@
         }
     }
     {
-        u16 *cp = cp_tab + (u64)c * kCpRows * HUFD_DEC_LANES + lane;
+        u32 cps[kQuarters - 1];
 #pragma unroll
         for (u32 qq = 0; qq + 1 < kQuarters; ++qq) {
             const u32 tail = ref_steps - cp_steps[qq];
-            cp[qq * HUFD_DEC_LANES] =
-                (u16)(cp_ok[qq] ? 0x8000u | ((cp_pos[qq] - (qq + 1) * kQuarterBits) << 11) | tail : 0u);
+            cps[qq] = cp_ok[qq] ? 0x8000u | ((cp_pos[qq] - (qq + 1) * kQuarterBits) << 11) | tail : 0u;
         }
         u32 merged = 0;
 #pragma unroll
@@ -154,7 +153,7 @@
             merged |= (have_ref && pos[s] != kDead) ? 1u << s : 0u;
         }
         const u32 common = have_ref ? (ref_stop ? kExitStop : ref_exit) : kExitNoRef;
-        cp[(kQuarters - 1) * HUFD_DEC_LANES] = (u16)(merged | (common << 12));
+        lane_rec_store(lane_rec, c, lane, lane_rec_pack(cps[0], cps[1], cps[2], merged | (common << 12), 0));
     }
     __syncthreads();
 
@@ -180,7 +179,7 @@
     u32 n_chunks,
     const u8 *d_in,
     u16 *fn_tab,
-    u16 *cp_tab,
+    hufd_lane_rec *lane_rec,
     u32 *chunk_fn,
     u8 *chunk_regular,
     const u32 *list,
@@ -196,7 +195,7 @@
         if (list && chunk_regular[c] == kRegularFew) {
             continue;
         }
-        dec_sync_chunk<NS>(tb, items, chunk_item, d_in, fn_tab, cp_tab, chunk_fn, chunk_regular, c);
+        dec_sync_chunk<NS>(tb, items, chunk_item, d_in, fn_tab, lane_rec, chunk_fn, chunk_regular, c);
         __syncthreads();
     }
 }
@@ -292,9 +291,8 @@
     const u32 *tail_chunks,
     const u8 *d_in,
     u16 *fn_tab,
-    u16 *cp_tab,
+    hufd_lane_rec *lane_rec,
     u32 *chunk_fn,
-    u16 *lane_count,
     u8 *chunk_regular,
     u32 *tail_entry,
     u32 *slow_list,
@@ -314,9 +312,8 @@
     u32 n_tail,
     const u8 *d_in,
     u16 *fn_tab,
-    u16 *cp_tab,
+    hufd_lane_rec *lane_rec,
     u32 *chunk_fn,
-    u16 *lane_count,
     u8 *chunk_regular,
     u32 *tail_entry,
     u32 *slow_list,
@@ -359,9 +356,8 @@
     u32 width,
     const u8 *d_in,
     u16 *fn_tab,
-    u16 *cp_tab,
+    hufd_lane_rec *lane_rec,
     u32 *chunk_fn,
-    u16 *lane_count,
     u8 *chunk_regular,
     u32 *tail_entry,
     u32 *long_list,
@@ -412,7 +408,6 @@
         mine = false;
     }
     const bool active = mine && lane < n_full;
-    u16 *cp = cp_tab + (u64)c * kCpRows * HUFD_DEC_LANES;
     u32 w[kFastRows];
     {
         const u32 from = active ? lane : 0u;
@@ -546,7 +541,7 @@
     }
 
     if (active) {
-        u16 *mcp = cp + lane;
+        u32 cps[kQuarters - 1];
 #pragma unroll
         for (u32 qq = 0; qq + 1 < kQuarters; ++qq) {
             const bool usable = (qq + 1) * (kSubWords / kQuarters) >= meet_row;
@@ -557,19 +552,12 @@
                 bits = rw.offset_of(head_cp);
                 have_cp = true;
             }
-            mcp[qq * HUFD_DEC_LANES] = (u16)(have_cp ? 0x8000u | (bits << 11) | tail : 0u);
-        }
-        lane_count[(u64)c * HUFD_DEC_LANES + lane] = (u16)(lane ? count : ref_count);
-        mcp[(kQuarters - 1) * HUFD_DEC_LANES] = (u16)((lane ? 1u << entry : sh.alive[slot]) | (ref_exit << 12));
+            cps[qq] = have_cp ? 0x8000u | (bits << 11) | tail : 0u;
+        }
+        lane_rec_store(lane_rec, c, lane, lane_rec_pack(cps[0], cps[1], cps[2], (lane ? 1u << entry : sh.alive[slot]) | (ref_exit << 12), lane ? count : ref_count));
     }
     if (lane < 2 && n_full + lane < HUFD_DEC_LANES) {
-        const u32 l = n_full + lane;
-#pragma unroll
-        for (u32 qq = 0; qq + 1 < kQuarters; ++qq) {
-            cp[qq * HUFD_DEC_LANES + l] = 0;
-        }
-        lane_count[(u64)c * HUFD_DEC_LANES + l] = 0;
-        cp[(kQuarters - 1) * HUFD_DEC_LANES + l] = (u16)(kExitStop << 12);
+        lane_rec_store(lane_rec, c, n_full + lane, lane_rec_unreached());
     }
     if (lane + 1 == n_full) {
         tail_entry[c] = ref_exit;
@@ -599,9 +587,8 @@
     const hufd_chunk_rec *chunk_rec,
     const u8 *d_in,
     u16 *fn_tab,
-    u16 *cp_tab,
+    hufd_lane_rec *lane_rec,
     u32 *chunk_fn,
-    u16 *lane_count,
     u8 *chunk_regular,
     u32 *slow_list,
     u32 *slow_count) {
@@ -809,15 +796,14 @@
     u32 lane_o = lane;
     opaque(lane_o);
     u16 *fn_out = fn_tab + (u64)c * ns * HUFD_DEC_LANES;
-    u16 *cp = cp_tab + (u64)c * kCpRows * HUFD_DEC_LANES + lane_o;
+    u32 cps[kQuarters - 1];
 #pragma unroll
     for (u32 qq = 0; qq + 1 < kQuarters; ++qq) {
         const bool have = lane != 0 || (qq + 1) * (kSubWords / kQuarters) >= meet_row;
         const u32 tail = count - (cp_state[qq] >> 16), bits = rw.offset_of(cp_state[qq]);
-        cp[qq * HUFD_DEC_LANES] = (u16)(have ? 0x8000u | (bits << 11) | tail : 0u);
-    }
-    lane_count[(u64)c * HUFD_DEC_LANES + lane_o] = (u16)count;
-    cp[(kQuarters - 1) * HUFD_DEC_LANES] = (u16)((lane ? 1u << entry : (u32)cand_alive) | (exit_bit << 12));
+        cps[qq] = have ? 0x8000u | (bits << 11) | tail : 0u;
+    }
+    lane_rec_store(lane_rec, c, lane_o, lane_rec_pack(cps[0], cps[1], cps[2], (lane ? 1u << entry : (u32)cand_alive) | (exit_bit << 12), count));
     if (lane == 0) {
         chunk_regular[c] = 1;
     }
@@ -842,9 +828,8 @@
     const hufd_chunk_rec *chunk_rec,
     const u8 *d_in,
     u16 *fn_tab,
-    u16 *cp_tab,
+    hufd_lane_rec *lane_rec,
     u32 *chunk_fn,
-    u16 *lane_count,
     u8 *chunk_regular,
     const u32 *given_up,
     const u32 *given_up_count,
@@ -859,7 +844,7 @@
             }
             continue;
         }
-        dec_sync_guess_chunk<LB, SURE>(c, tb, chunk_rec, d_in, fn_tab, cp_tab, chunk_fn, lane_count, chunk_regular, slow_list, slow_count);
+        dec_sync_guess_chunk<LB, SURE>(c, tb, chunk_rec, d_in, fn_tab, lane_rec, chunk_fn, chunk_regular, slow_list, slow_count);
         __syncthreads();
     }
 }
@@ -915,7 +900,7 @@
     const hufd_chunk_rec *chunk_rec,
     const u8 *d_in,
     u16 *fn_tab,
-    u16 *cp_tab,
+    hufd_lane_rec *lane_rec,
     u32 *chunk_fn,
     u8 *chunk_regular,
     const u32 *list,
@@ -1002,12 +987,7 @@
             fn_tab[((u64)c * ns + s) * HUFD_DEC_LANES + lane] = sh.ftab[s * HUFD_DEC_LANES + lane];
         }
         {
-            u16 *cp = cp_tab + (u64)c * kCpRows * HUFD_DEC_LANES + lane;
-#pragma unroll
-            for (u32 qq = 0; qq + 1 < kQuarters; ++qq) {
-                cp[qq * HUFD_DEC_LANES] = 0;
-            }
-            cp[(kQuarters - 1) * HUFD_DEC_LANES] = (u16)(kExitNoRef << 12);
+            lane_rec_store(lane_rec, c, lane, lane_rec_pack(0, 0, 0, kExitNoRef << 12, 0));
         }
         __syncthreads();
         if (lane < kGroups * ns) {
@@ -1035,8 +1015,7 @@
     const hufd_chunk_rec *chunk_rec,
     const u8 *d_in,
     const u16 *fn_tab,
-    u16 *cp_tab,
-    u16 *lane_count,
+    hufd_lane_rec *lane_rec,
     u8 *chunk_regular,
     const u32 *chunk_entry,
     hufd_emit_rec *emit_rec,
@@ -1108,14 +1087,13 @@
         const bool good = sh.bad == 0;
         __syncthreads();
         if (good) {
-            u16 *cp = cp_tab + (u64)c * kCpRows * HUFD_DEC_LANES + lane;
+            u32 cps[kQuarters - 1];
 #pragma unroll
             for (u32 qq = 0; qq + 1 < kQuarters; ++qq) {
                 const u32 tail = count - (cp_state[qq] >> 16), bits = rw.offset_of(cp_state[qq]);
-                cp[qq * HUFD_DEC_LANES] = (u16)(bits < 16u ? 0x8000u | (bits << 11) | tail : 0u);
-            }
-            lane_count[(u64)c * HUFD_DEC_LANES + lane] = (u16)count;
-            cp[(kQuarters - 1) * HUFD_DEC_LANES] = (u16)((1u << entry) | (ex << 12));
+                cps[qq] = bits < 16u ? 0x8000u | (bits << 11) | tail : 0u;
+            }
+            lane_rec_store(lane_rec, c, lane, lane_rec_pack(cps[0], cps[1], cps[2], (1u << entry) | (ex << 12), count));
         }
         if (lane == 0) {
             chunk_regular[c] = good ? 1 : 0;
@@ -1137,9 +1115,8 @@
     const u8 *chunk_regular,
     const u32 *tail_entry,
     u16 *fn_tab,
-    u16 *cp_tab,
-    u32 *chunk_fn,
-    u16 *lane_count) {
+    hufd_lane_rec *lane_rec,
+    u32 *chunk_fn) {
 
     tail_lds &sh = *reinterpret_cast<tail_lds *>(dyn_lds);
     u16 *lut = reinterpret_cast<u16 *>(dyn_lds + sizeof(tail_lds));
@@ -1182,7 +1159,6 @@
     const tail_walk tw = tail_follow(words, lut, tb.lut_bits, entry, (u32)(tail_bytes * 8), limit, nullptr, &stop_pos, &stop_why);
 
     u16 *fn_out = fn_tab + (u64)c * ns * HUFD_DEC_LANES;
-    u16 *cp = cp_tab + (u64)c * kCpRows * HUFD_DEC_LANES;
     for (u32 k = 0; k < 2; ++k) {
         const u32 lane = n_full + k;
         const bool reached = k == 0 || tw.stop != 0;
@@ -1191,10 +1167,9 @@
         }
         const u32 my_entry = k == 0 ? entry : tw.exit;
         const bool stops_here = tw.stop == k;
-        lane_count[(u64)c * HUFD_DEC_LANES + lane] = (u16)tw.count[k];
         fn_out[(u64)my_entry * HUFD_DEC_LANES + lane] =
             stops_here ? fn_pack(true, 0, tw.count[k] & 0x7FFu) : fn_pack(false, tw.exit, tw.count[k] & 0x7FFu);
-        cp[(kQuarters - 1) * HUFD_DEC_LANES + lane] = (u16)((1u << my_entry) | ((stops_here ? kExitStop : tw.exit) << 12));
+        lane_rec_store(lane_rec, c, lane, lane_rec_pack(0, 0, 0, (1u << my_entry) | ((stops_here ? kExitStop : tw.exit) << 12), tw.count[k]));
     }
     const bool stops = tw.stop != 2u;
     for (u32 st = 0; st < ns; ++st) {
@@ -1258,27 +1233,27 @@
     hipLaunchKernelGGL(                                                                                            \
         (dec_sync_one_mixed_kernel<LBV, SUREV>), dim3(a->n_chunks + a->n_tail), dim3(HUFD_DEC_LANES),              \
         (uint32_t)sizeof(one_shared<LBV>), st, a->tables, a->chunk_rec, a->tail_chunks, a->n_tail,                  \
-        (const u8 *)a->d_in, a->fn_tab, a->cp_tab, a->chunk_fn, a->lane_count, a->chunk_regular, a->tail_entry,     \
+        (const u8 *)a->d_in, a->fn_tab, a->lane_rec, a->chunk_fn, a->chunk_regular, a->tail_entry,                 \
         a->slow_list, slow_count, lean_long_list, lean_long_count);                                                \
 } else if (n_packed) {                                                                                                    \
     hipLaunchKernelGGL(                                                                                            \
         (dec_sync_pack_kernel<LBV, SUREV>), dim3((n_packed + pack_slots - 1) / pack_slots), dim3(HUFD_DEC_LANES),   \
         (uint32_t)sizeof(pack_shared<LBV>), tst, a->tables, a->chunk_rec, a->tail_chunks, n_packed, pack_width,     \
-        (const u8 *)a->d_in, a->fn_tab, a->cp_tab, a->chunk_fn, a->lane_count, a->chunk_regular, a->tail_entry,     \
+        (const u8 *)a->d_in, a->fn_tab, a->lane_rec, a->chunk_fn, a->chunk_regular, a->tail_entry,                 \
         lean_long_list, lean_long_count);                                                                          \
 }                                                                                                                  \
 if (!folded && n_single) {                                                                                         \
     hipLaunchKernelGGL(                                                                                            \
         (dec_sync_one_kernel<LBV, SUREV, true>), dim3(n_single), dim3(HUFD_DEC_LANES),                              \
         (uint32_t)sizeof(one_shared<LBV>), tst, a->tables, a->chunk_rec, single_chunks,                             \
-        (const u8 *)a->d_in, a->fn_tab, a->cp_tab, a->chunk_fn, a->lane_count, a->chunk_regular, a->tail_entry,     \
+        (const u8 *)a->d_in, a->fn_tab, a->lane_rec, a->chunk_fn, a->chunk_regular, a->tail_entry,                 \
         a->slow_list, slow_count, lean_long_list, lean_long_count);                                                \
 }                                                                                                                  \
 if (!folded && some_inside) {                                                                                      \
     hipLaunchKernelGGL(                                                                                            \
         (dec_sync_one_kernel<LBV, SUREV, false>), dim3(a->n_chunks), dim3(HUFD_DEC_LANES),                          \
         (uint32_t)sizeof(one_shared<LBV>), st, a->tables, a->chunk_rec, a->tail_chunks,                             \
-        (const u8 *)a->d_in, a->fn_tab, a->cp_tab, a->chunk_fn, a->lane_count, a->chunk_regular, a->tail_entry,     \
+        (const u8 *)a->d_in, a->fn_tab, a->lane_rec, a->chunk_fn, a->chunk_regular, a->tail_entry,                 \
         a->slow_list, slow_count, lean_long_list, lean_long_count);                                                \
 }
     if (lb_of_launch == 10) {
@@ -1295,7 +1270,7 @@
         hipLaunchKernelGGL(
             dec_sync_tail_kernel, dim3((a->n_tail + kTailThreads - 1) / kTailThreads), dim3(kTailThreads), lds, tst,
             a->tables, a->items, a->chunk_item, a->tail_chunks, a->n_tail, (const u8 *)a->d_in,
-            (const u8 *)a->chunk_regular, (const u32 *)a->tail_entry, a->fn_tab, a->cp_tab, a->chunk_fn, a->lane_count);
+            (const u8 *)a->chunk_regular, (const u32 *)a->tail_entry, a->fn_tab, a->lane_rec, a->chunk_fn);
     }
     if (beside) {
         (void)hipEventRecord((hipEvent_t)a->join_event, tst);
@@ -1309,7 +1284,7 @@
     dim3(persistent_grid(dec_sync_guess_kernel<LBV, SUREV>, HUFD_DEC_LANES, (uint32_t)sizeof(lean_shared<LBV>),     \
                          a->n_chunks)),                                                                            \
     dim3(HUFD_DEC_LANES), (uint32_t)sizeof(lean_shared<LBV>), st, a->tables, a->chunk_rec, (const u8 *)a->d_in,     \
-    a->fn_tab, a->cp_tab, a->chunk_fn, a->lane_count, a->chunk_regular, (const u32 *)a->slow_list,                 \
+    a->fn_tab, a->lane_rec, a->chunk_fn, a->chunk_regular, (const u32 *)a->slow_list,                              \
     (const u32 *)slow_count, a->emit_list, a->counters + HUFK_DEC_COUNT_LONG)
         if (lb_of_launch == 10) {
             switch (sure) {
@@ -1329,20 +1304,20 @@
                     (dec_sync_few_kernel<10>),
                     dim3(persistent_grid(dec_sync_few_kernel<10>, HUFD_DEC_LANES, (uint32_t)sizeof(few_shared<10>), a->n_chunks)),
                     dim3(HUFD_DEC_LANES), (uint32_t)sizeof(few_shared<10>), st, a->tables, a->chunk_rec, (const u8 *)a->d_in,
-                    a->fn_tab, a->cp_tab, a->chunk_fn, a->chunk_regular, long_list, long_count, a->slow_list, few_count);
+                    a->fn_tab, a->lane_rec, a->chunk_fn, a->chunk_regular, long_list, long_count, a->slow_list, few_count);
             } else {
                 hipLaunchKernelGGL(
                     (dec_sync_few_kernel<12>),
                     dim3(persistent_grid(dec_sync_few_kernel<12>, HUFD_DEC_LANES, (uint32_t)sizeof(few_shared<12>), a->n_chunks)),
                     dim3(HUFD_DEC_LANES), (uint32_t)sizeof(few_shared<12>), st, a->tables, a->chunk_rec, (const u8 *)a->d_in,
-                    a->fn_tab, a->cp_tab, a->chunk_fn, a->chunk_regular, long_list, long_count, a->slow_list, few_count);
+                    a->fn_tab, a->lane_rec, a->chunk_fn, a->chunk_regular, long_list, long_count, a->slow_list, few_count);
             }
         }
     }
     hipLaunchKernelGGL(
         sync, dim3(persistent_grid(sync, HUFD_DEC_LANES, dec_sync_lds_bytes(&a->tables), a->n_chunks)),
         dim3(HUFD_DEC_LANES), dec_sync_lds_bytes(&a->tables), st, a->tables, a->items, a->chunk_item, a->n_chunks,
-        (const u8 *)a->d_in, a->fn_tab, a->cp_tab, a->chunk_fn, a->chunk_regular, long_list, long_count,
+        (const u8 *)a->d_in, a->fn_tab, a->lane_rec, a->chunk_fn, a->chunk_regular, long_list, long_count,
         a->counters_self_cleared ? a->counters : (u32 *)nullptr);
     s.few = few;
 }
@@ -1356,14 +1331,14 @@
             (dec_sync_true_kernel<10>),
             dim3(persistent_grid(dec_sync_true_kernel<10>, HUFD_DEC_LANES, (uint32_t)sizeof(few_shared<10>), a->n_chunks)),
             dim3(HUFD_DEC_LANES), (uint32_t)sizeof(few_shared<10>), st, a->tables, a->chunk_rec, (const u8 *)a->d_in,
-            (const u16 *)a->fn_tab, a->cp_tab, a->lane_count, a->chunk_regular, (const u32 *)a->chunk_entry,
+            (const u16 *)a->fn_tab, a->lane_rec, a->chunk_regular, (const u32 *)a->chunk_entry,
             a->emit_rec, (const u32 *)a->slow_list, (const u32 *)(a->counters + HUFK_DEC_COUNT_FEW));
     } else {
         hipLaunchKernelGGL(
             (dec_sync_true_kernel<12>),
             dim3(persistent_grid(dec_sync_true_kernel<12>, HUFD_DEC_LANES, (uint32_t)sizeof(few_shared<12>), a->n_chunks)),
             dim3(HUFD_DEC_LANES), (uint32_t)sizeof(few_shared<12>), st, a->tables, a->chunk_rec, (const u8 *)a->d_in,
-            (const u16 *)a->fn_tab, a->cp_tab, a->lane_count, a->chunk_regular, (const u32 *)a->chunk_entry,
+            (const u16 *)a->fn_tab, a->lane_rec, a->chunk_regular, (const u32 *)a->chunk_entry,
             a->emit_rec, (const u32 *)a->slow_list, (const u32 *)(a->counters + HUFK_DEC_COUNT_FEW));
     }
 }
diff --git a/aws-c-compression_amd/csrc/hip/decode_sync_one_body.inc b/aws-c-compression_amd/csrc/hip/decode_sync_one_body.inc
--- a/aws-c-compression_amd/csrc/hip/decode_sync_one_body.inc
+++ b/aws-c-compression_amd/csrc/hip/decode_sync_one_body.inc
@@ -47,7 +47,6 @@
         }
         return;
     }
-    u16 *cp = cp_tab + (u64)c * kCpRows * HUFD_DEC_LANES + lane;
     constexpr u32 kLutPerLane = (1u << LB) / HUFD_DEC_LANES, kLutBatch = 4;
     const auto table_share = [&](u32 j0) {
         u32 lut_raw[kLutBatch];
@@ -66,12 +65,7 @@
             table_share(j0);
         }
         if (!FOLLOW || (lane != n_full && lane != n_full + 1)) {
-#pragma unroll
-            for (u32 qq = 0; qq + 1 < kQuarters; ++qq) {
-                cp[qq * HUFD_DEC_LANES] = 0;
-            }
-            lane_count[(u64)c * HUFD_DEC_LANES + lane] = 0;
-            cp[(kQuarters - 1) * HUFD_DEC_LANES] = (u16)(kExitStop << 12);
+            lane_rec_store(lane_rec, c, lane, lane_rec_unreached());
         }
         return;
     }
@@ -251,8 +245,9 @@
     }
     __syncthreads();
     const bool stay = sh.moved != 0;
-    auto lane_records = [&]() {
+    auto lane_record = [&](u32 merged, u32 symbols) {
         if (active) {
+            u32 cps[kQuarters - 1];
 #pragma unroll
             for (u32 qq = 0; qq + 1 < kQuarters; ++qq) {
                 const u32 boundary = (qq + 1) * (kSubWords / kQuarters);
@@ -264,15 +259,11 @@
                     bits = ow.offset_of(head_cp[qq]);
                     have = true;
                 }
-                cp[qq * HUFD_DEC_LANES] = (u16)(have ? 0x8000u | (bits << 11) | tail : 0u);
-            }
+                cps[qq] = have ? 0x8000u | (bits << 11) | tail : 0u;
+            }
+            lane_rec_store(lane_rec, c, lane, lane_rec_pack(cps[0], cps[1], cps[2], merged, symbols));
         } else if (!FOLLOW || (lane != n_full && lane != n_full + 1)) {
-#pragma unroll
-            for (u32 qq = 0; qq + 1 < kQuarters; ++qq) {
-                cp[qq * HUFD_DEC_LANES] = 0;
-            }
-            lane_count[(u64)c * HUFD_DEC_LANES + lane] = 0;
-            cp[(kQuarters - 1) * HUFD_DEC_LANES] = (u16)(kExitStop << 12);
+            lane_rec_store(lane_rec, c, lane, lane_rec_unreached());
         }
         if (TAIL && lane + 1 == n_full) {
             tail_entry[c] = ref_exit;
@@ -280,11 +271,7 @@
     };
     if (!stay && lane >= kWave) {
         if (!sh.bad && !sh.bad_mine) {
-            lane_records();
-            if (active) {
-                lane_count[(u64)c * HUFD_DEC_LANES + lane] = (u16)count;
-                cp[(kQuarters - 1) * HUFD_DEC_LANES] = (u16)((1u << entry) | (ref_exit << 12));
-            }
+            lane_record((1u << entry) | (ref_exit << 12), count);
         }
         return;
     }
@@ -451,12 +438,7 @@
     }
 
     u16 *fn_out = fn_tab + (u64)c * ns * HUFD_DEC_LANES;
-    lane_records();
-    if (active) {
-        const u32 total = lane ? count : ref_count0;
-        lane_count[(u64)c * HUFD_DEC_LANES + lane] = (u16)total;
-        cp[(kQuarters - 1) * HUFD_DEC_LANES] = (u16)((lane ? 1u << entry : (u32)cand_alive) | (ref_exit << 12));
-    }
+    lane_record((lane ? 1u << entry : (u32)cand_alive) | (ref_exit << 12), lane ? count : ref_count0);
     if (lane == 0) {
         chunk_regular[c] = TAIL ? 2 : 1;
     }
@@ -486,22 +468,15 @@
                 if (ln >= HUFD_DEC_LANES) {
                     break;
                 }
-                u16 *cpl = cp_tab + (u64)c * kCpRows * HUFD_DEC_LANES + ln;
                 const bool reached = k == 0 || tw.stop != 0;
-#pragma unroll
-                for (u32 qq = 0; qq + 1 < kQuarters; ++qq) {
-                    cpl[qq * HUFD_DEC_LANES] = 0;
-                }
                 if (reached) {
                     const u32 my_entry = k == 0 ? entry_t : tw.exit;
                     const bool stops_here = tw.stop == k;
-                    lane_count[(u64)c * HUFD_DEC_LANES + ln] = (u16)tw.count[k];
                     fn_out[(u64)my_entry * HUFD_DEC_LANES + ln] =
                         stops_here ? fn_pack(true, 0, tw.count[k] & 0x7FFu) : fn_pack(false, tw.exit, tw.count[k] & 0x7FFu);
-                    cpl[(kQuarters - 1) * HUFD_DEC_LANES] = (u16)((1u << my_entry) | ((stops_here ? kExitStop : tw.exit) << 12));
+                    lane_rec_store(lane_rec, c, ln, lane_rec_pack(0, 0, 0, (1u << my_entry) | ((stops_here ? kExitStop : tw.exit) << 12), tw.count[k]));
                 } else {
-                    lane_count[(u64)c * HUFD_DEC_LANES + ln] = 0;
-                    cpl[(kQuarters - 1) * HUFD_DEC_LANES] = (u16)(kExitStop << 12);
+                    lane_rec_store(lane_rec, c, ln, lane_rec_unreached());
                 }
             }
         }
diff --git a/aws-c-compression_amd/csrc/hip/device_types.h b/aws-c-compression_amd/csrc/hip/device_types.h
--- a/aws-c-compression_amd/csrc/hip/device_types.h
+++ b/aws-c-compression_amd/csrc/hip/device_types.h
@@ -193,6 +193,13 @@
     uint64_t base;
 };
 
+struct __attribute__((aligned(16))) hufd_lane_rec {
+    uint16_t cp[HUFD_DEC_CP_ROWS - 1];
+    uint16_t merged;
+    uint16_t count;
+    uint16_t reserved[3];
+};
+
 #define HUFD_ITEMS_DEVICE_ARRAY 0u
 #define HUFD_ITEMS_STRIDED 1u
 #define HUFD_ITEMS_FROM_ENCODE 2u
diff --git a/aws-c-compression_amd/csrc/hip/huffman_kernels.h b/aws-c-compression_amd/csrc/hip/huffman_kernels.h
--- a/aws-c-compression_amd/csrc/hip/huffman_kernels.h
+++ b/aws-c-compression_amd/csrc/hip/huffman_kernels.h
@@ -82,7 +82,7 @@
     const void *d_in;
     void *d_out;
     uint16_t *fn_tab;
-    uint16_t *cp_tab;
+    struct hufd_lane_rec *lane_rec;
     uint32_t *chunk_fn;
     uint32_t *slow_list;
     uint32_t *emit_list;
@@ -91,7 +91,6 @@
     uint32_t counters_self_cleared;
     uint32_t *summary;
     uint32_t quiet;
-    uint16_t *lane_count;
     uint8_t *chunk_regular;
     uint32_t *tail_entry;
     uint32_t *chunk_entry;
diff --git a/aws-c-compression_amd/csrc/host/engine.c b/aws-c-compression_amd/csrc/host/engine.c
--- a/aws-c-compression_amd/csrc/host/engine.c
+++ b/aws-c-compression_amd/csrc/host/engine.c
@@ -1536,13 +1536,12 @@
     X(d_runs, (cr) * 2 * sizeof(uint32_t))                                                                             \
     X(d_run_fn, (cr) * (ns) * sizeof(uint32_t))                                                                        \
     X(d_fn_tab, (cc) * (ns) * HUFD_DEC_LANES * sizeof(uint16_t))                                                       \
-    X(d_cp_tab, (cc) * HUFD_DEC_CP_ROWS * HUFD_DEC_LANES * sizeof(uint16_t))                                           \
+    X(d_lane_rec, (cc) * HUFD_DEC_LANES * sizeof(struct hufd_lane_rec))  \
     X(d_chunk_fn, (cc) * (ns) * sizeof(uint32_t))                                                                      \
     X(d_slow_list, ((cc) + 1) * sizeof(uint32_t))                                         \
     X(d_emit_list, ((cc) + 1) * sizeof(uint32_t))                                                                      \
     X(d_dense_list, ((cc) + 1) * sizeof(uint32_t))                                                                     \
     X(d_counters, HUFK_DEC_COUNTERS * sizeof(uint32_t))                                                                \
-    X(d_lane_count, (cc) * HUFD_DEC_LANES * sizeof(uint16_t))                                                          \
     X(d_chunk_regular, (cc))                                                                                           \
     X(d_tail_entry, (cc) * sizeof(uint32_t))                                                                           \
     X(d_chunk_entry, (cc) * sizeof(uint32_t))                                                                          \
@@ -1553,6 +1552,8 @@
                                                                                  \
     X(d_summary, DEC_SUMMARY_BYTES)                                                                                    \
     X(d_results, (ci) * sizeof(struct hufd_dec_result))
+
+_Static_assert(sizeof(struct hufd_lane_rec) == 16, "a sub-chunk's record is one 16-byte load or store");
 
 static void dec_plan_release_device(struct aws_huffman_amd_decode_plan *p) {
     hufs_free(p->d_arena);
@@ -2455,7 +2456,7 @@
     a.d_in = device_input;
     a.d_out = device_output;
     a.fn_tab = p->d_fn_tab;
-    a.cp_tab = p->d_cp_tab;
+    a.lane_rec = p->d_lane_rec;
     a.chunk_fn = p->d_chunk_fn;
     a.slow_list = p->d_slow_list + 1;
     a.emit_list = p->d_emit_list + 1;
@@ -2464,7 +2465,6 @@
     a.counters_self_cleared = 1;
     a.summary = p->d_summary;
     a.quiet = p->quiet && !(testing_decode_road() & AWS_HUFFMAN_AMD_TEST_DECODE_ALL_KERNELS);
-    a.lane_count = p->d_lane_count;
     a.chunk_regular = p->d_chunk_regular;
     a.tail_entry = p->d_tail_entry;
     a.chunk_entry = p->d_chunk_entry;
diff --git a/aws-c-compression_amd/csrc/host/engine.h b/aws-c-compression_amd/csrc/host/engine.h
--- a/aws-c-compression_amd/csrc/host/engine.h
+++ b/aws-c-compression_amd/csrc/host/engine.h
@@ -126,14 +126,13 @@
     uint32_t *d_runs;
     uint32_t *d_run_fn;
     uint16_t *d_fn_tab;
-    uint16_t *d_cp_tab;
+    struct hufd_lane_rec *d_lane_rec;
     uint32_t *d_chunk_fn;
     uint32_t *d_slow_list;
     uint32_t *d_emit_list;
     uint32_t *d_dense_list;
     uint32_t *d_counters;
     uint32_t launches_with_chunks;
-    uint16_t *d_lane_count;
     uint8_t *d_chunk_regular;
     uint32_t *d_tail_entry;
     uint32_t *d_chunk_entry;
```

Result: faster. 688.7 (median of 6 runs) (+2.6%).
